# foollh/PicoPose

Measured on AMD Instinct MI355X. Metric: image-crops/sec (224x224, 162 templates), higher is better.
Workload: dtype f32 tensors; networks: f32 operands split into 2 f16 terms (22 bits) on f16 MFMA with f32 accumulate; stage-1 contraction: f16 MFMA operands, f32 accumulate, exact f32 re-evaluation of near-ties; PnP f64

## Files before the change

### include/picopose_hip.h

```cpp
#ifndef PICOPOSE_HIP_H
#define PICOPOSE_HIP_H

#include <stddef.h>
#include <stdint.h>

#ifdef __cplusplus
extern "C" {
#endif

#define PP_OK 0
#define PP_EINVAL (-1)
#define PP_EWORKSPACE (-2)
#define PP_ELAUNCH (-3)

#define PP_MATCH_EXACT 0
#define PP_MATCH_FAST 1

const char* pp_strerror(int code);
int pp_version(void);

int pp_prof_enable(int max_records);
int pp_prof_collect(float* out_ms, int max_out, int* count);
int pp_prof_gemm_enable(int max_records);
int pp_prof_gemm_collect(double* ms, double* flops, int* launches);
int pp_prof_gemm_records(int max_records, int* shape, float* ms, double* flops, int* count);
int pp_prof_gemm_records2(int max_records, int* shape, float* ms, double* flops, double* bytes, int* count);
int pp_gemm_tune_save(const char* path);
int pp_gemm_tune_load(const char* path);
int pp_gemm_tune_entries(void);
int pp_gemm_generic_epilogue(int on);

int pp_stage1_workspace_bytes(int B, int N, int C, size_t* bytes);

int pp_stage1_scores(const float* bank, const float* query, const float* mask,
                     int mask_h, int mask_w, int B, int N, int C, int mode,
                     float eps, void* workspace, size_t workspace_bytes,
                     float* sim_avg, int32_t* stats, void* stream);

#define PP_BANK_F32 0
#define PP_BANK_F16 1
int pp_stage1_scores_ex(const void* bank, int bank_dtype, const float* query, const float* mask,
                        int mask_h, int mask_w, int B, int N, int C, int mode,
                        float eps, void* workspace, size_t workspace_bytes,
                        float* sim_avg, int32_t* stats, void* stream);

int pp_topk(const float* scores, int B, int N, int k, float* out_score,
            int64_t* out_index, void* stream);

int pp_stage1_match(const float* bank, const float* query, const float* mask,
                    int mask_h, int mask_w, int B, int N, int C, int k, int mode,
                    float eps, void* workspace, size_t workspace_bytes,
                    float* sim_avg, float* out_score, int64_t* out_index,
                    int32_t* stats, void* stream);
int pp_stage1_match_ex(const void* bank, int bank_dtype, const float* query, const float* mask,
                       int mask_h, int mask_w, int B, int N, int C, int k, int mode,
                       float eps, void* workspace, size_t workspace_bytes, float* sim_avg,
                       float* out_score, int64_t* out_index, int32_t* stats, void* stream);

int pp_stage1_indexed_workspace_bytes(int B, int N, int C, size_t* bytes);
int pp_stage1_scores_indexed(const void* bank, int bank_dtype, const int64_t* obj_index, int n_obj,
                             const float* query, const float* mask, int mask_h, int mask_w, int B, int N,
                             int C, int mode, float eps, void* workspace, size_t workspace_bytes,
                             float* sim_avg, int32_t* stats, void* stream);
int pp_stage1_match_indexed(const void* bank, int bank_dtype, const int64_t* obj_index, int n_obj,
                            const float* query, const float* mask, int mask_h, int mask_w, int B, int N,
                            int C, int k, int mode, float eps, void* workspace, size_t workspace_bytes,
                            float* sim_avg, float* out_score, int64_t* out_index, int32_t* stats,
                            void* stream);



int pp_similarity_volume(const float* src_feat, const float* tar_feat, const float* src_mask,
                         int mask_h, int mask_w, int B, int C, float* out, void* stream);

int pp_calc_pred_Ms(const float* pred_scale, const float* pred_inplane, const float* pred_translation,
                    const float* tem_pose, const float* tem_K, const float* tem_M, int B,
                    float trans_scale, float* pred_Ms, void* stream);

int pp_pose_recovery_2d(const float* query_M, const float* query_K, const float* pred_Ms,
                        const float* tem_K, const float* tem_M, const float* tem_pose, int B,
                        float* pred_pose, void* stream);

int pp_init_correspondences(const float* pred_Ms, const float* tem_mask, int mask_h, int mask_w, int B,
                            float* init_flow, float* init_certainty, void* stream);

int pp_stage3_correspondences(const float* pred_flow, const float* pred_certainty, int B, int H, int W,
                              float threshold, int64_t* tar_pts, int64_t* src_pts, void* stream);

int pp_gather_valid(const float* features, const int64_t* index_patches, int B, int C, int H, int W,
                    int N, float* out, int32_t* count, void* stream);

#define PP_ACT_NONE 0
#define PP_ACT_RELU 1
#define PP_ACT_GELU 2
#define PP_ACT_LEAKY01 3
#define PP_ACT_TANH 4

#define PP_PREC_F32 0
#define PP_PREC_F16X3 1
#define PP_PREC_F16 2

typedef struct PpGemmDesc {
    const float* A;
    const float* B;
    float* C;
    const float* bias;
    const float* gamma;
    const float* residual;
    const float* residual2;
    int M, N, K;
    int lda, ldb, ldc;
    int b_kn;
    int batch0, batch1;
    long long a_bs0, a_bs1, b_bs0, b_bs1, c_bs0, c_bs1;
    float alpha;
    int act;
    int relu_in;
    int conv_kh, conv_kw, conv_cin, conv_stride, conv_pad, conv_h, conv_w, conv_ho, conv_wo;
    long long conv_bstride;
    int shuffle_r, shuffle_h, shuffle_w;
    int prec;
    const void* B_hl;
    float b_scale;
    const void* A_hl;
    long long a_hl_bytes, b_hl_bytes;
    void* C_hl;
    int ldc_h;
    int c_relu;
    const float* alpha_dev;
    const float* alpha_dev2;
    int ksplit;
    int ks_rows;
    int grp_rows;
    long long grp_b_bytes;
} PpGemmDesc;

int pp_gemm(const PpGemmDesc* desc, void* stream);
int pp_split_f16x3(const float* w, long long n, void* hl, float* scale, void* stream);
int pp_split_weights_ws(const float* w, long long n, int terms, void* out, float* scale2, float* partials, void* stream);
int pp_split_activation(const float* x, long long batch_stride, int B, int P, int row_stride, int C, int relu,
                        void* hl, void* stream);
int pp_split_activation_ld(const float* x, long long batch_stride, int B, int P, int row_stride, int C, int relu,
                           void* hl, int ld_h, void* stream);
int pp_pow2_scale_ws(const float* x, long long n, float* scale2, float* partials, void* stream);
int pp_split_scaled_t(const float* x, long long rows, int ld, int C, const float* scale, void* out, int terms, void* stream);
int pp_split_transpose_t(const float* x, long long rows, int cols, int ld, const float* scale, void* out, int terms, void* stream);
int pp_split_transpose_ld(const float* x, long long rows, int cols, int ld, const float* scale, void* out, long long ld_out, int terms,
                          void* stream);
int pp_im2col_t_operand(const float* x, int B, int H, int W, int C, int ksize, int stride, int pad, void* out, int terms, void* stream);
int pp_sum_slices(const float* part, int S, int M, int N, const float* bias, int act, float* out, void* stream);
int pp_hl_patch_columns(const float* x, int ld_x, int c, long long rows, void* hl, int ld_h, int col0, void* stream);

int pp_split_weights_t(const float* w, long long n, int terms, void* out, float* scale, void* stream);
int pp_split_activation_t(const float* x, long long batch_stride, int B, int P, int row_stride, int C, int relu, void* out,
                          int ld_h, int terms, void* stream);
int pp_hl_patch_columns_t(const float* x, int ld_x, int c, long long rows, void* out, int ld_h, int col0, int terms, void* stream);
int pp_layernorm_t(const float* x, const float* gamma, const float* beta, int rows, int C, float eps, float* y, void* out, int terms,
                   void* stream);
int pp_resize_bilinear_nhwc_t(const float* in, int B, int H, int W, int C, int Ho, int Wo, float mul, void* out, int terms,
                              void* stream);
int pp_resize_bilinear_nhwc_dual(const float* in, int B, int H, int W, int C, int Ho, int Wo, float mul, float* out, void* out_operand,
                                 int terms, void* stream);
int pp_warp_nhwc_t(const float* feat, int feat_batch, const float* flow, int B, int H, int W, int C, int ld_flow, void* out,
                   int ld_h, int terms, void* stream);
int pp_attention_t(const void* qkv_operand, int terms, int B, int T, int heads, int head_dim, float scale, float* out,
                   void* out_operand, void* stream);

int pp_attention(const float* qkv, int B, int T, int heads, int head_dim, float scale, float* out, void* stream);
int pp_attention_split(const float* qkv, int B, int T, int heads, int head_dim, float scale, float* out, void* out_hl,
                       void* stream);
int pp_attention_ex(const float* qkv, int B, int T, int heads, int head_dim, float scale, int prec, float* out, void* out_hl,
                    void* stream);
int pp_attention_hl(const void* qkv_hl, int B, int T, int heads, int head_dim, float scale, float* out, void* out_hl,
                    void* stream);
int pp_attention_train(const float* qkv, int B, int T, int heads, int head_dim, float scale, float* out, float* lse2, void* stream);
int pp_attention_backward(const float* qkv, const float* out, const float* dout, const float* lse2, const float* gpair, int B, int T,
                          int heads, int head_dim, float scale, float* Dws, float* dqkv, void* stream);

int pp_layernorm(const float* x, const float* gamma, const float* beta, int rows, int C, float eps,
                 float* y, void* stream);
int pp_layernorm_split(const float* x, const float* gamma, const float* beta, int rows, int C, float eps, float* y,
                       void* hl, void* stream);
int pp_softmax_rows(float* x, int rows, int n, int ld, void* stream);
int pp_groupnorm_nhwc(const float* x, const float* gamma, const float* beta, int B, int HW, int C,
                      int groups, float eps, int relu, float* y, void* stream);
int pp_transpose_batched(const float* in, long long in_batch_stride, int B, int R, int C, float* out,
                         long long out_batch_stride, int ld_out, int col_off, void* stream);
int pp_assemble_tokens(const float* patches, const float* cls_token, const float* pos, int B, int T, int C,
                       float* tokens, void* stream);
int pp_normalize_rows(const float* x, int rows, int n, float eps, float* y, void* stream);

int pp_resize_bilinear_nhwc(const float* in, int B, int H, int W, int C, int Ho, int Wo, float mul,
                            float* out, void* stream);
int pp_resize_bilinear_nhwc_hl(const float* in, int B, int H, int W, int C, int Ho, int Wo, float mul, void* out_hl,
                               void* stream);
int pp_warp_nhwc(const float* feat, int feat_batch, const float* flow, int B, int H, int W, int C, int ld_flow,
                 float* out, int ld_out, void* stream);
int pp_warp_nhwc_hl(const float* feat, int feat_batch, const float* flow, int B, int H, int W, int C, int ld_flow,
                    void* out_hl, int ld_h, void* stream);
int pp_avgpool2_nhwc(const float* in, int B, int H, int W, int C, float* out, void* stream);
int pp_gather_rows(const float* src, const long long* index, long long n_src_rows, long long row_floats, int n, float* dst,
                   void* stream);
int pp_bank_rows_to_tokens(const float* bank, long long n_bank_rows, int C, int P, const long long* index, int n, float* tokens, int ld,
                           int T, int skip, void* stream);
int pp_patch_operand(const float* bank, long long n_bank_rows, const long long* index, int n, const float* front, int n_front, int H, int W,
                     void* out, int terms, void* stream);
int pp_flow_operand(const float* flow, int ld_flow, long long rows, void* out8, int terms, void* stream);

int pp_crop_resize_normalize(const unsigned char* image, int H, int W, const unsigned char* mask, int y1, int y2, int x1,
                             int x2, int S, int rgb_mask_flag, const double* mean3, const double* std3, float* out_rgb,
                             float* out_mask, void* stream);
int pp_depth_points_nearest(const float* depth_m, int H, int W, int y1, int y2, int x1, int x2, int P, float fx, float fy,
                            float cx, float cy, float* out_pts, void* stream);
int pp_corr_lookup_nhwc(const float* f1, int ld_f1, const float* f2_l0, const float* f2_l1, const float* f2_l2,
                        int f2_batch, const float* flow, int B, int H, int W, int C, int levels, int radius,
                        int ld_flow, float* out, int ld_out, void* stream);
int pp_corr_lookup_nhwc_ex(const float* f1, int ld_f1, const float* f2_l0, const float* f2_l1, const float* f2_l2,
                           int f2_batch, const float* flow, int B, int H, int W, int C, int levels, int radius,
                           int ld_flow, int prec, float* out, int ld_out, void* stream);

int pp_conv_narrow_hl(const void* x_hl, int ld_x, int B, int H, int W, int C, const float* weight, const float* bias, int ksize,
                      int n_out, const float* residual, float* out, void* stream);
int pp_conv_narrow_f32(const float* x, int ld_x, int B, int H, int W, int C, const float* weight, const float* bias, int ksize,
                       int n_out, const float* residual, float* out, void* stream);

int pp_winograd_input_f32(const float* x, int ld_x, long long batch_stride, int B, int H, int W, int C, int relu, float* U, void* stream);
int pp_winograd_weight_f32(const float* w, int Cout, int Cin, int ldw, float* V, void* stream);
int pp_winograd_output_f32(const float* Y, int B, int H, int W, int Cout, const float* bias, int act, const float* residual,
                           const float* residual2, float* out, int ldc, void* stream);

int pp_winograd4_input_hl(const void* x_hl, int ld_x, long long batch_stride, int B, int H, int W, int C, int relu, void* U_hl, long long P_pad,
                          void* stream);
int pp_winograd4_weight_f32(const float* w, int Cout, int Cin, int ldw, float* V, void* stream);
int pp_winograd4_output(const float* Y, int ld_y, int B, int H, int W, int Cout, const float* bias, int act, const float* residual,
                        const float* residual2, float* out, int ldc, void* out_hl, int ld_h, int c_relu, long long P_pad, void* stream);

int pp_winograd4_chain(const float* Y, int ld_y, int B, int H, int W, int C, const float* bias, int act, int c_relu, void* U_hl, long long P_pad,
                       void* stream);

int pp_winograd_chain_f32(const float* Y, int B, int H, int W, int C, const float* bias, int act, int relu_next, float* U, void* stream);

int pp_set_saturation_word(unsigned int* word);

int pp_saturation_take(unsigned int* word, unsigned int* slot, void* stream);


int pp_corr_lookup_nhwc_hl(const void* f1_hl, int ld_f1, const void* f2_hl_l0, const void* f2_hl_l1, const void* f2_hl_l2,
                           int f2_batch, const float* flow, int B, int H, int W, int C, int levels, int radius, int ld_flow,
                           float* out, int ld_out, void* stream);

int pp_pnp_ransac(const float* tar_pts_2d, const float* src_pts_3d, const float* K, const float* tem_pose,
                  const int64_t* tar_pts, const int64_t* src_pts, int P, int H, int W, int N, int iterations,
                  float reproj_threshold, double* rot, double* tvec, double* inlier_ratio, int32_t* success,
                  int32_t* num_points, void* stream);

int pp_pnp_ransac_debug(const float* tar_pts_2d, const float* src_pts_3d, const float* K, const float* tem_pose,
                        const int64_t* tar_pts, const int64_t* src_pts, int P, int H, int W, int N, int iterations,
                        float reproj_threshold, double* rot, double* tvec, double* inlier_ratio, int32_t* success,
                        int32_t* num_points, double* refit_branches, void* stream);

int pp_pnp_ransac_refine(const float* tar_pts_2d, const float* src_pts_3d, const float* K, const float* tem_pose,
                         const int64_t* tar_pts, const int64_t* src_pts, int P, int H, int W, int N, int iterations,
                         float reproj_threshold, int max_iters, double eps, double* rot, double* tvec, double* inlier_ratio,
                         int32_t* success, int32_t* num_points, double* rms_before, double* rms_after, int32_t* lm_iterations,
                         uint8_t* inlier_mask, void* stream);

int pp_pnp_refine_lm(const double* object_points, const double* image_points, const int32_t* count, const double* K,
                     const double* rot_init, const double* tvec_init, int P, int Nmax, int max_iters, double eps, double* rot,
                     double* tvec, double* rms_before, double* rms_after, int32_t* lm_iterations, void* stream);

int pp_rgbd_ransac(const float* tar_pts_2d, const float* src_pts_3d, const float* K, const float* tem_pose,
                   const int64_t* tar_pts, const int64_t* src_pts, int P, int H, int W, int N,
                   const float* depth, int n_images, int dH, int dW, const int32_t* image_index,
                   const float* inlier_dist, int iterations,
                   double* rot, double* tvec, double* inlier_ratio, int32_t* success,
                   int32_t* num_points, int32_t* num_listed, double* rms, uint8_t* inlier_mask, void* stream);

size_t pp_train_keypoints_workspace_bytes(int B);
int pp_train_keypoints(const float* src_mask, const float* tar_mask, int mask_h, int mask_w, const float* src_depth,
                       const float* tar_depth, int depth_h, int depth_w, const float* src_Minv, const float* tar_Minv,
                       const float* src_M, const float* tar_M, const float* src_Kinv, const float* tar_Kinv, const float* src_K,
                       const float* tar_K, const float* T_src2tar, const float* T_tar2src, int B, float* src_pts, float* tar_pts,
                       void* workspace, size_t workspace_bytes, void* stream);
size_t pp_batchnorm_train_workspace_bytes(int rows, int C);
int pp_batchnorm_train(const float* x, const float* gamma, const float* beta, int rows, int C, float eps, float momentum,
                       float* running_mean, float* running_var, int relu, const float* residual, const float* residual2, float* y,
                       void* workspace, size_t workspace_bytes, void* stream);
int pp_gather_normalize_rows(const float* src, long long row_stride, const int64_t* index, int n, int C, float eps, float* out,
                             void* stream);
int pp_xent_diag_rows(const float* logits, int n, int ld, float scale, float* row_loss, void* stream);
int pp_flow_loss_blocks(void);
int pp_flow_loss_sums(const float* flow, const float* certainty, const float* tar_pts, int B, int H, int W, float max_flow,
                      double* partial_sums, void* stream);

size_t pp_colsum_workspace_bytes(long long rows, int cols);
int pp_colsum(const float* x, long long rows, int cols, int ld, float* out, void* workspace, size_t workspace_bytes, void* stream);
int pp_act_forward(const float* z, long long n, int act, float* y, void* stream);
int pp_act_backward(const float* z, const float* dy, long long n, int act, float* dz, void* stream);
int pp_elementwise(int op, const float* a, const float* b, long long n, int cols, float* out, void* stream);
int pp_layernorm_backward(const float* x, const float* gamma, const float* dy, int rows, int C, float eps, float* dx, float* gx, void* stream);
int pp_groupnorm_backward_nhwc(const float* x, const float* gamma, const float* beta, const float* dy, int B, int HW, int C, int groups,
                               float eps, int relu, float* dx, float* gx, float* gy, void* stream);
int pp_softmax_backward_rows(const float* p, const float* dp, long long rows, int n, float* ds, void* stream);
int pp_xent_diag_backward(const float* logits, int n, int ld, float scale, const float* upstream, float* dlogits, void* stream);
int pp_scatter_add_rows(const float* src, const int64_t* index, int n, int C, float* dst, void* stream);
int pp_normalize_rows_backward(const float* x, long long row_stride, const int64_t* index, const float* dq, int rows, int C, float eps,
                               float* dx, void* stream);
int pp_im2col_nhwc(const float* x, int B, int H, int W, int C, int ksize, int stride, int pad, float* col, void* stream);
int pp_col2im_nhwc(const float* col, int B, int H, int W, int C, int ksize, int stride, int pad, float* dx, void* stream);
int pp_split_with_scale_t(const float* w, long long n, int terms, const float* scale, void* out, void* stream);
int pp_pow2_scale(const float* x, long long n, float* scale2, void* stream);
int pp_im2col_t_nhwc(const float* x, int B, int H, int W, int C, int ksize, int stride, int pad, float* colT, void* stream);
int pp_simvol_backward(const float* out, const float* dout, const float* src_mask, int mask_h, int mask_w, int B, float* dS, void* stream);

size_t pp_batchnorm_train_backward_workspace_bytes(long long rows, int C);
int pp_batchnorm_train_backward(const float* x, const float* gamma, const float* beta, const float* dy, long long rows, int C, float eps,
                                int relu, float* dx, float* dgamma, float* dbeta, void* workspace, size_t workspace_bytes, void* stream);
int pp_resize_bilinear_backward_nhwc(const float* dy, int B, int H, int W, int C, int Ho, int Wo, float mul, float* dx, void* stream);
int pp_avgpool2_backward_nhwc(const float* dy, int B, int H, int W, int C, int accumulate, float* dx, void* stream);
int pp_warp_backward_nhwc(const float* feat, const float* flow, const float* dy, int B, int H, int W, int C, int ld_flow, float* dfeat,
                          float* dflow, void* stream);
int pp_corr_lookup_backward_nhwc(const float* f1, const float* const* f2_levels, const float* flow, const float* dout, int B, int H, int W,
                                 int C, int levels, int radius, int ld_flow, int ld_dout, float* df1, float* const* df2_levels, float* dflow,
                                 void* stream);
int pp_warp_backward_nhwc_fixed(const float* feat, const float* flow, const float* dy, int B, int H, int W, int C, int ld_flow,
                                long long* dfeat_acc, float* dflow, void* stream);
int pp_corr_lookup_backward_nhwc_fixed(const float* f1, const float* const* f2_levels, const float* flow, const float* dout, int B, int H,
                                       int W, int C, int levels, int radius, int ld_flow, int ld_dout, float* df1,
                                       long long* const* df2_acc_levels, float* dflow, void* stream);
int pp_fixed_to_float(const long long* acc, long long n, float* out, void* stream);
int pp_flow_loss_backward(const float* flow, const float* certainty, const float* tar_pts, int B, int H, int W, float max_flow,
                          const float* g_flow, const float* g_cert, float* dflow, float* dcertainty, void* stream);


#define PP_ADAM_CHUNK 65536
typedef struct PpAdamTensor {
    float* p;
    float* m;
    float* v;
    void* hl;
    float* scale2;
    long long n;
} PpAdamTensor;
typedef struct PpAdamStep {
    const float* g;
    float neg_step_size, inv_bc2_sqrt, decay, lerp_w, beta2, one_minus_beta2, eps;
    int mode;
} PpAdamStep;
int pp_adam_workspace_bytes(const PpAdamTensor* tensors, int ntensors, size_t* bytes);
int pp_adam_multi_tensor(const PpAdamTensor* tensors, int ntensors, const PpAdamStep* steps, int terms, int rebuild, void* workspace,
                         size_t workspace_bytes, void* stream);

#define PP_AUG_OP_WORDS 8
#define PP_AUG_IMG_WORDS 20
#define PP_AUG_MAX_OPS 13
#define PP_AUG_MAX_PASSES 4
#define PP_AUG_DROP_THRESHOLD 858993459u
int pp_augment_execute(const unsigned char* rgb0, const unsigned char* mask0, long long n_frame0_px, const unsigned char* rgba1,
                       long long n_frame1_px,
                       const int* images, int n_images, const int* ops, int n_ops, const int* tiles, const int* pass_tiles,
                       int n_passes, unsigned char* buf0, unsigned char* buf1, long long n_buf_px, unsigned int* lsum,
                       void* stream);
int pp_augment_resize(const unsigned char* buf0, const unsigned char* buf1, long long n_buf_px, const int* images, int n_images,
                      int S, int rgb_mask_flag, const double* mean3, const double* std3, float* out_rgb, float* out_mask,
                      void* stream);
int pp_depth_u16_scaled(const unsigned short* depth, long long n_per_frame, int n_frames, const float* scale, float* out,
                        void* stream);
int pp_depth_u16_template(const unsigned short* depth, long long n, float* out, void* stream);

int pp_detections_crop(const unsigned char* image, int H, int W, const int* run_ends, int n_runs, const int* run_offset,
                       const int* window, const int* run_offset_host, const int* window_host, int n, int S, int rgb_mask_flag,
                       const double* mean3, const double* std3, float* out_rgb, float* out_mask, void* stream);

int pp_render_workspace_bytes(int H, int W, int n_faces, int chunk_views, size_t* bytes);
int pp_render_views(const float* vertices, int n_vertices, const int* faces, const int* faces_host, int n_faces,
                    const unsigned char* colors, const float* poses, int n_views, float fx, float fy, float cx, float cy, int H,
                    int W, float near, void* workspace, size_t workspace_bytes, unsigned char* rgba, unsigned short* depth_mm,
                    float* depth_m, int* face_id, unsigned int* near_count, void* stream);
#define PP_TEXTURE_MAX 16384
int pp_texture_mips_bytes(int Wt, int Ht, size_t* bytes, int* levels);
int pp_texture_build_mips(const unsigned char* rgb, int Wt, int Ht, void* mips, size_t mips_bytes, void* stream);
int pp_render_views_textured(const float* vertices, int n_vertices, const int* faces, const int* faces_host, int n_faces,
                             const float* face_uv, const void* mips, int Wt, int Ht, const float* poses, int n_views, float fx,
                             float fy, float cx, float cy, int H, int W, float near, void* workspace, size_t workspace_bytes,
                             unsigned char* rgba, unsigned short* depth_mm, float* depth_m, int* face_id, unsigned int* near_count,
                             void* stream);
#define PP_MAX_LIGHTS 16
#define PP_TONE_MAX 65536
#define PP_NORMALS_FLAT 0
#define PP_NORMALS_SMOOTH 1
int pp_vertex_normals(const float* vertices, int n_vertices, const int* faces, int n_faces, const int* vf_offsets, const int* vf_faces,
                      float* normals, void* stream);
int pp_render_views_lit(const float* vertices, int n_vertices, const int* faces, const int* faces_host, int n_faces,
                        const unsigned char* colors, const float* face_uv, const void* mips, int Wt, int Ht, const float* poses,
                        int n_views, float fx, float fy, float cx, float cy, int H, int W, float near, void* workspace,
                        size_t workspace_bytes, unsigned char* rgba, unsigned short* depth_mm, float* depth_m, int* face_id,
                        unsigned int* near_count, const float* lights_host, int n_lights, float ambient, int normal_mode,
                        const float* normals, const unsigned char* base_color_host, const unsigned char* tone_table, int tone_entries,
                        void* stream);
int pp_template_extents(const unsigned char* rgba, int n_views, int H, int W, int* extents, int* counts, void* stream);
int pp_templates_crop(const unsigned char* rgba, const void* depth, int depth_is_f32, int n_views, int H, int W, const int* boxes,
                      const int* boxes_host, float fx, float fy, float cx, float cy, int S, int P, int rgb_mask_flag,
                      const double* mean3, const double* std3, float* out_rgb, float* out_mask, float* out_pts, void* stream);

#define PP_EVAL_MSSD 1
#define PP_EVAL_MSPD 2
#define PP_EVAL_ADD 4
#define PP_EVAL_ADDS 8
#define PP_EVAL_ADDS_TILE 1024
int pp_pose_errors_workspace_bytes(int n_pairs, int max_syms, int max_adds_vertices, int kinds, size_t* bytes);
int pp_pose_errors(const float* vertices, const int* vert_off, const float* adds_vertices, const int* adds_off, const float* sym_R,
                   const float* sym_t, const int* sym_off, const int* vert_off_host, const int* adds_off_host,
                   const int* sym_off_host, int n_objects, const int* pair_obj, const int* pair_obj_host, const float* R_est,
                   const float* t_est, const float* R_gt, const float* t_gt, const float* focal, int n_pairs, int kinds,
                   void* workspace, size_t workspace_bytes, float* mssd, int* mssd_sym, float* mspd, int* mspd_sym, float* add,
                   float* adds, void* stream);

typedef struct PpScene {
    const float* vertices;
    const int* vert_off;
    const int* faces;
    const int* face_off;
    const float* diameters;
    const float* cams;
    const int* view_obj;
    const int* view_img;
    const float* poses;
    const int* windows;
    const long long* view_zoff;
    const int* vert_off_host;
    const int* faces_host;
    const int* face_off_host;
    const float* diameters_host;
    const float* cams_host;
    const int* view_obj_host;
    const int* view_img_host;
    const int* windows_host;
    const long long* view_zoff_host;
    int n_objects, n_images, H, W, n_views;
    float near;
} PpScene;

#define PP_VSD_MAX_TAUS 16
int pp_vsd_workspace_bytes(long long window_samples, long long view_faces, size_t* bytes);
int pp_vsd_errors(const PpScene* scene, const int* pair_est, const int* pair_gt, const int* pair_est_host, const int* pair_gt_host,
                  int n_pairs, const float* depth, float delta, const float* taus_host, int n_taus, void* workspace,
                  size_t workspace_bytes, float* vsd, int* counts, unsigned int* near_count, float* depth_out, void* stream);

#define PP_DEPTH_REFINE_STRIP_ROWS 8
#define PP_DEPTH_REFINE_SUMS 29
#define PP_DEPTH_REFINE_MAX_ITERATIONS 1000
int pp_depth_refine_workspace_bytes(long long window_samples, long long view_faces, long long strips, size_t* bytes);
int pp_depth_refine(const PpScene* scene, const float* boxes, const float* boxes_host, const int* view_soff, const int* view_soff_host,
                    const float* depth, int iterations, float max_distance, int min_points, float min_cos, float rcond, float eps,
                    float max_translation, float max_rotation, void* workspace, size_t workspace_bytes, float* poses_out,
                    int* active, int* status, int* n_iterations, int* rank, int* n_points, float* rms_before, float* rms_after,
                    unsigned int* near_count, float* trajectory, double* sums, void* stream);

int pp_scene_gt_workspace_bytes(long long window_samples, long long view_faces, long long composite_pixels, size_t* bytes);
int pp_scene_gt(const PpScene* scene, const float* canvas_cams, const float* canvas_cams_host, int pad_x, int pad_y, const float* depth,
                float delta, const int* view_label, int use_view_label, void* workspace, size_t workspace_bytes, int* counts, int* boxes,
                unsigned int* near_count, unsigned char* mask_all, unsigned char* mask_visib, float* scene_depth, int* instance_map,
                void* stream);

#define PP_MODEL_INFO_TILE 1024
int pp_model_diameter_workspace_bytes(const int* vert_off_host, int n_objects, size_t* bytes);
int pp_model_diameter(const float* vertices, const int* vert_off, const int* vert_off_host, int n_objects, void* workspace,
                      size_t workspace_bytes, float* d2max, int* pair, void* stream);
int pp_transform_hausdorff_workspace_bytes(int n_candidates, int max_query_vertices, size_t* bytes);
int pp_transform_hausdorff(const float* vertices, const int* vert_off, const float* q_vertices, const int* q_off,
                           const int* vert_off_host, const int* q_off_host, int n_objects, const int* cand_obj,
                           const int* cand_obj_host, const float* cand_T, int n_candidates, void* workspace, size_t workspace_bytes,
                           float* h, void* stream);

#define PP_SYNTH_BG_WORDS 4
#define PP_SYNTH_TILE 1024
int pp_scene_composite_workspace_bytes(int n_layers, int H, int W, size_t* bytes);
int pp_scene_composite(const unsigned char* layers_rgba, const float* layers_depth, const int* layer_off, const int* layer_off_host,
                       int n_layers, int n_images, int H, int W, const int* background, const int* background_host,
                       const unsigned char* bg_images, const float* depth_scale, const float* depth_scale_host, void* workspace,
                       size_t workspace_bytes, unsigned char* rgb, unsigned short* depth, int* instance, int* counts, int* boxes,
                       unsigned char* mask_visib, void* stream);
int pp_depth_quantize_u16(const float* depth_m, long long n, float units_per_metre, unsigned short* out, void* stream);

#define PP_MATCH_TILE 16
#define PP_MATCH_MAX_C 1024
#define PP_MATCH_MAX_TOPK 8
#define PP_MASK_MAX_N 4096
int pp_descriptor_normalize(const float* x, int n, int C, float eps, float* y, void* stream);
int pp_proposal_match(const float* query, int P, const float* bank, const int* offsets, const int* offsets_host, int O, int C,
                      int topk, float* score, int* view, int* label, float* best, void* stream);
int pp_rle_pack_bits(const int* run_ends, int n_runs, const int* run_offset, const int* run_offset_host, int n, int hw, int words,
                     unsigned* bits, int* area, void* stream);
int pp_mask_intersections(const unsigned* bits, int n, int words, int* inter, void* stream);

#ifdef __cplusplus
}
#endif
#endif
```

### picopose_amd/_lib.py

```python
import ctypes
import os
import re

from .build import LIB

_HEADER = os.path.join(os.path.dirname(os.path.abspath(__file__)), "..", "include", "picopose_hip.h")

PP_OK = 0
PP_MATCH_EXACT = 0
PP_MATCH_FAST = 1
PP_BANK_F32 = 0
PP_BANK_F16 = 1

_lib = None


class PpGemmDesc(ctypes.Structure):
    _fields_ = [
        ("A", ctypes.c_void_p), ("B", ctypes.c_void_p), ("C", ctypes.c_void_p), ("bias", ctypes.c_void_p),
        ("gamma", ctypes.c_void_p), ("residual", ctypes.c_void_p), ("residual2", ctypes.c_void_p),
        ("M", ctypes.c_int), ("N", ctypes.c_int), ("K", ctypes.c_int),
        ("lda", ctypes.c_int), ("ldb", ctypes.c_int), ("ldc", ctypes.c_int), ("b_kn", ctypes.c_int),
        ("batch0", ctypes.c_int), ("batch1", ctypes.c_int),
        ("a_bs0", ctypes.c_longlong), ("a_bs1", ctypes.c_longlong), ("b_bs0", ctypes.c_longlong),
        ("b_bs1", ctypes.c_longlong), ("c_bs0", ctypes.c_longlong), ("c_bs1", ctypes.c_longlong),
        ("alpha", ctypes.c_float), ("act", ctypes.c_int), ("relu_in", ctypes.c_int),
        ("conv_kh", ctypes.c_int), ("conv_kw", ctypes.c_int), ("conv_cin", ctypes.c_int),
        ("conv_stride", ctypes.c_int), ("conv_pad", ctypes.c_int), ("conv_h", ctypes.c_int),
        ("conv_w", ctypes.c_int), ("conv_ho", ctypes.c_int), ("conv_wo", ctypes.c_int),
        ("conv_bstride", ctypes.c_longlong),
        ("shuffle_r", ctypes.c_int), ("shuffle_h", ctypes.c_int), ("shuffle_w", ctypes.c_int),
        ("prec", ctypes.c_int), ("B_hl", ctypes.c_void_p), ("b_scale", ctypes.c_float), ("A_hl", ctypes.c_void_p),
        ("a_hl_bytes", ctypes.c_longlong), ("b_hl_bytes", ctypes.c_longlong),
        ("C_hl", ctypes.c_void_p), ("ldc_h", ctypes.c_int), ("c_relu", ctypes.c_int),
        ("alpha_dev", ctypes.c_void_p), ("alpha_dev2", ctypes.c_void_p),
        ("ksplit", ctypes.c_int), ("ks_rows", ctypes.c_int), ("grp_rows", ctypes.c_int), ("grp_b_bytes", ctypes.c_longlong),
    ]


class PpScene(ctypes.Structure):
    _fields_ = ([(name, ctypes.c_void_p) for name in (
        "vertices", "vert_off", "faces", "face_off", "diameters", "cams", "view_obj", "view_img", "poses", "windows", "view_zoff",
        "vert_off_host", "faces_host", "face_off_host", "diameters_host", "cams_host", "view_obj_host", "view_img_host", "windows_host",
        "view_zoff_host")] + [(name, ctypes.c_int) for name in ("n_objects", "n_images", "H", "W", "n_views")] + [("near", ctypes.c_float)])


class PpAdamTensor(ctypes.Structure):
    _fields_ = [("p", ctypes.c_void_p), ("m", ctypes.c_void_p), ("v", ctypes.c_void_p), ("hl", ctypes.c_void_p),
                ("scale2", ctypes.c_void_p), ("n", ctypes.c_longlong)]


class PicoPoseHipError(RuntimeError):
    pass


def declared_symbols():
    text = open(_HEADER).read()
    text = re.sub(r"/\*.*?\*/", "", text, flags=re.S)
    return sorted(set(re.findall(r"\b(pp_[a-z0-9_]+)\s*\(", text)))


def lib():
    global _lib
    if _lib is None:
        if not os.path.exists(LIB):
            raise PicoPoseHipError(
                f"{LIB} not found: build it with `python -m picopose_amd.build` "
                "(hipcc --offload-arch=gfx950). There is no CPU fallback."
            )
        import torch

        L = ctypes.CDLL(LIB)
        c = ctypes
        vp, i32, f32, sz = c.c_void_p, c.c_int, c.c_float, c.c_size_t
        L.pp_strerror.restype = c.c_char_p
        L.pp_strerror.argtypes = [i32]
        L.pp_version.restype = i32
        L.pp_prof_enable.argtypes = [i32]
        L.pp_prof_collect.argtypes = [c.POINTER(f32), i32, c.POINTER(i32)]
        L.pp_prof_gemm_enable.argtypes = [i32]
        L.pp_prof_gemm_collect.argtypes = [c.POINTER(c.c_double), c.POINTER(c.c_double), c.POINTER(i32)]
        L.pp_prof_gemm_records.argtypes = [i32, c.POINTER(i32), c.POINTER(f32), c.POINTER(c.c_double), c.POINTER(i32)]
        L.pp_prof_gemm_records2.argtypes = [i32, c.POINTER(i32), c.POINTER(f32), c.POINTER(c.c_double), c.POINTER(c.c_double), c.POINTER(i32)]
        L.pp_gemm_tune_save.argtypes = [c.c_char_p]
        L.pp_gemm_tune_load.argtypes = [c.c_char_p]
        L.pp_gemm_tune_entries.argtypes = []
        L.pp_gemm_generic_epilogue.argtypes = [i32]
        L.pp_stage1_workspace_bytes.argtypes = [i32, i32, i32, c.POINTER(sz)]
        L.pp_stage1_scores.argtypes = [vp, vp, vp, i32, i32, i32, i32, i32, i32, f32, vp, sz, vp, vp, vp]
        L.pp_stage1_scores_ex.argtypes = [vp, i32, vp, vp, i32, i32, i32, i32, i32, i32, f32, vp, sz, vp, vp, vp]
        L.pp_topk.argtypes = [vp, i32, i32, i32, vp, vp, vp]
        L.pp_stage1_match.argtypes = [vp, vp, vp, i32, i32, i32, i32, i32, i32, i32, f32, vp, sz,
                                      vp, vp, vp, vp, vp]
        L.pp_stage1_match_ex.argtypes = [vp, i32, vp, vp, i32, i32, i32, i32, i32, i32, i32, f32, vp, sz, vp, vp, vp, vp, vp]
        L.pp_stage1_indexed_workspace_bytes.argtypes = [i32, i32, i32, c.POINTER(sz)]
        L.pp_stage1_scores_indexed.argtypes = [vp, i32, vp, i32, vp, vp, i32, i32, i32, i32, i32, i32, f32, vp, sz, vp, vp, vp]
        L.pp_stage1_match_indexed.argtypes = [vp, i32, vp, i32, vp, vp, i32, i32, i32, i32, i32, i32, i32, f32, vp, sz, vp, vp, vp,
                                              vp, vp]
        L.pp_similarity_volume.argtypes = [vp, vp, vp, i32, i32, i32, i32, vp, vp]
        L.pp_calc_pred_Ms.argtypes = [vp, vp, vp, vp, vp, vp, i32, f32, vp, vp]
        L.pp_pose_recovery_2d.argtypes = [vp, vp, vp, vp, vp, vp, i32, vp, vp]
        L.pp_init_correspondences.argtypes = [vp, vp, i32, i32, i32, vp, vp, vp]
        L.pp_stage3_correspondences.argtypes = [vp, vp, i32, i32, i32, f32, vp, vp, vp]
        L.pp_gather_valid.argtypes = [vp, vp, i32, i32, i32, i32, i32, vp, vp, vp]
        L.pp_gemm.argtypes = [c.POINTER(PpGemmDesc), vp]
        L.pp_split_f16x3.argtypes = [vp, c.c_longlong, vp, vp, vp]
        L.pp_split_activation.argtypes = [vp, c.c_longlong, i32, i32, i32, i32, i32, vp, vp]
        L.pp_split_activation_ld.argtypes = [vp, c.c_longlong, i32, i32, i32, i32, i32, vp, i32, vp]
        L.pp_conv_narrow_hl.argtypes = [vp, i32, i32, i32, i32, i32, vp, vp, i32, i32, vp, vp, vp]
        L.pp_conv_narrow_f32.argtypes = [vp, i32, i32, i32, i32, i32, vp, vp, i32, i32, vp, vp, vp]
        L.pp_winograd_input_f32.argtypes = [vp, i32, c.c_longlong, i32, i32, i32, i32, i32, vp, vp]
        L.pp_winograd_weight_f32.argtypes = [vp, i32, i32, i32, vp, vp]
        L.pp_winograd_output_f32.argtypes = [vp, i32, i32, i32, i32, vp, i32, vp, vp, vp, i32, vp]
        L.pp_winograd4_input_hl.argtypes = [vp, i32, c.c_longlong, i32, i32, i32, i32, i32, vp, c.c_longlong, vp]
        L.pp_winograd4_weight_f32.argtypes = [vp, i32, i32, i32, vp, vp]
        L.pp_winograd4_output.argtypes = [vp, i32, i32, i32, i32, i32, vp, i32, vp, vp, vp, i32, vp, i32, i32, c.c_longlong, vp]
        L.pp_winograd4_chain.argtypes = [vp, i32, i32, i32, i32, i32, vp, i32, i32, vp, c.c_longlong, vp]
        L.pp_winograd_chain_f32.argtypes = [vp, i32, i32, i32, i32, vp, i32, i32, vp, vp]
        L.pp_set_saturation_word.argtypes = [vp]
        L.pp_saturation_take.argtypes = [vp, vp, vp]
        L.pp_split_weights_t.argtypes = [vp, c.c_longlong, i32, vp, vp, vp]
        L.pp_split_weights_ws.argtypes = [vp, c.c_longlong, i32, vp, vp, vp, vp]
        L.pp_split_activation_t.argtypes = [vp, c.c_longlong, i32, i32, i32, i32, i32, vp, i32, i32, vp]
        L.pp_hl_patch_columns_t.argtypes = [vp, i32, i32, c.c_longlong, vp, i32, i32, i32, vp]
        L.pp_layernorm_t.argtypes = [vp, vp, vp, i32, i32, f32, vp, vp, i32, vp]
        L.pp_resize_bilinear_nhwc_t.argtypes = [vp, i32, i32, i32, i32, i32, i32, f32, vp, i32, vp]
        L.pp_resize_bilinear_nhwc_dual.argtypes = [vp, i32, i32, i32, i32, i32, i32, f32, vp, vp, i32, vp]
        L.pp_warp_nhwc_t.argtypes = [vp, i32, vp, i32, i32, i32, i32, i32, vp, i32, i32, vp]
        L.pp_attention_t.argtypes = [vp, i32, i32, i32, i32, i32, f32, vp, vp, vp]
        L.pp_sum_slices.argtypes = [vp, i32, i32, i32, vp, i32, vp, vp]
        L.pp_hl_patch_columns.argtypes = [vp, i32, i32, c.c_longlong, vp, i32, i32, vp]
        L.pp_warp_nhwc_hl.argtypes = [vp, i32, vp, i32, i32, i32, i32, i32, vp, i32, vp]
        L.pp_attention.argtypes = [vp, i32, i32, i32, i32, f32, vp, vp]
        L.pp_attention_split.argtypes = [vp, i32, i32, i32, i32, f32, vp, vp, vp]
        L.pp_attention_ex.argtypes = [vp, i32, i32, i32, i32, f32, i32, vp, vp, vp]
        L.pp_attention_hl.argtypes = [vp, i32, i32, i32, i32, f32, vp, vp, vp]
        L.pp_attention_train.argtypes = [vp, i32, i32, i32, i32, f32, vp, vp, vp]
        L.pp_attention_backward.argtypes = [vp, vp, vp, vp, vp, i32, i32, i32, i32, f32, vp, vp, vp]
        L.pp_layernorm.argtypes = [vp, vp, vp, i32, i32, f32, vp, vp]
        L.pp_layernorm_split.argtypes = [vp, vp, vp, i32, i32, f32, vp, vp, vp]
        L.pp_softmax_rows.argtypes = [vp, i32, i32, i32, vp]
        L.pp_groupnorm_nhwc.argtypes = [vp, vp, vp, i32, i32, i32, i32, f32, i32, vp, vp]
        L.pp_transpose_batched.argtypes = [vp, c.c_longlong, i32, i32, i32, vp, c.c_longlong, i32, i32, vp]
        L.pp_assemble_tokens.argtypes = [vp, vp, vp, i32, i32, i32, vp, vp]
        L.pp_normalize_rows.argtypes = [vp, i32, i32, f32, vp, vp]
        L.pp_resize_bilinear_nhwc.argtypes = [vp, i32, i32, i32, i32, i32, i32, f32, vp, vp]
        L.pp_resize_bilinear_nhwc_hl.argtypes = [vp, i32, i32, i32, i32, i32, i32, f32, vp, vp]
        L.pp_warp_nhwc.argtypes = [vp, i32, vp, i32, i32, i32, i32, i32, vp, i32, vp]
        L.pp_avgpool2_nhwc.argtypes = [vp, i32, i32, i32, i32, vp, vp]
        L.pp_gather_rows.argtypes = [vp, vp, c.c_longlong, c.c_longlong, i32, vp, vp]
        L.pp_bank_rows_to_tokens.argtypes = [vp, c.c_longlong, i32, i32, vp, i32, vp, i32, i32, i32, vp]
        L.pp_patch_operand.argtypes = [vp, c.c_longlong, vp, i32, vp, i32, i32, i32, vp, i32, vp]
        L.pp_flow_operand.argtypes = [vp, i32, c.c_longlong, vp, i32, vp]
        L.pp_depth_points_nearest.argtypes = [vp, i32, i32, i32, i32, i32, i32, i32, f32, f32, f32, f32, vp, vp]
        L.pp_crop_resize_normalize.argtypes = [vp, i32, i32, vp, i32, i32, i32, i32, i32, i32, c.POINTER(c.c_double),
                                               c.POINTER(c.c_double), vp, vp, vp]
        L.pp_corr_lookup_nhwc.argtypes = [vp, i32, vp, vp, vp, i32, vp, i32, i32, i32, i32, i32, i32, i32, vp, i32, vp]
        L.pp_corr_lookup_nhwc_ex.argtypes = [vp, i32, vp, vp, vp, i32, vp, i32, i32, i32, i32, i32, i32, i32, i32, vp, i32, vp]
        L.pp_corr_lookup_nhwc_hl.argtypes = [vp, i32, vp, vp, vp, i32, vp, i32, i32, i32, i32, i32, i32, i32, vp, i32, vp]
        L.pp_pnp_ransac.argtypes = [vp, vp, vp, vp, vp, vp, i32, i32, i32, i32, i32, f32, vp, vp, vp, vp, vp, vp]
        L.pp_pnp_ransac_debug.argtypes = [vp, vp, vp, vp, vp, vp, i32, i32, i32, i32, i32, f32, vp, vp, vp, vp, vp, vp, vp]
        L.pp_pnp_ransac_refine.argtypes = [vp, vp, vp, vp, vp, vp, i32, i32, i32, i32, i32, f32, i32, c.c_double] + [vp] * 10
        L.pp_pnp_refine_lm.argtypes = [vp] * 6 + [i32, i32, i32, c.c_double] + [vp] * 6
        L.pp_rgbd_ransac.argtypes = [vp] * 6 + [i32] * 4 + [vp, i32, i32, i32, vp, vp, i32] + [vp] * 9
        L.pp_train_keypoints_workspace_bytes.restype = sz
        L.pp_train_keypoints_workspace_bytes.argtypes = [i32]
        L.pp_train_keypoints.argtypes = [vp, vp, i32, i32, vp, vp, i32, i32] + [vp] * 10 + [i32, vp, vp, vp, sz, vp]
        L.pp_batchnorm_train_workspace_bytes.restype = sz
        L.pp_batchnorm_train_workspace_bytes.argtypes = [i32, i32]
        L.pp_batchnorm_train.argtypes = [vp, vp, vp, i32, i32, f32, f32, vp, vp, i32, vp, vp, vp, vp, sz, vp]
        L.pp_gather_normalize_rows.argtypes = [vp, c.c_longlong, vp, i32, i32, f32, vp, vp]
        L.pp_xent_diag_rows.argtypes = [vp, i32, i32, f32, vp, vp]
        L.pp_flow_loss_blocks.argtypes = []
        L.pp_flow_loss_sums.argtypes = [vp, vp, vp, i32, i32, i32, f32, vp, vp]
        ll = c.c_longlong
        L.pp_colsum_workspace_bytes.restype = sz
        L.pp_colsum_workspace_bytes.argtypes = [ll, i32]
        L.pp_colsum.argtypes = [vp, ll, i32, i32, vp, vp, sz, vp]
        L.pp_act_forward.argtypes = [vp, ll, i32, vp, vp]
        L.pp_act_backward.argtypes = [vp, vp, ll, i32, vp, vp]
        L.pp_elementwise.argtypes = [i32, vp, vp, ll, i32, vp, vp]
        L.pp_layernorm_backward.argtypes = [vp, vp, vp, i32, i32, f32, vp, vp, vp]
        L.pp_groupnorm_backward_nhwc.argtypes = [vp, vp, vp, vp, i32, i32, i32, i32, f32, i32, vp, vp, vp, vp]
        L.pp_softmax_backward_rows.argtypes = [vp, vp, ll, i32, vp, vp]
        L.pp_xent_diag_backward.argtypes = [vp, i32, i32, f32, vp, vp, vp]
        L.pp_normalize_rows_backward.argtypes = [vp, ll, vp, vp, i32, i32, f32, vp, vp]
        L.pp_scatter_add_rows.argtypes = [vp, vp, i32, i32, vp, vp]
        L.pp_im2col_nhwc.argtypes = [vp, i32, i32, i32, i32, i32, i32, i32, vp, vp]
        L.pp_col2im_nhwc.argtypes = [vp, i32, i32, i32, i32, i32, i32, i32, vp, vp]
        L.pp_simvol_backward.argtypes = [vp, vp, vp, i32, i32, i32, vp, vp]
        L.pp_im2col_t_nhwc.argtypes = [vp, i32, i32, i32, i32, i32, i32, i32, vp, vp]
        L.pp_pow2_scale.argtypes = [vp, ll, vp, vp]
        L.pp_pow2_scale_ws.argtypes = [vp, ll, vp, vp, vp]
        L.pp_split_scaled_t.argtypes = [vp, ll, i32, i32, vp, vp, i32, vp]
        L.pp_split_transpose_t.argtypes = [vp, ll, i32, i32, vp, vp, i32, vp]
        L.pp_split_transpose_ld.argtypes = [vp, ll, i32, i32, vp, vp, ll, i32, vp]
        L.pp_im2col_t_operand.argtypes = [vp, i32, i32, i32, i32, i32, i32, i32, vp, i32, vp]
        L.pp_split_with_scale_t.argtypes = [vp, ll, i32, vp, vp, vp]
        L.pp_batchnorm_train_backward_workspace_bytes.restype = sz
        L.pp_batchnorm_train_backward_workspace_bytes.argtypes = [ll, i32]
        L.pp_batchnorm_train_backward.argtypes = [vp, vp, vp, vp, ll, i32, f32, i32, vp, vp, vp, vp, sz, vp]
        L.pp_resize_bilinear_backward_nhwc.argtypes = [vp, i32, i32, i32, i32, i32, i32, f32, vp, vp]
        L.pp_avgpool2_backward_nhwc.argtypes = [vp, i32, i32, i32, i32, i32, vp, vp]
        L.pp_warp_backward_nhwc.argtypes = [vp, vp, vp, i32, i32, i32, i32, i32, vp, vp, vp]
        L.pp_corr_lookup_backward_nhwc.argtypes = [vp, vp, vp, vp, i32, i32, i32, i32, i32, i32, i32, i32, vp, vp, vp, vp]
        L.pp_warp_backward_nhwc_fixed.argtypes = [vp, vp, vp, i32, i32, i32, i32, i32, vp, vp, vp]
        L.pp_corr_lookup_backward_nhwc_fixed.argtypes = [vp, vp, vp, vp, i32, i32, i32, i32, i32, i32, i32, i32, vp, vp, vp, vp]
        L.pp_fixed_to_float.argtypes = [vp, ll, vp, vp]
        L.pp_flow_loss_backward.argtypes = [vp, vp, vp, i32, i32, i32, f32, vp, vp, vp, vp, vp]
        L.pp_adam_workspace_bytes.argtypes = [c.POINTER(PpAdamTensor), i32, c.POINTER(sz)]
        L.pp_adam_multi_tensor.argtypes = [c.POINTER(PpAdamTensor), i32, vp, i32, i32, vp, sz, vp]
        L.pp_augment_execute.argtypes = [vp, vp, ll, vp, ll, vp, i32, vp, i32, vp, c.POINTER(i32), i32, vp, vp, ll, vp, vp]
        L.pp_augment_resize.argtypes = [vp, vp, ll, vp, i32, i32, i32, c.POINTER(c.c_double), c.POINTER(c.c_double), vp, vp, vp]
        L.pp_depth_u16_scaled.argtypes = [vp, ll, i32, vp, vp, vp]
        L.pp_depth_u16_template.argtypes = [vp, ll, vp, vp]
        L.pp_detections_crop.argtypes = [vp, i32, i32, vp, i32, vp, vp, c.POINTER(i32), c.POINTER(i32), i32, i32, i32,
                                         c.POINTER(c.c_double), c.POINTER(c.c_double), vp, vp, vp]
        L.pp_render_workspace_bytes.argtypes = [i32, i32, i32, i32, c.POINTER(sz)]
        L.pp_render_views.argtypes = [vp, i32, vp, vp, i32, vp, vp, i32, f32, f32, f32, f32, i32, i32, f32, vp, sz, vp, vp, vp, vp, vp, vp]
        L.pp_texture_mips_bytes.argtypes = [i32, i32, c.POINTER(sz), c.POINTER(i32)]
        L.pp_texture_build_mips.argtypes = [vp, i32, i32, vp, sz, vp]
        L.pp_render_views_textured.argtypes = [vp, i32, vp, vp, i32, vp, vp, i32, i32, vp, i32, f32, f32, f32, f32, i32, i32, f32, vp, sz,
                                               vp, vp, vp, vp, vp, vp]
        L.pp_vertex_normals.argtypes = [vp, i32, vp, i32, vp, vp, vp, vp]
        L.pp_render_views_lit.argtypes = [vp, i32, vp, vp, i32, vp, vp, vp, i32, i32, vp, i32, f32, f32, f32, f32, i32, i32, f32, vp, sz,
                                          vp, vp, vp, vp, vp, vp, i32, f32, i32, vp, vp, vp, i32, vp]
        L.pp_template_extents.argtypes = [vp, i32, i32, i32, vp, vp, vp]
        L.pp_templates_crop.argtypes = [vp, vp, i32, i32, i32, i32, vp, vp, f32, f32, f32, f32, i32, i32, i32,
                                        c.POINTER(c.c_double), c.POINTER(c.c_double), vp, vp, vp, vp]
        L.pp_pose_errors_workspace_bytes.argtypes = [i32, i32, i32, i32, c.POINTER(sz)]
        L.pp_pose_errors.argtypes = [vp] * 10 + [i32] + [vp] * 7 + [i32, i32, vp, sz] + [vp] * 7
        L.pp_vsd_workspace_bytes.argtypes = [ll, ll, c.POINTER(sz)]
        scene = c.POINTER(PpScene)
        L.pp_vsd_errors.argtypes = [scene, vp, vp, vp, vp, i32, vp, f32, vp, i32, vp, sz, vp, vp, vp, vp, vp]
        L.pp_depth_refine_workspace_bytes.argtypes = [ll, ll, ll, c.POINTER(sz)]
        L.pp_depth_refine.argtypes = [scene, vp, vp, vp, vp, vp, i32, f32, i32, f32, f32, f32, f32, f32, vp, sz,
                                      vp, vp, vp, vp, vp, vp, vp, vp, vp, vp, vp, vp]
        L.pp_scene_gt_workspace_bytes.argtypes = [ll, ll, ll, c.POINTER(sz)]
        L.pp_scene_gt.argtypes = [scene, vp, vp, i32, i32, vp, f32, vp, i32, vp, sz, vp, vp, vp, vp, vp, vp, vp, vp]
        L.pp_model_diameter_workspace_bytes.argtypes = [vp, i32, c.POINTER(sz)]
        L.pp_model_diameter.argtypes = [vp, vp, vp, i32, vp, sz, vp, vp, vp]
        L.pp_transform_hausdorff_workspace_bytes.argtypes = [i32, i32, c.POINTER(sz)]
        L.pp_transform_hausdorff.argtypes = [vp] * 6 + [i32, vp, vp, vp, i32, vp, sz, vp, vp]
        L.pp_scene_composite_workspace_bytes.argtypes = [i32, i32, i32, c.POINTER(sz)]
        L.pp_scene_composite.argtypes = [vp] * 4 + [i32] * 4 + [vp] * 6 + [sz] + [vp] * 7
        L.pp_depth_quantize_u16.argtypes = [vp, ll, f32, vp, vp]
        L.pp_descriptor_normalize.argtypes = [vp, i32, i32, f32, vp, vp]
        L.pp_proposal_match.argtypes = [vp, i32, vp, vp, c.POINTER(i32), i32, i32, i32, vp, vp, vp, vp, vp]
        L.pp_rle_pack_bits.argtypes = [vp, i32, vp, c.POINTER(i32), i32, i32, i32, vp, vp, vp]
        L.pp_mask_intersections.argtypes = [vp, i32, i32, vp, vp]
        _lib = L
    return _lib


def stream_ptr():
    import torch

    return ctypes.c_void_p(torch.cuda.current_stream().cuda_stream)


def dev_f32(*tensors):
    out = []
    for t in tensors:
        if not t.is_cuda:
            raise PicoPoseHipError("picopose_amd runs on the GPU only: inputs must be CUDA(HIP) tensors")
        out.append(t.contiguous().float())
    return out


def check(rc, what):
    if rc != PP_OK:
        raise PicoPoseHipError(f"{what} failed: {lib().pp_strerror(rc).decode()} (code {rc})")
```

### picopose_amd/csrc/pp_sample.hip

```cpp

#include <hip/hip_runtime.h>
#include <stdlib.h>
#include <stdint.h>
#include "../../include/picopose_hip.h"
#include "pp_common.h"
#include "pp_crop_dev.h"

namespace {

typedef float f4 __attribute__((ext_vector_type(4)));

__device__ __forceinline__ float resize_blend(float a, float b, float c, float d, float hx, float lx, float hy, float ly, float mul) {
#pragma clang fp contract(off)
    const float top = fmaf(hx, a, lx * b), bot = fmaf(hx, c, lx * d);
    return (hy * top + ly * bot) * mul;
}

__global__ __launch_bounds__(256) void resize_kernel(const float* __restrict__ in, int H, int W, int C,
                                                     int Ho, int Wo, float mul, float* __restrict__ out,
                                                     _Float16* __restrict__ out_hl, int terms) {
    const int b = blockIdx.z, oy = blockIdx.y, tid = threadIdx.x;
    const float sy = Ho > 1 ? (float)(H - 1) / (float)(Ho - 1) : 0.f;
    const float sx = Wo > 1 ? (float)(W - 1) / (float)(Wo - 1) : 0.f;
    const float fy = sy * (float)oy;
    const int y0 = (int)fy, y1 = y0 + (y0 < H - 1 ? 1 : 0);
    const float ly = fy - (float)y0, hy = 1.f - ly;
    const float* ib = in + (size_t)b * H * W * C;
    if (out_hl) {
        _Float16* oh = out_hl + ((size_t)b * Ho + oy) * Wo * terms * C;
        float* of = out ? out + ((size_t)b * Ho + oy) * Wo * C : nullptr;
        const int C8 = C >> 3;
        for (int i = blockIdx.x * 256 + tid; i < Wo * C8; i += gridDim.x * 256) {
            const int ox = i / C8, c = (i - ox * C8) * 8;
            const float fx = sx * (float)ox;
            const int x0 = (int)fx, x1 = x0 + (x0 < W - 1 ? 1 : 0);
            const float lx = fx - (float)x0, hx = 1.f - lx;
            typedef _Float16 h8 __attribute__((ext_vector_type(8)));
            h8 hh, ll;
#pragma unroll
            for (int q = 0; q < 2; ++q) {
                const int cc = c + 4 * q;
                const f4 a = *(const f4*)(ib + ((size_t)y0 * W + x0) * C + cc), bq = *(const f4*)(ib + ((size_t)y0 * W + x1) * C + cc);
                const f4 cq = *(const f4*)(ib + ((size_t)y1 * W + x0) * C + cc), dq = *(const f4*)(ib + ((size_t)y1 * W + x1) * C + cc);
                f4 vq;
#pragma unroll
                for (int k = 0; k < 4; ++k) {
                    const float v = resize_blend(a[k], bq[k], cq[k], dq[k], hx, lx, hy, ly, mul);
                    _Float16 h, l;
                    pp_split_f16_chk(v, h, l);
                    hh[4 * q + k] = h;
                    ll[4 * q + k] = l;
                    vq[k] = v;
                }
                if (of) *(f4*)(of + (size_t)ox * C + cc) = vq;
            }
            *(h8*)(oh + ((size_t)ox * C + c) * terms) = hh;
            if (terms == 2) *(h8*)(oh + (size_t)ox * 2 * C + 2 * c + 8) = ll;
        }
        return;
    }
    float* ob = out + ((size_t)b * Ho + oy) * Wo * C;
    if ((C & 3) == 0 && (((uintptr_t)in | (uintptr_t)out) & 15) == 0) {
        const int C4 = C >> 2;
        for (int i = blockIdx.x * 256 + tid; i < Wo * C4; i += gridDim.x * 256) {
            const int ox = i / C4, c = (i - ox * C4) * 4;
            const float fx = sx * (float)ox;
            const int x0 = (int)fx, x1 = x0 + (x0 < W - 1 ? 1 : 0);
            const float lx = fx - (float)x0, hx = 1.f - lx;
            const f4 a = *(const f4*)(ib + ((size_t)y0 * W + x0) * C + c), bq = *(const f4*)(ib + ((size_t)y0 * W + x1) * C + c);
            const f4 cq = *(const f4*)(ib + ((size_t)y1 * W + x0) * C + c), dq = *(const f4*)(ib + ((size_t)y1 * W + x1) * C + c);
            f4 v;
#pragma unroll
            for (int k = 0; k < 4; ++k) v[k] = resize_blend(a[k], bq[k], cq[k], dq[k], hx, lx, hy, ly, mul);
            *(f4*)(ob + (size_t)ox * C + c) = v;
        }
        return;
    }
    for (int i = blockIdx.x * 256 + tid; i < Wo * C; i += gridDim.x * 256) {
        const int ox = i / C, c = i - ox * C;
        const float fx = sx * (float)ox;
        const int x0 = (int)fx, x1 = x0 + (x0 < W - 1 ? 1 : 0);
        const float lx = fx - (float)x0, hx = 1.f - lx;
        ob[i] = resize_blend(ib[((size_t)y0 * W + x0) * C + c], ib[((size_t)y0 * W + x1) * C + c], ib[((size_t)y1 * W + x0) * C + c],
                             ib[((size_t)y1 * W + x1) * C + c], hx, lx, hy, ly, mul);
    }
}

__device__ __forceinline__ float roundtrip(float x, int size) {
    const float n = x * 2.f / (float)(size - 1 > 1 ? size - 1 : 1) - 1.f;
    return ((n + 1.f) / 2.f) * (float)(size - 1);
}

template <bool HL>
__global__ __launch_bounds__(256) void warp_kernel(const float* __restrict__ feat, int feat_batch,
                                                   const float* __restrict__ flow, int H, int W, int C, int ld_flow,
                                                   float* __restrict__ out, int ld_out, int terms) {
    const int b = blockIdx.y, p = blockIdx.x * 4 + (threadIdx.x >> 6), lane = threadIdx.x & 63;
    if (p >= H * W) return;
    const int y = p / W, x = p - y * W;
    const float* fl = flow + ((size_t)b * H * W + p) * ld_flow;
    const float ix = fminf(fmaxf(roundtrip((float)x + fl[0], W), -2.f), (float)W + 1.f);
    const float iy = fminf(fmaxf(roundtrip((float)y + fl[1], H), -2.f), (float)H + 1.f);
    const float x0f = floorf(ix), y0f = floorf(iy);
    const int x0 = (int)x0f, y0 = (int)y0f;
    const float wx1 = ix - x0f, wx0 = (x0f + 1.f) - ix, wy1 = iy - y0f, wy0 = (y0f + 1.f) - iy;
    const float* fb = feat + (size_t)(b % feat_batch) * H * W * C;
    float* o = HL ? nullptr : out + ((size_t)b * H * W + p) * ld_out;
    _Float16* oh = HL ? (_Float16*)out + ((size_t)b * H * W + p) * terms * ld_out : nullptr;
    const bool vx0 = x0 >= 0 && x0 < W, vx1 = x0 + 1 >= 0 && x0 + 1 < W;
    const bool vy0 = y0 >= 0 && y0 < H, vy1 = y0 + 1 >= 0 && y0 + 1 < H;
    typedef unsigned u4w __attribute__((ext_vector_type(4)));
    const unsigned m00 = 0u - (unsigned)(vy0 & vx0), m01 = 0u - (unsigned)(vy0 & vx1), m10 = 0u - (unsigned)(vy1 & vx0),
                   m11 = 0u - (unsigned)(vy1 & vx1);
    const int xa = min(max(x0, 0), W - 1), xb = min(max(x0 + 1, 0), W - 1), ya = min(max(y0, 0), H - 1), yb = min(max(y0 + 1, 0), H - 1);
    auto tap = [&](int yy, int xx, int c, unsigned m) __attribute__((always_inline)) -> f4 {
        const u4w raw = *(const u4w*)(fb + ((size_t)yy * W + xx) * C + c) & m;
        return __builtin_bit_cast(f4, raw);
    };
    for (int c = lane * 4; c < C; c += 256) {
        f4 acc = {0.f, 0.f, 0.f, 0.f};
        acc += tap(ya, xa, c, m00) * (wx0 * wy0);
        acc += tap(ya, xb, c, m01) * (wx1 * wy0);
        acc += tap(yb, xa, c, m10) * (wx0 * wy1);
        acc += tap(yb, xb, c, m11) * (wx1 * wy1);
        if (HL) {
            typedef _Float16 h4w __attribute__((ext_vector_type(4)));
            _Float16 h0, h1, h2, h3, l0, l1, l2, l3;
            pp_split_f16_chk(acc.x, h0, l0);
            pp_split_f16_chk(acc.y, h1, l1);
            pp_split_f16_chk(acc.z, h2, l2);
            pp_split_f16_chk(acc.w, h3, l3);
            if (terms == 2) {
                _Float16* q = oh + pp_hl_col(c, 0);
                *(h4w*)q = h4w{h0, h1, h2, h3};
                *(h4w*)(q + 8) = h4w{l0, l1, l2, l3};
            } else {
                *(h4w*)(oh + c) = h4w{h0, h1, h2, h3};
            }
        } else {
            *(f4*)(o + c) = acc;
        }
    }
}

__global__ __launch_bounds__(256) void avgpool2_kernel(const float* __restrict__ in, int H, int W, int C,
                                                       float* __restrict__ out) {
    const int Ho = H / 2, Wo = W / 2, b = blockIdx.y;
    const size_t n = (size_t)Ho * Wo * C;
    const float* ib = in + (size_t)b * H * W * C;
    float* ob = out + (size_t)b * n;
    for (size_t i = (size_t)blockIdx.x * 256 + threadIdx.x; i < n; i += (size_t)gridDim.x * 256) {
        const int c = (int)(i % C);
        const size_t q = i / C;
        const int ox = (int)(q % Wo), oy = (int)(q / Wo);
        const float* p = ib + ((size_t)(2 * oy) * W + 2 * ox) * C + c;
        ob[i] = ((p[0] + p[C]) + (p[(size_t)W * C] + p[(size_t)W * C + C])) * 0.25f;
    }
}

constexpr int MAXR = 2, TW = 2 * MAXR + 2, MAXL = 3;
__global__ __launch_bounds__(256) void corr_lookup_kernel(const float* __restrict__ f1, int ld_f1,
                                                          int f2_batch, const float* __restrict__ f2l0,
                                                          const float* __restrict__ f2l1,
                                                          const float* __restrict__ f2l2,
                                                          const float* __restrict__ flow, int H, int W, int C,
                                                          int L, int r, int ld_flow, float inv_sqrt_c,
                                                          float* __restrict__ out, int ld_out) {
    extern __shared__ __attribute__((aligned(16))) float sm[];
    const int wv = threadIdx.x >> 6, lane = threadIdx.x & 63;
    float* a = sm + (size_t)wv * (C + MAXL * TW * TW);
    float* tab = a + C;
    const int b = blockIdx.y, p = blockIdx.x * 4 + wv;
    const bool live = p < H * W;
    const int y = live ? p / W : 0, x = live ? p - y * W : 0;
    const int tw = 2 * r + 2, win = 2 * r + 1;
    if (live) {
        const float* src = f1 + ((size_t)b * H * W + p) * ld_f1;
        for (int c = lane * 4; c < C; c += 256) *(f4*)(a + c) = *(const f4*)(src + c);
    }
    __builtin_amdgcn_fence(__ATOMIC_RELEASE, "wavefront");
    __builtin_amdgcn_s_waitcnt(0xC07F);
    __builtin_amdgcn_wave_barrier();
    float cx[MAXL], cy[MAXL];
    int bx[MAXL], by[MAXL];
    if (live) {
        const float* fl = flow + ((size_t)b * H * W + p) * ld_flow;
        const float gx = (float)x + fl[0], gy = (float)y + fl[1];
        for (int l = 0; l < L; ++l) {
            const int Hl = H >> l, Wl = W >> l;
            const float sc = (float)(1 << l);
            cx[l] = fminf(fmaxf(roundtrip(gx / sc, Wl), -(float)(r + 2)), (float)(Wl + r + 1));
            cy[l] = fminf(fmaxf(roundtrip(gy / sc, Hl), -(float)(r + 2)), (float)(Hl + r + 1));
            bx[l] = (int)floorf(cx[l]) - r;
            by[l] = (int)floorf(cy[l]) - r;
        }
        const int npos = L * tw * tw;
        for (int i = lane; i < npos; i += 64) {
            const int l = i / (tw * tw), rem = i - l * tw * tw, dy = rem / tw, dx = rem - dy * tw;
            const int Hl = H >> l, Wl = W >> l;
            const int qx = bx[l] + dx, qy = by[l] + dy;
            float dot = 0.f;
            const bool inside = qx >= 0 && qx < Wl && qy >= 0 && qy < Hl;
            const int qxc = min(max(qx, 0), Wl - 1), qyc = min(max(qy, 0), Hl - 1);
            const float* f2 = l == 0 ? f2l0 : (l == 1 ? f2l1 : f2l2);
            const float* q = f2 + (((size_t)(b % f2_batch) * Hl + qyc) * Wl + qxc) * C;
            for (int c = 0; c < C; c += 4) {
                const f4 u = *(const f4*)(a + c), v = *(const f4*)(q + c);
                dot = fmaf(u.x, v.x, dot);
                dot = fmaf(u.y, v.y, dot);
                dot = fmaf(u.z, v.z, dot);
                dot = fmaf(u.w, v.w, dot);
            }
            tab[i] = inside ? dot * inv_sqrt_c : 0.f;
        }
    }
    __builtin_amdgcn_fence(__ATOMIC_RELEASE, "wavefront");
    __builtin_amdgcn_s_waitcnt(0xC07F);
    __builtin_amdgcn_wave_barrier();
    if (live) {
        float* o = out + ((size_t)b * H * W + p) * ld_out;
        const int nout = L * win * win;
        for (int i = lane; i < nout; i += 64) {
            const int l = i / (win * win), rem = i - l * win * win, ai = rem / win, bi = rem - ai * win;
            const float wx1 = cx[l] - floorf(cx[l]), wy1 = cy[l] - floorf(cy[l]);
            const float wx0 = 1.f - wx1, wy0 = 1.f - wy1;
            const float* t = tab + l * tw * tw + bi * tw + ai;
            o[i] = t[0] * (wx0 * wy0) + t[1] * (wx1 * wy0) + t[tw] * (wx0 * wy1) + t[tw + 1] * (wx1 * wy1);
        }
        for (int i = nout + lane; i < ld_out; i += 64) o[i] = 0.f;
    }
}

constexpr int CT = 8, CM = CT * CT;
constexpr int CRW = 16, CN = CRW * CRW;
constexpr int CK = 32, CKP = CK + 4;
typedef _Float16 h8_t __attribute__((ext_vector_type(8)));
typedef _Float16 h4_t __attribute__((ext_vector_type(4)));
constexpr int CSP = CN + 4;
typedef float f32x16_t __attribute__((ext_vector_type(16)));

template <bool HLIN, bool EXACT = false, bool ONE = false>
__global__ __launch_bounds__(256, 2) void corr_lookup_mfma_kernel(const void* __restrict__ f1v, int ld_f1, int f2_batch,
                                                                  const void* __restrict__ f2l0, const void* __restrict__ f2l1,
                                                                  const void* __restrict__ f2l2, const float* __restrict__ flow,
                                                                  int B, int H, int W, int C, int L, int r, int ld_flow,
                                                                  float inv_sqrt_c, float* __restrict__ out, int ld_out) {
    extern __shared__ __attribute__((aligned(16))) float sm[];
    float* As = sm;
    float* Bs = sm + CM * CKP;
    float* S = sm;
    __shared__ float s_cx[CM], s_cy[CM];
    __shared__ int s_bx[CM], s_by[CM], s_state[CM], s_ox, s_oy, s_todo;
    const int tid = threadIdx.x, lane = tid & 63, wv = tid >> 6, l31 = lane & 31, lh = lane >> 5;
    const int tiles_x = W / CT, tiles = tiles_x * (H / CT), total = tiles * B;
    int g = blockIdx.x;
    if (total % 8 == 0) g = (g % 8) * (total / 8) + g / 8;
    const int b = g / tiles, tile = g - b * tiles;
    const int y0 = (tile / tiles_x) * CT, x0 = (tile % tiles_x) * CT;
    const int tw = 2 * r + 2, win = 2 * r + 1, fit = CRW - tw;
    const int my = tid >> 3, mx = tid & 7;
    float gx = 0.f, gy = 0.f;
    if (tid < CM) {
        const float* fl = flow + ((size_t)b * H * W + (size_t)(y0 + my) * W + x0 + mx) * ld_flow;
        gx = (float)(x0 + mx) + fl[0];
        gy = (float)(y0 + my) + fl[1];
    }
    for (int npad = ld_out - L * win * win, idx = tid; idx < CM * npad; idx += 256) {
        const int m = idx / npad, o = idx - m * npad;
        out[((size_t)b * H * W + (size_t)(y0 + (m >> 3)) * W + x0 + (m & 7)) * ld_out + L * win * win + o] = 0.f;
    }
    for (int l = 0; l < L; ++l) {
        const int Hl = H >> l, Wl = W >> l;
        const void* f2v = l == 0 ? f2l0 : (l == 1 ? f2l1 : f2l2);
        const float* f2 = (const float*)f2v + (size_t)(b % f2_batch) * Hl * Wl * C;
        const _Float16* f2h = (const _Float16*)f2v + (size_t)(b % f2_batch) * Hl * Wl * C * 2;
        const float* f1 = (const float*)f1v;
        const _Float16* f1h = (const _Float16*)f1v;
        if (tid == 0) s_todo = 0;
        __syncthreads();
        if (tid < CM) {
            const float sc = (float)(1 << l);
            const float cx = fminf(fmaxf(roundtrip(gx / sc, Wl), -1.0e6f), 1.0e6f);
            const float cy = fminf(fmaxf(roundtrip(gy / sc, Hl), -1.0e6f), 1.0e6f);
            const int bx = (int)floorf(cx) - r, by = (int)floorf(cy) - r;
            s_cx[tid] = cx; s_cy[tid] = cy; s_bx[tid] = bx; s_by[tid] = by;
            const bool outside = bx >= Wl || by >= Hl || bx + tw <= 0 || by + tw <= 0;
            s_state[tid] = outside ? 2 : 0;
            if (!outside) atomicAdd(&s_todo, 1);
        }
        __syncthreads();
        for (int idx = tid; idx < CM * win * win; idx += 256) {
            const int m = idx / (win * win), o = idx - m * (win * win);
            if (s_state[m] == 2)
                out[((size_t)b * H * W + (size_t)(y0 + (m >> 3)) * W + x0 + (m & 7)) * ld_out + l * win * win + o] = 0.f;
        }
        while (s_todo > 0) {
            if (tid == 0) { s_ox = 0x7fffffff; s_oy = 0x7fffffff; }
            __syncthreads();
            if (tid < CM && s_state[tid] == 0) atomicMin(&s_ox, s_bx[tid]);
            __syncthreads();
            if (tid < CM && s_state[tid] == 0 && s_bx[tid] - s_ox <= fit) atomicMin(&s_oy, s_by[tid]);
            __syncthreads();
            const int ox = s_ox, oy = s_oy;
            f32x16_t acc[2][2];
#pragma unroll
            for (int i = 0; i < 2; ++i)
#pragma unroll
                for (int j = 0; j < 2; ++j)
#pragma unroll
                    for (int e = 0; e < 16; ++e) acc[i][j][e] = 0.f;
            f4 ra0[2], rb0[8], ra1[2], rb1[8];
            const int part = tid & 7, row0 = tid >> 3;
            auto load_chunk = [&](int kc, f4 (&ra)[2], f4 (&rb)[8]) __attribute__((always_inline)) {
#pragma unroll
                for (int i = 0; i < 2; ++i) {
                    const int m = row0 + 32 * i;
                    const size_t px = (size_t)b * H * W + (size_t)(y0 + (m >> 3)) * W + x0 + (m & 7);
                    ra[i] = HLIN ? *(const f4*)(f1h + (px * ld_f1 + kc * CK) * 2 + 8 * part) : *(const f4*)(f1 + px * ld_f1 + kc * CK + 4 * part);
                }
#pragma unroll
                for (int i = 0; i < 8; ++i) {
                    const int n = row0 + 32 * i, qy = oy + (n >> 4), qx = ox + (n & 15);
                    const bool in = qx >= 0 && qx < Wl && qy >= 0 && qy < Hl;
                    const size_t px = (size_t)qy * Wl + qx;
                    rb[i] = !in ? f4{0.f, 0.f, 0.f, 0.f}
                                : (HLIN ? *(const f4*)(f2h + (px * C + kc * CK) * 2 + 8 * part) : *(const f4*)(f2 + px * C + kc * CK + 4 * part));
                }
            };
            auto put = [&](float* rowp, f4 v) __attribute__((always_inline)) {
                if (EXACT) {
                    *(f4*)(rowp + 4 * part) = v;
                    return;
                }
                if (HLIN) {
                    *(f4*)((_Float16*)rowp + 8 * part) = v;
                    return;
                }
                _Float16* g8 = (_Float16*)rowp + 16 * (part >> 1) + 4 * (part & 1);
                if (ONE) {
                    const h4_t hi = {pp_to_f16(v.x), pp_to_f16(v.y), pp_to_f16(v.z), pp_to_f16(v.w)};
                    *(h4_t*)g8 = hi;
                    return;
                }
                _Float16 h0, h1, h2, h3, l0, l1, l2, l3;
                pp_split_f16(v.x, h0, l0);
                pp_split_f16(v.y, h1, l1);
                pp_split_f16(v.z, h2, l2);
                pp_split_f16(v.w, h3, l3);
                const h4_t hi = {h0, h1, h2, h3}, lo = {l0, l1, l2, l3};
                *(h4_t*)g8 = hi;
                *(h4_t*)(g8 + 8) = lo;
            };
#ifdef PP_STUDY_CORR_NK1
            const int nk = 1;
#else
            const int nk = C / CK;
#endif
            auto chunk = [&](int kc, f4 (&ra)[2], f4 (&rb)[8]) __attribute__((always_inline)) {
                __syncthreads();
#pragma unroll
                for (int i = 0; i < 2; ++i) put(As + (row0 + 32 * i) * CKP, ra[i]);
#pragma unroll
                for (int i = 0; i < 8; ++i) put(Bs + (row0 + 32 * i) * CKP, rb[i]);
                __syncthreads();
                if (kc + 2 < nk) load_chunk(kc + 2, ra, rb);
                if constexpr (EXACT) {
#pragma unroll
                    for (int q = 0; q < 4; ++q) {
                        f4 af[2], bf[2];
#pragma unroll
                        for (int i = 0; i < 2; ++i) {
                            af[i] = *(const f4*)(As + (i * 32 + l31) * CKP + 16 * lh + 4 * q);
                            bf[i] = *(const f4*)(Bs + (wv * 64 + i * 32 + l31) * CKP + 16 * lh + 4 * q);
                        }
#pragma unroll
                        for (int e = 0; e < 4; ++e)
#pragma unroll
                            for (int i = 0; i < 2; ++i)
#pragma unroll
                                for (int j = 0; j < 2; ++j)
                                    acc[i][j] = __builtin_amdgcn_mfma_f32_32x32x2f32(af[i][e], bf[j][e], acc[i][j], 0, 0, 0);
                    }
                    return;
                }
#pragma unroll
                for (int q = 0; q < 2; ++q) {
                    h8_t ah[2], al[2], bh[2], bl[2];
#pragma unroll
                    for (int i = 0; i < 2; ++i) {
                        const _Float16* ar = (const _Float16*)(As + (i * 32 + l31) * CKP) + 16 * (2 * q + lh);
                        const _Float16* br = (const _Float16*)(Bs + (wv * 64 + i * 32 + l31) * CKP) + 16 * (2 * q + lh);
                        ah[i] = *(const h8_t*)ar;
                        bh[i] = *(const h8_t*)br;
                        if (!ONE) {
                            al[i] = *(const h8_t*)(ar + 8);
                            bl[i] = *(const h8_t*)(br + 8);
                        }
                    }
#pragma unroll
                    for (int i = 0; i < 2; ++i)
#pragma unroll
                        for (int j = 0; j < 2; ++j) {
                            acc[i][j] = __builtin_amdgcn_mfma_f32_32x32x16_f16(ah[i], bh[j], acc[i][j], 0, 0, 0);
                            if (!ONE) {
                                acc[i][j] = __builtin_amdgcn_mfma_f32_32x32x16_f16(ah[i], bl[j], acc[i][j], 0, 0, 0);
                                acc[i][j] = __builtin_amdgcn_mfma_f32_32x32x16_f16(al[i], bh[j], acc[i][j], 0, 0, 0);
                            }
                        }
                }
            };
            load_chunk(0, ra0, rb0);
            if (nk > 1) load_chunk(1, ra1, rb1);
            for (int kc = 0; kc < nk; kc += 2) {
                chunk(kc, ra0, rb0);
                if (kc + 1 < nk) chunk(kc + 1, ra1, rb1);
            }
            __syncthreads();
#pragma unroll
            for (int i = 0; i < 2; ++i)
#pragma unroll
                for (int j = 0; j < 2; ++j)
#pragma unroll
                    for (int e = 0; e < 16; ++e)
                        S[(i * 32 + (e >> 2) * 8 + lh * 4 + (e & 3)) * CSP + wv * 64 + j * 32 + l31] =
                            acc[i][j][e] * (EXACT ? inv_sqrt_c : inv_sqrt_c / (PP_A_SCALE * PP_A_SCALE));
            __syncthreads();
            for (int idx = tid; idx < CM * win * win; idx += 256) {
                const int m = idx / (win * win), o = idx - m * (win * win), ai = o / win, bi = o - ai * win;
                const int dx = s_bx[m] - ox, dy = s_by[m] - oy;
                if (s_state[m] == 0 && dx >= 0 && dx <= fit && dy >= 0 && dy <= fit) {
                    const float cx = s_cx[m], cy = s_cy[m];
                    const float wx1 = cx - floorf(cx), wy1 = cy - floorf(cy), wx0 = 1.f - wx1, wy0 = 1.f - wy1;
                    const float* t = S + m * CSP + (dy + bi) * CRW + dx + ai;
                    out[((size_t)b * H * W + (size_t)(y0 + (m >> 3)) * W + x0 + (m & 7)) * ld_out + l * win * win + o] =
                        t[0] * (wx0 * wy0) + t[1] * (wx1 * wy0) + t[CRW] * (wx0 * wy1) + t[CRW + 1] * (wx1 * wy1);
                }
            }
            __syncthreads();
            if (tid < CM && s_state[tid] == 0) {
                const int dx = s_bx[tid] - ox, dy = s_by[tid] - oy;
                if (dx >= 0 && dx <= fit && dy >= 0 && dy <= fit) {
                    s_state[tid] = 1;
                    atomicSub(&s_todo, 1);
                }
            }
            __syncthreads();
        }
        __syncthreads();
    }
}

__global__ __launch_bounds__(256) void gather_rows_kernel(const float* __restrict__ src, const long long* __restrict__ index,
                                                          long long row, long long nsrc, float* __restrict__ dst) {
    const long long r = index[blockIdx.y];
    if (r < 0 || r >= nsrc) return;
    const f4* s4 = (const f4*)(src + r * row);
    f4* d4 = (f4*)(dst + (long long)blockIdx.y * row);
    const long long n4 = row >> 2;
    for (long long i = (long long)blockIdx.x * 256 + threadIdx.x; i < n4; i += (long long)gridDim.x * 256) d4[i] = s4[i];
}

__global__ __launch_bounds__(256) void bank_rows_to_tokens_kernel(const float* __restrict__ bank, const long long* __restrict__ index,
                                                                  long long nsrc, int C, int P, float* __restrict__ tokens, int ld, int T,
                                                                  int skip) {
    __shared__ float t[32][33];
    const long long r = index[blockIdx.z];
    if (r < 0 || r >= nsrc) return;
    const int c0 = blockIdx.x * 32, p0 = blockIdx.y * 32;
    const int tx = threadIdx.x & 31, ty = threadIdx.x >> 5;
    const float* src = bank + (size_t)r * C * P;
    float* dst = tokens + (size_t)blockIdx.z * T * ld;
#pragma unroll
    for (int i = 0; i < 4; ++i) {
        const int c = c0 + ty + 8 * i, p = p0 + tx;
        if (c < C && p < P) t[ty + 8 * i][tx] = src[(size_t)c * P + p];
    }
    __syncthreads();
#pragma unroll
    for (int i = 0; i < 4; ++i) {
        const int p = p0 + ty + 8 * i, c = c0 + tx;
        if (p < P && c < C) dst[(size_t)(skip + p) * ld + c] = t[tx][ty + 8 * i];
    }
    if (blockIdx.y == 0 && c0 + tx < C)
        for (int s = ty; s < skip; s += 8) dst[(size_t)s * ld + c0 + tx] = 0.f;
}

__global__ __launch_bounds__(64) void saturation_take_kernel(unsigned* __restrict__ word, unsigned* __restrict__ slot) {
    if (threadIdx.x == 0) *slot = atomicExch(word, 0u);
}

__global__ __launch_bounds__(256) void crop_resize_kernel(const unsigned char* __restrict__ img, int W,
                                                          const unsigned char* __restrict__ mask, int y1, int y2, int x1,
                                                          int x2, int S, int mask_rgb, double m0, double m1, double m2,
                                                          double s0, double s1, double s2, float* __restrict__ out_rgb,
                                                          float* __restrict__ out_mask) {
    const int i = blockIdx.x * 256 + threadIdx.x;
    if (i >= S * S) return;
    const int oy = i / S, ox = i - oy * S, h = y2 - y1, w = x2 - x1;
    int ya, yb, xa, xb;
    double fy, fx;
    pp_crop_taps(oy, h, S, ya, yb, fy);
    pp_crop_taps(ox, w, S, xa, xb, fx);
    const double mean[3] = {m0, m1, m2}, stdv[3] = {s0, s1, s2};
    auto px = [&](int yy, int xx, int c) -> double {
        const size_t p = (size_t)(y1 + yy) * W + (x1 + xx);
        double v = (double)img[p * 3 + (2 - c)] / 255.0;
        if (mask_rgb && mask && mask[p] == 0) v = 0.0;
        return v;
    };
#pragma unroll
    for (int c = 0; c < 3; ++c) out_rgb[(size_t)c * S * S + i] = pp_crop_blend(px, c, ya, yb, xa, xb, fx, fy, mean[c], stdv[c]);
    if (out_mask) {
        const int yi = pp_crop_nearest(oy, h, S), xi = pp_crop_nearest(ox, w, S);
        out_mask[i] = mask ? (float)mask[(size_t)(y1 + yi) * W + (x1 + xi)] : 1.f;
    }
}

__global__ __launch_bounds__(256) void depth_points_kernel(const float* __restrict__ depth, int W, int y1, int y2, int x1,
                                                           int x2, int P, float fx, float fy, float cx, float cy,
                                                           float* __restrict__ out) {
    const int i = blockIdx.x * 256 + threadIdx.x;
    if (i >= P * P) return;
    const int oy = i / P, ox = i - oy * P, h = y2 - y1, w = x2 - x1;
    const int y = y1 + pp_crop_nearest(oy, h, P), x = x1 + pp_crop_nearest(ox, w, P);
    pp_depth_point(depth[(size_t)y * W + x], x, y, fx, fy, cx, cy, out + 3 * i);
}


constexpr int NRW_PITCH = 144;

template <int KS, int NOUT, bool F32IN = false>
__global__ __launch_bounds__(256) void conv_narrow_kernel(const _Float16* __restrict__ x, int ldx, int H, int W, int C,
                                                          const float* __restrict__ w, const float* __restrict__ bias,
                                                          const float* __restrict__ residual, float* __restrict__ out) {
    constexpr int R = KS / 2;
    extern __shared__ __attribute__((aligned(16))) unsigned char nsm[];
    const int TH = 256 / W, bands = H / TH;
    const int b = blockIdx.x / bands, y0 = (blockIdx.x % bands) * TH;
    const int tid = threadIdx.x, ty = tid / W, tx = tid % W;
    const int PW = W + 2 * R, PH = TH + 2 * R;
    float acc[NOUT];
#pragma unroll
    for (int n = 0; n < NOUT; ++n) acc[n] = 0.f;
    const int K = KS * KS * C;
    constexpr int MAXP = F32IN ? 13 : 7, PPX = F32IN ? 8 : 4;
    const int npiece = PH * PW * PPX;
    float4 pre[F32IN ? MAXP : 2 * MAXP];
    auto fetch = [&](int c0) __attribute__((always_inline)) {
#pragma unroll
        for (int j = 0; j < MAXP; ++j) {
            const int i = min(tid + 256 * j, npiece - 1);
            const int piece = i % PPX, px = i / PPX, sy = px / PW, sx = px - sy * PW;
            const int iy = y0 + sy - R, ix = sx - R;
            const unsigned m = 0u - (unsigned)((tid + 256 * j < npiece) & (iy >= 0) & (iy < H) & (ix >= 0) & (ix < W));
            const int iyc = min(max(iy, 0), H - 1), ixc = min(max(ix, 0), W - 1);
            typedef unsigned u4n __attribute__((ext_vector_type(4)));
            if constexpr (F32IN) {
                const u4n raw = *(const u4n*)((const float*)x + (((size_t)b * H + iyc) * W + ixc) * (size_t)ldx + c0 + 4 * piece) & m;
                pre[j] = __builtin_bit_cast(float4, raw);
            } else {
                const u4n* src = (const u4n*)(x + (((size_t)b * H + iyc) * W + ixc) * (size_t)(2 * ldx) + 2 * c0 + 16 * piece);
                pre[2 * j] = __builtin_bit_cast(float4, src[0] & m);
                pre[2 * j + 1] = __builtin_bit_cast(float4, src[1] & m);
            }
        }
    };
    fetch(0);
    for (int c0 = 0; c0 < C; c0 += 32) {
        __syncthreads();
#pragma unroll
        for (int j = 0; j < MAXP; ++j) {
            const int i = tid + 256 * j;
            if (i >= npiece) continue;
            if constexpr (F32IN) {
                *(float4*)(nsm + (size_t)(i >> 3) * NRW_PITCH + 16 * (i & 7)) = pre[j];
            } else {
                typedef _Float16 h8v __attribute__((ext_vector_type(8)));
                const h8v hi = __builtin_bit_cast(h8v, pre[2 * j]), lo = __builtin_bit_cast(h8v, pre[2 * j + 1]);
                float4 a, c;
                a.x = (float)hi[0] + (float)lo[0]; a.y = (float)hi[1] + (float)lo[1]; a.z = (float)hi[2] + (float)lo[2]; a.w = (float)hi[3] + (float)lo[3];
                c.x = (float)hi[4] + (float)lo[4]; c.y = (float)hi[5] + (float)lo[5]; c.z = (float)hi[6] + (float)lo[6]; c.w = (float)hi[7] + (float)lo[7];
                unsigned char* d = nsm + (size_t)(i >> 2) * NRW_PITCH + 32 * (i & 3);
                *(float4*)d = a;
                *(float4*)(d + 16) = c;
            }
        }
        __syncthreads();
        if (c0 + 32 < C) fetch(c0 + 32);
#pragma unroll
        for (int dy = 0; dy < KS; ++dy)
#pragma unroll
            for (int dx = 0; dx < KS; ++dx) {
                const unsigned char* p = nsm + (size_t)((ty + dy) * PW + tx + dx) * NRW_PITCH;
                const float* wt = w + (dy * KS + dx) * C + c0;
#pragma unroll
                for (int g = 0; g < 8; ++g) {
                    const f4 xv = *(const f4*)(p + 16 * g);
#pragma unroll
                    for (int e = 0; e < 4; ++e)
#pragma unroll
                        for (int n = 0; n < NOUT; ++n) acc[n] = fmaf(xv[e], wt[n * K + 4 * g + e], acc[n]);
                }
            }
    }
    const size_t o = (((size_t)b * H + y0 + ty) * W + tx) * NOUT;
#pragma unroll
    for (int n = 0; n < NOUT; ++n) {
        float v = (F32IN ? acc[n] : acc[n] * (1.0f / PP_A_SCALE)) + (bias ? bias[n] : 0.f);
        if (residual) v += residual[o + n];
        out[o + n] = v;
    }
}

__global__ __launch_bounds__(256) void flow_operand_kernel(const float* __restrict__ flow, int ld_flow, long long rows, _Float16* __restrict__ op8,
                                                           int terms) {
    const long long p = (long long)blockIdx.x * 256 + threadIdx.x;
    if (p >= rows) return;
    const float* f = flow + p * ld_flow;
    _Float16 h0, l0, h1, l1;
    pp_split_f16_chk(f[0], h0, l0);
    pp_split_f16_chk(f[1], h1, l1);
    const _Float16 z = (_Float16)0.f;
    const h8_t hi = {h0, h1, z, z, z, z, z, z}, lo = {l0, l1, z, z, z, z, z, z};
    h8_t* o = (h8_t*)(op8 + p * 8 * terms);
    o[0] = hi;
    if (terms == 2) o[1] = lo;
}

constexpr int PO_TILE = 1024;
__global__ __launch_bounds__(256) void patch_operand_kernel(const float* __restrict__ bank, const long long* __restrict__ index, long long n_rows,
                                                            const float* __restrict__ front, int n_front, int HW, _Float16* __restrict__ out,
                                                            int terms) {
    __shared__ __attribute__((aligned(16))) float t[3][PO_TILE];
    const int j = blockIdx.y, tid = threadIdx.x;
    const float* src;
    if (j < n_front) {
        src = front + (size_t)j * 3 * HW;
    } else {
        const long long r = index[j - n_front];
        if (r < 0 || r >= n_rows) return;
        src = bank + (size_t)r * 3 * HW;
    }
    const int p0 = blockIdx.x * PO_TILE, np = min(PO_TILE, HW - p0);
    if ((HW & 3) == 0) {
        for (int i = tid; i < 3 * (np >> 2); i += 256) {
            const int c = i / (np >> 2), q = i - c * (np >> 2);
            *(f4*)&t[c][4 * q] = *(const f4*)(src + (size_t)c * HW + p0 + 4 * q);
        }
    } else {
        for (int i = tid; i < 3 * np; i += 256) {
            const int c = i / np, q = i - c * np;
            t[c][q] = src[(size_t)c * HW + p0 + q];
        }
    }
    __syncthreads();
    h8_t* o = (h8_t*)(out + ((size_t)j * HW + p0) * 8 * terms);
    const _Float16 z = (_Float16)0.f;
    for (int i = tid; i < np * terms; i += 256) {
        const int q = terms == 2 ? i >> 1 : i;
        _Float16 h0, l0, h1, l1, h2, l2;
        if (terms == 1 || (i & 1) == 0) {
            pp_split_f16_chk(t[0][q], h0, l0);
            pp_split_f16_chk(t[1][q], h1, l1);
            pp_split_f16_chk(t[2][q], h2, l2);
            o[i] = h8_t{h0, h1, h2, z, z, z, z, z};
        } else {
            pp_split_f16(t[0][q], h0, l0);
            pp_split_f16(t[1][q], h1, l1);
            pp_split_f16(t[2][q], h2, l2);
            o[i] = h8_t{l0, l1, l2, z, z, z, z, z};
        }
    }
}

}

PP_SAT_SETTER(pp_sat_set_sample)

extern "C" {

int pp_resize_bilinear_nhwc(const float* in, int B, int H, int W, int C, int Ho, int Wo, float mul, float* out,
                            void* stream) {
    if (!in || !out || B <= 0 || H <= 0 || W <= 0 || C <= 0 || Ho <= 0 || Wo <= 0) return PP_EINVAL;
    const bool vec = (C & 3) == 0 && (((uintptr_t)in | (uintptr_t)out) & 15) == 0;
    const int work = vec ? Wo * (C / 4) : Wo * C;
    const int gx = (work + 1023) / 1024;
    hipLaunchKernelGGL(resize_kernel, dim3(gx < 64 ? gx : 64, Ho, B), dim3(256), 0, (hipStream_t)stream, in, H, W,
                       C, Ho, Wo, mul, out, (_Float16*)nullptr, 2);
    return pp_last_launch();
}

int pp_resize_bilinear_nhwc_t(const float* in, int B, int H, int W, int C, int Ho, int Wo, float mul, void* out_hl,
                              int terms, void* stream) {
    if (!in || !out_hl || B <= 0 || H <= 0 || W <= 0 || C <= 0 || C % 8 != 0 || Ho <= 0 || Wo <= 0 ||
        (((uintptr_t)in | (uintptr_t)out_hl) & 15) != 0 || (terms != 1 && terms != 2))
        return PP_EINVAL;
    const int gx = (Wo * (C / 8) + 1023) / 1024;
    hipLaunchKernelGGL(resize_kernel, dim3(gx < 64 ? gx : 64, Ho, B), dim3(256), 0, (hipStream_t)stream, in, H, W,
                       C, Ho, Wo, mul, (float*)nullptr, (_Float16*)out_hl, terms);
    return pp_last_launch();
}

int pp_resize_bilinear_nhwc_dual(const float* in, int B, int H, int W, int C, int Ho, int Wo, float mul, float* out, void* out_hl,
                                 int terms, void* stream) {
    if (!in || !out || !out_hl || B <= 0 || H <= 0 || W <= 0 || C <= 0 || C % 8 != 0 || Ho <= 0 || Wo <= 0 ||
        (((uintptr_t)in | (uintptr_t)out | (uintptr_t)out_hl) & 15) != 0 || (terms != 1 && terms != 2))
        return PP_EINVAL;
    const int gx = (Wo * (C / 8) + 1023) / 1024;
    hipLaunchKernelGGL(resize_kernel, dim3(gx < 64 ? gx : 64, Ho, B), dim3(256), 0, (hipStream_t)stream, in, H, W,
                       C, Ho, Wo, mul, out, (_Float16*)out_hl, terms);
    return pp_last_launch();
}

int pp_resize_bilinear_nhwc_hl(const float* in, int B, int H, int W, int C, int Ho, int Wo, float mul, void* out_hl,
                               void* stream) {
    return pp_resize_bilinear_nhwc_t(in, B, H, W, C, Ho, Wo, mul, out_hl, 2, stream);
}

int pp_warp_nhwc(const float* feat, int feat_batch, const float* flow, int B, int H, int W, int C, int ld_flow,
                 float* out, int ld_out, void* stream) {
    if (!feat || !flow || !out || B <= 0 || H <= 0 || W <= 0 || C <= 0 || C % 4 != 0 || ld_flow < 2 || feat_batch <= 0 ||
        ld_out < C || ld_out % 4 != 0 || ((uintptr_t)out % 16) != 0)
        return PP_EINVAL;
    hipLaunchKernelGGL(warp_kernel<false>, dim3((H * W + 3) / 4, B), dim3(256), 0, (hipStream_t)stream, feat, feat_batch, flow,
                       H, W, C, ld_flow, out, ld_out, 2);
    return pp_last_launch();
}

int pp_warp_nhwc_t(const float* feat, int feat_batch, const float* flow, int B, int H, int W, int C, int ld_flow,
                   void* out_hl, int ld_h, int terms, void* stream) {
    if (!feat || !flow || !out_hl || B <= 0 || H <= 0 || W <= 0 || C <= 0 || C % 8 != 0 || ld_flow < 2 || feat_batch <= 0 ||
        ld_h < C || ld_h % 8 != 0 || ((uintptr_t)out_hl % 16) != 0 || (terms != 1 && terms != 2))
        return PP_EINVAL;
    hipLaunchKernelGGL(warp_kernel<true>, dim3((H * W + 3) / 4, B), dim3(256), 0, (hipStream_t)stream, feat, feat_batch, flow,
                       H, W, C, ld_flow, (float*)out_hl, ld_h, terms);
    return pp_last_launch();
}

int pp_warp_nhwc_hl(const float* feat, int feat_batch, const float* flow, int B, int H, int W, int C, int ld_flow,
                    void* out_hl, int ld_h, void* stream) {
    return pp_warp_nhwc_t(feat, feat_batch, flow, B, H, W, C, ld_flow, out_hl, ld_h, 2, stream);
}

int pp_avgpool2_nhwc(const float* in, int B, int H, int W, int C, float* out, void* stream) {
    if (!in || !out || B <= 0 || H < 2 || W < 2 || C <= 0 || H % 2 != 0 || W % 2 != 0) return PP_EINVAL;
    const size_t n = (size_t)(H / 2) * (W / 2) * C;
    const int gx = (int)((n + 255) / 256 < 1024 ? (n + 255) / 256 : 1024);
    hipLaunchKernelGGL(avgpool2_kernel, dim3(gx, B), dim3(256), 0, (hipStream_t)stream, in, H, W, C, out);
    return pp_last_launch();
}

static int corr_tiled_launch(bool hl, const void* f1, int ld_f1, const void* f2_l0, const void* f2_l1, const void* f2_l2, int f2_batch,
                             const float* flow, int B, int H, int W, int C, int levels, int radius, int ld_flow, float* out, int ld_out,
                             void* stream, bool exact = false, bool one = false) {
    const size_t lds = (size_t)(CM * CSP > (CM + CN) * CKP ? CM * CSP : (CM + CN) * CKP) * sizeof(float);
    static signed char attr[PP_MAX_DEVICES];
    signed char& ok = attr[pp_cur_device()];
    if (ok == 0)
        ok = hipFuncSetAttribute((const void*)corr_lookup_mfma_kernel<false>, hipFuncAttributeMaxDynamicSharedMemorySize, (int)lds) == hipSuccess &&
                     hipFuncSetAttribute((const void*)corr_lookup_mfma_kernel<true>, hipFuncAttributeMaxDynamicSharedMemorySize, (int)lds) == hipSuccess &&
                     hipFuncSetAttribute((const void*)corr_lookup_mfma_kernel<false, true>, hipFuncAttributeMaxDynamicSharedMemorySize, (int)lds) == hipSuccess &&
                     hipFuncSetAttribute((const void*)corr_lookup_mfma_kernel<false, false, true>, hipFuncAttributeMaxDynamicSharedMemorySize, (int)lds) == hipSuccess
                 ? 1 : -1;
    if (ok < 0) return PP_ELAUNCH;
    const dim3 grid((unsigned)((H / CT) * (W / CT) * B));
    if (exact)
        hipLaunchKernelGGL((corr_lookup_mfma_kernel<false, true>), grid, dim3(256), lds, (hipStream_t)stream, f1, ld_f1, f2_batch, f2_l0, f2_l1, f2_l2,
                           flow, B, H, W, C, levels, radius, ld_flow, 1.0f / sqrtf((float)C), out, ld_out);
    else if (one)
        hipLaunchKernelGGL((corr_lookup_mfma_kernel<false, false, true>), grid, dim3(256), lds, (hipStream_t)stream, f1, ld_f1, f2_batch, f2_l0, f2_l1,
                           f2_l2, flow, B, H, W, C, levels, radius, ld_flow, 1.0f / sqrtf((float)C), out, ld_out);
    else if (hl)
        hipLaunchKernelGGL(corr_lookup_mfma_kernel<true>, grid, dim3(256), lds, (hipStream_t)stream, f1, ld_f1, f2_batch, f2_l0, f2_l1, f2_l2,
                           flow, B, H, W, C, levels, radius, ld_flow, 1.0f / sqrtf((float)C), out, ld_out);
    else
        hipLaunchKernelGGL(corr_lookup_mfma_kernel<false>, grid, dim3(256), lds, (hipStream_t)stream, f1, ld_f1, f2_batch, f2_l0, f2_l1, f2_l2,
                           flow, B, H, W, C, levels, radius, ld_flow, 1.0f / sqrtf((float)C), out, ld_out);
    return pp_last_launch();
}

int pp_conv_narrow_f32(const float* x, int ld_x, int B, int H, int W, int C, const float* weight, const float* bias, int ksize,
                       int n_out, const float* residual, float* out, void* stream) {
    if (!x || !weight || !out || B <= 0 || H <= 0 || C <= 0 || C % 32 != 0 || ld_x < C || ld_x % 4 != 0) return PP_EINVAL;
    if ((W != 16 && W != 32 && W != 64) || H % (256 / W) != 0 || (ksize != 1 && ksize != 3) || (n_out != 1 && n_out != 2)) return PP_EINVAL;
    if (((uintptr_t)x % 16) != 0) return PP_EINVAL;
    const int TH = 256 / W, R = ksize / 2;
    const size_t lds = (size_t)(TH + 2 * R) * (W + 2 * R) * NRW_PITCH;
    const dim3 grid((unsigned)(B * (H / TH)));
    hipStream_t st = (hipStream_t)stream;
#define NRW_LAUNCH(KS_, N_)                                                                                                                  \
    hipLaunchKernelGGL((conv_narrow_kernel<KS_, N_, true>), grid, dim3(256), lds, st, (const _Float16*)x, ld_x, H, W, C, weight, bias, residual, out)
    if (ksize == 3 && n_out == 2) NRW_LAUNCH(3, 2);
    else if (ksize == 3) NRW_LAUNCH(3, 1);
    else if (n_out == 2) NRW_LAUNCH(1, 2);
    else NRW_LAUNCH(1, 1);
#undef NRW_LAUNCH
    return pp_last_launch();
}

int pp_corr_lookup_nhwc_ex(const float* f1, int ld_f1, const float* f2_l0, const float* f2_l1, const float* f2_l2,
                           int f2_batch, const float* flow, int B, int H, int W, int C, int levels, int radius,
                           int ld_flow, int prec, float* out, int ld_out, void* stream) {
    if (prec != PP_PREC_F32 && prec != PP_PREC_F16X3 && prec != PP_PREC_F16) return PP_EINVAL;
    if (!f1 || !f2_l0 || !flow || !out || B <= 0 || H <= 0 || W <= 0 || C <= 0 || C % 4 != 0) return PP_EINVAL;
    if (ld_f1 < C || ld_f1 % 4 != 0 || ((uintptr_t)f1 % 16) != 0 || f2_batch <= 0) return PP_EINVAL;
    if (levels < 1 || levels > MAXL || radius < 1 || radius > MAXR) return PP_EINVAL;
    if ((levels > 1 && !f2_l1) || (levels > 2 && !f2_l2)) return PP_EINVAL;
    if ((H >> (levels - 1)) < 1 || (W >> (levels - 1)) < 1 || ld_flow < 2) return PP_EINVAL;
    const int win = 2 * radius + 1;
    if (ld_out < levels * win * win) return PP_EINVAL;
    const char* te = getenv("PP_CORR_TILED");
    const bool tiled = !(te && te[0] == '0');
    const bool aligned = (((uintptr_t)f2_l0 | (levels > 1 ? (uintptr_t)f2_l1 : 0) | (levels > 2 ? (uintptr_t)f2_l2 : 0)) % 16) == 0;
    if (tiled && H % CT == 0 && W % CT == 0 && C % CK == 0 && aligned)
        return corr_tiled_launch(false, f1, ld_f1, f2_l0, f2_l1, f2_l2, f2_batch, flow, B, H, W, C, levels, radius, ld_flow, out, ld_out, stream,
                                 prec == PP_PREC_F32, prec == PP_PREC_F16);
    const size_t smem = (size_t)4 * (C + MAXL * TW * TW) * sizeof(float);
    hipLaunchKernelGGL(corr_lookup_kernel, dim3((H * W + 3) / 4, B), dim3(256), smem, (hipStream_t)stream, f1, ld_f1,
                       f2_batch, f2_l0, f2_l1, f2_l2, flow, H, W, C, levels, radius, ld_flow, 1.0f / sqrtf((float)C), out,
                       ld_out);
    return pp_last_launch();
}

int pp_corr_lookup_nhwc_hl(const void* f1_hl, int ld_f1, const void* f2_hl_l0, const void* f2_hl_l1, const void* f2_hl_l2,
                           int f2_batch, const float* flow, int B, int H, int W, int C, int levels, int radius, int ld_flow,
                           float* out, int ld_out, void* stream) {
    if (!f1_hl || !f2_hl_l0 || !flow || !out || B <= 0 || H <= 0 || W <= 0 || C <= 0 || f2_batch <= 0) return PP_EINVAL;
    if (H % CT != 0 || W % CT != 0 || C % CK != 0 || ld_f1 < C || ld_f1 % 8 != 0) return PP_EINVAL;
    if (((uintptr_t)f1_hl | (uintptr_t)f2_hl_l0 | (uintptr_t)f2_hl_l1 | (uintptr_t)f2_hl_l2) % 16 != 0) return PP_EINVAL;
    if (levels < 1 || levels > MAXL || radius < 1 || radius > MAXR) return PP_EINVAL;
    if ((levels > 1 && !f2_hl_l1) || (levels > 2 && !f2_hl_l2)) return PP_EINVAL;
    if ((H >> (levels - 1)) < 1 || (W >> (levels - 1)) < 1 || ld_flow < 2) return PP_EINVAL;
    const int win = 2 * radius + 1;
    if (ld_out < levels * win * win) return PP_EINVAL;
    return corr_tiled_launch(true, f1_hl, ld_f1, f2_hl_l0, f2_hl_l1, f2_hl_l2, f2_batch, flow, B, H, W, C, levels, radius, ld_flow, out, ld_out,
                             stream);
}

int pp_corr_lookup_nhwc(const float* f1, int ld_f1, const float* f2_l0, const float* f2_l1, const float* f2_l2,
                        int f2_batch, const float* flow, int B, int H, int W, int C, int levels, int radius,
                        int ld_flow, float* out, int ld_out, void* stream) {
    return pp_corr_lookup_nhwc_ex(f1, ld_f1, f2_l0, f2_l1, f2_l2, f2_batch, flow, B, H, W, C, levels, radius, ld_flow,
                                  PP_PREC_F16X3, out, ld_out, stream);
}

int pp_gather_rows(const float* src, const long long* index, long long n_src_rows, long long row_floats, int n, float* dst,
                   void* stream) {
    if (!src || !index || !dst || n <= 0 || n_src_rows <= 0 || row_floats <= 0 || row_floats % 4 != 0 ||
        ((uintptr_t)src % 16) != 0 || ((uintptr_t)dst % 16) != 0)
        return PP_EINVAL;
    const long long n4 = row_floats / 4;
    const int gx = (int)((n4 + 255) / 256 < 64 ? (n4 + 255) / 256 : 64);
    hipLaunchKernelGGL(gather_rows_kernel, dim3(gx, n), dim3(256), 0, (hipStream_t)stream, src, index, row_floats, n_src_rows,
                       dst);
    return pp_last_launch();
}

int pp_bank_rows_to_tokens(const float* bank, long long n_bank_rows, int C, int P, const long long* index, int n, float* tokens, int ld,
                           int T, int skip, void* stream) {
    if (!bank || !index || !tokens || n_bank_rows <= 0 || C <= 0 || P <= 0 || n <= 0 || ld < C || skip < 0 || T <= 0 ||
        (long long)skip + P > T)
        return PP_EINVAL;
    if (n > 65535 || (P + 31) / 32 > 65535) return PP_EINVAL;
    hipLaunchKernelGGL(bank_rows_to_tokens_kernel, dim3((C + 31) / 32, (P + 31) / 32, n), dim3(256), 0, (hipStream_t)stream, bank, index,
                       n_bank_rows, C, P, tokens, ld, T, skip);
    return pp_last_launch();
}

int pp_patch_operand(const float* bank, long long n_bank_rows, const long long* index, int n, const float* front, int n_front, int H, int W,
                     void* out, int terms, void* stream) {
    if (!out || n < 0 || n_front < 0 || n + n_front <= 0 || H <= 0 || W <= 0 || (terms != 1 && terms != 2)) return PP_EINVAL;
    if ((n > 0 && (!bank || !index || n_bank_rows <= 0)) || (n_front > 0 && !front)) return PP_EINVAL;
    if (((uintptr_t)out | (n > 0 ? (uintptr_t)bank : 0) | (n_front > 0 ? (uintptr_t)front : 0)) % 16 != 0) return PP_EINVAL;
    const long long hw = (long long)H * W, tiles = (hw + PO_TILE - 1) / PO_TILE;
    if (n + n_front > 65535 || hw > 0x7fffffff || tiles > 0x7fffffff) return PP_EINVAL;
    hipLaunchKernelGGL(patch_operand_kernel, dim3((unsigned)tiles, n + n_front), dim3(256), 0, (hipStream_t)stream, bank, index, n_bank_rows,
                       front, n_front, (int)hw, (_Float16*)out, terms);
    return pp_last_launch();
}

int pp_flow_operand(const float* flow, int ld_flow, long long rows, void* out8, int terms, void* stream) {
    if (!flow || !out8 || rows <= 0 || ld_flow < 2 || ((uintptr_t)out8 % 16) != 0 || (terms != 1 && terms != 2)) return PP_EINVAL;
    if ((rows + 255) / 256 > 0x7fffffff) return PP_EINVAL;
    hipLaunchKernelGGL(flow_operand_kernel, dim3((unsigned)((rows + 255) / 256)), dim3(256), 0, (hipStream_t)stream, flow, ld_flow, rows,
                       (_Float16*)out8, terms);
    return pp_last_launch();
}

int pp_saturation_take(unsigned int* word, unsigned int* slot, void* stream) {
    if (!word || !slot) return PP_EINVAL;
    hipLaunchKernelGGL(saturation_take_kernel, dim3(1), dim3(64), 0, (hipStream_t)stream, word, slot);
    return pp_last_launch();
}

int pp_crop_resize_normalize(const unsigned char* image, int H, int W, const unsigned char* mask, int y1, int y2, int x1,
                             int x2, int S, int rgb_mask_flag, const double* mean3, const double* std3, float* out_rgb,
                             float* out_mask, void* stream) {
    if (!image || !out_rgb || !mean3 || !std3 || H <= 0 || W <= 0 || S <= 0 || y1 < 0 || x1 < 0 || y2 > H || x2 > W ||
        y2 <= y1 || x2 <= x1)
        return PP_EINVAL;
    hipLaunchKernelGGL(crop_resize_kernel, dim3((S * S + 255) / 256), dim3(256), 0, (hipStream_t)stream, image, W, mask, y1, y2,
                       x1, x2, S, rgb_mask_flag, mean3[0], mean3[1], mean3[2], std3[0], std3[1], std3[2], out_rgb, out_mask);
    return pp_last_launch();
}

int pp_depth_points_nearest(const float* depth_m, int H, int W, int y1, int y2, int x1, int x2, int P, float fx, float fy,
                            float cx, float cy, float* out_pts, void* stream) {
    if (!depth_m || !out_pts || H <= 0 || W <= 0 || P <= 0 || y1 < 0 || x1 < 0 || y2 > H || x2 > W || y2 <= y1 || x2 <= x1 ||
        fx == 0.f || fy == 0.f)
        return PP_EINVAL;
    hipLaunchKernelGGL(depth_points_kernel, dim3((P * P + 255) / 256), dim3(256), 0, (hipStream_t)stream, depth_m, W, y1, y2, x1,
                       x2, P, fx, fy, cx, cy, out_pts);
    return pp_last_launch();
}

int pp_conv_narrow_hl(const void* x_hl, int ld_x, int B, int H, int W, int C, const float* weight, const float* bias, int ksize,
                      int n_out, const float* residual, float* out, void* stream) {
    if (!x_hl || !weight || !out || B <= 0 || H <= 0 || C <= 0 || C % 32 != 0 || ld_x < C || ld_x % 8 != 0) return PP_EINVAL;
    if ((W != 16 && W != 32 && W != 64) || H % (256 / W) != 0 || (ksize != 1 && ksize != 3) || (n_out != 1 && n_out != 2)) return PP_EINVAL;
    if (((uintptr_t)x_hl % 16) != 0) return PP_EINVAL;
    const int TH = 256 / W, R = ksize / 2;
    const size_t lds = (size_t)(TH + 2 * R) * (W + 2 * R) * NRW_PITCH;
    const dim3 grid((unsigned)(B * (H / TH)));
    hipStream_t st = (hipStream_t)stream;
#define NRW_LAUNCH(KS_, N_)                                                                                                        \
    hipLaunchKernelGGL((conv_narrow_kernel<KS_, N_>), grid, dim3(256), lds, st, (const _Float16*)x_hl, ld_x, H, W, C, weight, bias, \
                       residual, out)
    if (ksize == 3 && n_out == 2) NRW_LAUNCH(3, 2);
    else if (ksize == 3) NRW_LAUNCH(3, 1);
    else if (n_out == 2) NRW_LAUNCH(1, 2);
    else NRW_LAUNCH(1, 1);
#undef NRW_LAUNCH
    return pp_last_launch();
}

}
```

### picopose_amd/model/stage3.py

```python
import os

import torch
import torch.nn as nn

from .. import ops
from .common import Holder, Packed, bn_p, conv_p, convT_p, fold_bn, seq


COMPUTE_DEAD_LAYER1 = os.environ.get("PP_DPT_DEAD_LAYER1", "0") == "1"
OUT_CONV_FIRST = os.environ.get("PP_DPT_OUT_CONV_FIRST", "1") != "0"


def _rcu(c):
    m = Holder()
    m.conv1, m.conv2 = conv_p(c, c, 3), conv_p(c, c, 3)
    m.bn1, m.bn2 = bn_p(c), bn_p(c)
    return m


def _fusion(c):
    m = Holder()
    m.out_conv = conv_p(c, c, 1)
    m.resConfUnit1, m.resConfUnit2 = _rcu(c), _rcu(c)
    return m


class DPTHead(Packed):
    def __init__(self, nclass, in_channels, features=256, use_bn=False, out_channels=(256, 512, 1024, 1024),
                 use_clstoken=False):
        super().__init__()
        oc = list(out_channels)
        self.projects = nn.ModuleList([conv_p(in_channels, c, 1) for c in oc])
        self.resize_layers = seq((0, convT_p(oc[0], oc[0], 4)), (1, convT_p(oc[1], oc[1], 2)), (3, conv_p(oc[3], oc[3], 3)))
        s = Holder()
        for i in range(4):
            setattr(s, f"layer{i + 1}_rn", conv_p(oc[i], features, 3, bias=False))
        for i in range(4):
            setattr(s, f"refinenet{i + 1}", _fusion(features))
        s.output_conv1 = conv_p(features, features // 2, 3)
        s.output_conv2 = seq((0, conv_p(features // 2, 32, 3)), (2, conv_p(32, 1, 1)))
        self.scratch = s

    def _pack(self):
        pk = {}
        for i, p in enumerate(self.projects):
            pk[f"proj{i}"] = ops.pack_conv_weight(p.weight.float())
        r = self.resize_layers
        pk["up0"], pk["up0_b"] = ops.pack_convT_weight(getattr(r, "0").weight.float(), getattr(r, "0").bias.float())
        pk["up1"], pk["up1_b"] = ops.pack_convT_weight(getattr(r, "1").weight.float(), getattr(r, "1").bias.float())
        pk["down3"] = ops.pack_conv_weight(getattr(r, "3").weight.float())
        for i in range(4):
            pk[f"rn{i + 1}"] = ops.pack_conv_weight(getattr(self.scratch, f"layer{i + 1}_rn").weight.float())
        for i in (2, 3, 4):
            f = getattr(self.scratch, f"refinenet{i}")
            pk[f"f{i}_out"] = ops.pack_conv_weight(f.out_conv.weight.float())
            for j in (1, 2):
                u = getattr(f, f"resConfUnit{j}")
                for c in (1, 2):
                    w, b = fold_bn(getattr(u, f"conv{c}").weight.float(), getattr(u, f"conv{c}").bias.float(),
                                   getattr(u, f"bn{c}"))
                    pk[f"f{i}_u{j}_c{c}"], pk[f"f{i}_u{j}_b{c}"] = ops.pack_conv_weight(w), b.contiguous()
        return pk

    def _pack_train(self):
        pk = {}
        for i in (2, 3, 4):
            f = getattr(self.scratch, f"refinenet{i}")
            for j in (1, 2):
                u = getattr(f, f"resConfUnit{j}")
                for c in (1, 2):
                    pk[f"f{i}_u{j}_c{c}"] = ops.pack_conv_weight(getattr(u, f"conv{c}").weight.float())
        return pk

    def _rcu_train(self, i, j, x, extra=None):
        u, pkt = getattr(getattr(self.scratch, f"refinenet{i}"), f"resConfUnit{j}"), self.packed_train()
        h = ops.conv2d(x, pkt[f"f{i}_u{j}_c1"], u.conv1.bias, 3, pad=1, relu_in=True)
        h = ops.batchnorm_train(h, u.bn1, relu=True)
        h = ops.conv2d(h, pkt[f"f{i}_u{j}_c2"], u.conv2.bias, 3, pad=1)
        return ops.batchnorm_train(h, u.bn2, residual=x, residual2=extra)

    def _rcu(self, pk, key, x, extra=None, more=False, operand_only=False):
        xin = getattr(x, "_hl_relu", None)
        h = ops.conv2d(x if xin is None else xin, pk[key + "_c1"], pk[key + "_b1"], 3, pad=1, relu_in=xin is None,
                       out_split=True, split_relu=True, wino_next="relu")
        return ops.conv2d(h, pk[key + "_c2"], pk[key + "_b2"], 3, pad=1, relu_in=not isinstance(h, (ops.Split, ops.WinoInput)), residual=x,
                          residual2=extra, also_split="relu" if more else None, out_split=operand_only)

    def _fuse(self, pk, i, size, x0, x1=None, train=False, operand_only=False):
        if train:
            out = x0 if x1 is None else self._rcu_train(i, 1, x1, extra=x0)
            out = self._rcu_train(i, 2, out)
        else:
            out = x0 if x1 is None else self._rcu(pk, f"f{i}_u1", x1, extra=x0, more=True)
            if OUT_CONV_FIRST:
                out = self._rcu(pk, f"f{i}_u2", out, operand_only=True)
                out = ops.conv2d(out, pk[f"f{i}_out"], getattr(self.scratch, f"refinenet{i}").out_conv.bias, 1)
                return ops.resize_bilinear(out, size[0], size[1], **(dict(out_split=True) if operand_only else dict(also_split=True)))
            out = self._rcu(pk, f"f{i}_u2", out)
        out = ops.resize_bilinear(out, size[0], size[1], out_split=True)
        return ops.conv2d(out, pk[f"f{i}_out"], getattr(self.scratch, f"refinenet{i}").out_conv.bias, 1, also_split="plain")

    def forward_nhwc(self, feats, train=False, finest_operand_only=False):
        pk, r = self.packed(for_training=train), self.resize_layers
        live = range(4) if COMPUTE_DEAD_LAYER1 else range(1, 4)
        x = {i: ops.conv2d(feats[i], pk[f"proj{i}"], self.projects[i].bias, 1, out_split=True) for i in live}
        _, H0, W0, _ = feats[0].shape
        size1 = (4 * H0, 4 * W0)
        l2 = ops.conv_transpose2d(x[1], pk["up1"], pk["up1_b"], 2, out_split=True)
        l3 = x[2]
        l4 = ops.conv2d(x[3], pk["down3"], getattr(r, "3").bias, 3, stride=2, pad=1, out_split=True)
        rn = {i: ops.conv2d(l, pk[f"rn{i + 1}"], None, 3, pad=1, also_split="relu", wino=i in (1, 2)) for i, l in ((1, l2), (2, l3), (3, l4))}
        if COMPUTE_DEAD_LAYER1:
            l1 = ops.conv_transpose2d(x[0], pk["up0"], pk["up0_b"], 4, out_split=True)
            rn[0] = ops.conv2d(l1, pk["rn1"], None, 3, pad=1, also_split="relu")
            assert tuple(rn[0].shape[1:3]) == size1
        p4 = self._fuse(pk, 4, rn[2].shape[1:3], rn[3], train=train)
        p3 = self._fuse(pk, 3, rn[1].shape[1:3], p4, rn[2], train)
        p2 = self._fuse(pk, 2, size1, p3, rn[1], train, operand_only=finest_operand_only and not train and ops.decoder_lean())
        if train:
            self.bn_moved()
        return [p4, p3, p2]

    def forward(self, out_features):
        with torch.no_grad():
            return [ops.to_nchw(p) for p in self.forward_nhwc([ops.to_nhwc(f) for f in out_features])]


def _cm(cin, cout, k):
    m = Holder()
    m.conv = conv_p(cin, cout, k)
    return m


def _motion_encoder(levels, radius):
    m = Holder()
    m.corr_net = seq((0, _cm(levels * (2 * radius + 1) ** 2, 256, 1)), (1, _cm(256, 192, 3)))
    m.flow_net = seq((0, _cm(2, 128, 7)), (1, _cm(128, 64, 3)))
    m.out_net = seq((0, _cm(256, 126, 3)))
    return m


FUSE_XHEADS = os.environ.get("PP_FUSE_XHEADS", "0") == "1"


def _xhead(cin, kind):
    m = Holder()
    m.layers = seq((0, _cm(cin, 512, 3)), (1, _cm(512, 256, 3)))
    m.predict_layer = conv_p(256, 2, 3) if kind == "flow" else conv_p(256, 1, 1)
    return m


class FlowDecoder(Packed):
    def __init__(self, num_levels, radius):
        super().__init__()
        self.num_levels, self.radius = num_levels, radius
        self.r = int(radius / 2)
        self.proj = nn.ModuleList([seq((0, conv_p(256, 256, 1)), (1, bn_p(256))) for _ in range(num_levels)])
        self.encoder = nn.ModuleList([_motion_encoder(l + 1, self.r) for l in range(num_levels)])
        self.flow_pred = nn.ModuleList([_xhead(640, "flow") for _ in range(num_levels)])
        self.mask_pred = nn.ModuleList([_xhead(640, "mask") for _ in range(num_levels)])

    def _pack(self):
        pk = {}
        for l in range(self.num_levels):
            w, b = fold_bn(getattr(self.proj[l], "0").weight.float(), getattr(self.proj[l], "0").bias.float(),
                           getattr(self.proj[l], "1"))
            pk[f"proj{l}"], pk[f"proj{l}_b"] = ops.pack_conv_weight(w), b.contiguous()
            e = self.encoder[l]
            for name, net in (("corr", e.corr_net), ("flow", e.flow_net), ("out", e.out_net)):
                for idx, sub in net.named_children():
                    w = sub.conv.weight.float()
                    pad = -(-w.shape[1] // 8) * 8 if w.shape[1] % 8 else None
                    pk[f"e{l}_{name}{idx}"] = ops.pack_conv_weight(w, cin_pad=pad)
            w126 = pk[f"e{l}_out0"]
            pk[f"e{l}_out0_128"] = torch.cat([w126, w126.new_zeros(2, w126.shape[1])]).contiguous()
            b126 = getattr(e.out_net, "0").conv.bias.float()
            pk[f"e{l}_out0_b128"] = torch.cat([b126, b126.new_zeros(2)]).contiguous()
            for name, head in (("fp", self.flow_pred[l]), ("mp", self.mask_pred[l])):
                for idx, sub in head.layers.named_children():
                    pk[f"{name}{l}_{idx}"] = ops.pack_conv_weight(sub.conv.weight.float())
                pk[f"{name}{l}_p"] = ops.pack_conv_weight(head.predict_layer.weight.float())
            pk[f"x{l}_0"] = torch.cat([pk[f"fp{l}_0"], pk[f"mp{l}_0"]]).contiguous()
            pk[f"x{l}_0_b"] = torch.cat([getattr(self.flow_pred[l].layers, "0").conv.bias.float(),
                                         getattr(self.mask_pred[l].layers, "0").conv.bias.float()]).contiguous()
        return pk

    def _pack_train(self):
        return {f"proj{l}": ops.pack_conv_weight(getattr(self.proj[l], "0").weight.float()) for l in range(self.num_levels)}

    def forward_nhwc(self, feat_render_list, feat_real_list, flow, cert, train=False):
        pkt = self.packed_train() if train else None
        pk = self.packed(for_training=train)
        flows, certs = [], []
        lean = ops.decoder_lean() and not train
        for l in range(self.num_levels):
            fr_in, fq_in = feat_render_list[l], feat_real_list[l]
            B, H, W = fr_in.image if isinstance(fr_in, ops.Split) else fr_in.shape[:3]
            opcat = ops.presplit()
            dev = fr_in.device
            if opcat:
                Xs = ops.Split.empty(B * H * W, 640, dev)
                Xs.image = (B, H, W)
                X = None
            else:
                X = torch.empty(B, H, W, 640, dtype=torch.float32, device=dev)
            e = self.encoder[l]
            fr_src = getattr(fr_in, "_hl", fr_in)
            if train:
                pj = self.proj[l]
                fr = ops.batchnorm_train(ops.conv2d(fr_src, pkt[f"proj{l}"], getattr(pj, "0").bias, 1), getattr(pj, "1"))
                fq = ops.batchnorm_train(ops.conv2d(getattr(fq_in, "_hl", fq_in), pkt[f"proj{l}"], getattr(pj, "0").bias, 1), getattr(pj, "1"))
                if opcat:
                    ops.split_activation(fr, B, H * W, 256, H * W * 256, 256, into=(Xs, 0))
                else:
                    X[..., 0:256] = fr
            else:
                fq = ops.conv2d(getattr(fq_in, "_hl", fq_in), pk[f"proj{l}"], pk[f"proj{l}_b"], 1, also_split="plain" if opcat else None)
            hl_maps = dict(f1_hl=(Xs, 0), f2_hl=getattr(fq, "_hl", None)) if opcat and not train and ops.terms() == 2 else {}
            if not train and opcat:
                fr_dead = lean and bool(hl_maps) and ops.corr_takes_operands(hl_maps["f1_hl"], hl_maps["f2_hl"], H, W, 256)
                fr = ops.conv2d(fr_src, pk[f"proj{l}"], pk[f"proj{l}_b"], 1, hl_into=(Xs, 0),
                                out=None if fr_dead else torch.empty(B, H, W, 256, dtype=torch.float32, device=dev))
            elif not train:
                fr = ops.conv2d(fr_src, pk[f"proj{l}"], pk[f"proj{l}_b"], 1, out=X[..., 0:256])
            ncorr = (l + 1) * (2 * self.r + 1) ** 2
            corr = ops.corr_lookup(fr, fq, flow, l + 1, self.r, c_pad=-(-ncorr // 8) * 8, **hl_maps)
            hl_cat = opcat
            if hl_cat:
                cf = ops.Split.empty(B * H * W, 256, dev)
                cf.image = (B, H, W)
            else:
                cf = torch.empty(B, H, W, 256, dtype=torch.float32, device=dev)
            c1 = ops.conv2d(corr, pk[f"e{l}_corr0"], getattr(e.corr_net, "0").conv.bias, 1, act="relu", out_split=True)
            ops.conv2d(c1, pk[f"e{l}_corr1"], getattr(e.corr_net, "1").conv.bias, 3, pad=1, act="relu",
                       **(dict(hl_into=(cf, 0)) if hl_cat else dict(out=cf[..., 0:192])))
            if lean and opcat:
                flow8 = ops.flow_operand(flow)
            else:
                flow8 = torch.zeros(B, H, W, 8, dtype=torch.float32, device=dev)
                flow8[..., 0:2] = flow
            f1 =ops.conv2d(flow8, pk[f"e{l}_flow0"], getattr(e.flow_net, "0").conv.bias, 7, pad=3, act="relu", out_split=True)
            ops.conv2d(f1, pk[f"e{l}_flow1"], getattr(e.flow_net, "1").conv.bias, 3, pad=1, act="relu",
                       **(dict(hl_into=(cf, 192)) if hl_cat else dict(out=cf[..., 192:256])))
            if opcat:
                ops.conv2d(cf, pk[f"e{l}_out0_128"], pk[f"e{l}_out0_b128"], 3, pad=1, act="relu", hl_into=(Xs, 512))
                ops.hl_patch_columns(flow[..., 0:2] if lean else (flow[..., 0:2].contiguous() if flow.shape[-1] != 2 else flow), Xs, 638)
                ops.warp(fq, flow, hl_into=(Xs, 256))
            else:
                ops.conv2d(cf, pk[f"e{l}_out0"], getattr(e.out_net, "0").conv.bias, 3, pad=1, act="relu", out=X[..., 512:638])
                X[..., 638:640] = flow
                ops.warp(fq, flow, out=X[..., 256:512])
                Xs = ops.split_image(X)
            fp, mp = self.flow_pred[l], self.mask_pred[l]
            if FUSE_XHEADS and isinstance(Xs, ops.Split) and B * H * W * 1024 * 2 * Xs.terms < 0xFFFFFF00:
                hx = ops.conv2d(Xs, pk[f"x{l}_0"], pk[f"x{l}_0_b"], 3, pad=1, act="relu", out_split=True)
                h = ops.conv2d(hx, pk[f"fp{l}_1"], getattr(fp.layers, "1").conv.bias, 3, pad=1, act="relu", out_split=True, in_cols=(0, 512))
                flow = ops.conv2d(h, pk[f"fp{l}_p"], fp.predict_layer.bias, 3, pad=1, residual=flow)
                h = ops.conv2d(hx, pk[f"mp{l}_1"], getattr(mp.layers, "1").conv.bias, 3, pad=1, act="relu", out_split=True, in_cols=(512, 512))
                cert = ops.conv2d(h, pk[f"mp{l}_p"], mp.predict_layer.bias, 1, residual=cert)
            else:
                Xs = ops.winograd_shared(Xs, cout=512)
                if isinstance(Xs, ops.WinoInput4):
                    hf, hm = ops.conv2d_wino_pair(Xs, (pk[f"fp{l}_0"], getattr(fp.layers, "0").conv.bias), (pk[f"mp{l}_0"], getattr(mp.layers, "0").conv.bias),
                                                  act="relu", out_split=True, wino_next=True)
                else:
                    hf = ops.conv2d(Xs, pk[f"fp{l}_0"], getattr(fp.layers, "0").conv.bias, 3, pad=1, act="relu", out_split=True, wino=True, wino_next=True)
                    hm = ops.conv2d(Xs, pk[f"mp{l}_0"], getattr(mp.layers, "0").conv.bias, 3, pad=1, act="relu", out_split=True, wino=True, wino_next=True)
                h = ops.conv2d(hf, pk[f"fp{l}_1"], getattr(fp.layers, "1").conv.bias, 3, pad=1, act="relu", out_split=True, wino=True)
                flow = ops.conv2d(h, pk[f"fp{l}_p"], fp.predict_layer.bias, 3, pad=1, residual=flow)
                h = ops.conv2d(hm, pk[f"mp{l}_1"], getattr(mp.layers, "1").conv.bias, 3, pad=1, act="relu", out_split=True, wino=True)
                cert = ops.conv2d(h, pk[f"mp{l}_p"], mp.predict_layer.bias, 1, residual=cert)
            flows.append(flow)
            certs.append(cert)
            if l != self.num_levels - 1:
                flow = ops.resize_bilinear(flow, 2 * H, 2 * W, mul=2.0)
                cert = ops.resize_bilinear(cert, 2 * H, 2 * W)
        if train:
            self.bn_moved()
        return flows, certs

    def forward(self, feat_render_list, feat_real_list, init_flow, init_certainty, iters=1):
        assert iters == 1
        with torch.no_grad():
            fl, ce = self.forward_nhwc([ops.to_nhwc(f) for f in feat_render_list], [ops.to_nhwc(f) for f in feat_real_list],
                                       ops.to_nhwc(init_flow), ops.to_nhwc(init_certainty))
            return [ops.to_nchw(f) for f in fl], [ops.to_nchw(c) for c in ce]


class OffsetRegressor(nn.Module):
    def __init__(self, cfg):
        super().__init__()
        self.dpt_head = DPTHead(cfg.nclass, cfg.in_channels, features=256, use_bn=True,
                                out_channels=[256, 512, 1024, 1024], use_clstoken=False)
        self.flow_decoder = FlowDecoder(cfg.num_levels, cfg.radius)

    def forward_nhwc(self, feats_tem, feats_real, init_flow, init_cert, train=False):
        tem = self.dpt_head.forward_nhwc(feats_tem, train)
        real = self.dpt_head.forward_nhwc(feats_real, train)
        return self.flow_decoder.forward_nhwc(tem, real, init_flow, init_cert, train)

    def forward(self, features_tem, features_real, init_flow, init_certainty):
        return self.flow_decoder(self.dpt_head(features_tem), self.dpt_head(features_real), init_flow, init_certainty)
```

### picopose_amd/ops.py

```python
import contextlib
import ctypes
import os
import threading

import torch

from . import _lib
from ._lib import PpGemmDesc

ACT = {None: 0, "none": 0, "relu": 1, "gelu": 2, "leaky01": 3, "tanh": 4}

PRECISION = "f16x3"
_PREC = {"f32": 0, "f16x3": 1, "f16": 2}
_split_cache = {}
_scope = threading.local()


def precision():
    return getattr(_scope, "mode", None) or PRECISION


def check_precision(mode):
    if mode is not None and mode not in _PREC:
        raise ValueError(f"unknown arithmetic mode {mode!r}: expected None or one of {sorted(_PREC)}")
# ... 734 lines not shown
    key = (wp.data_ptr(), tuple(wp.shape), "wino4")
    hit = _wino_cache.get(key)
    if hit is None or hit[2] != wp._version:
        Cout = wp.shape[0]
        V = hit[0] if hit is not None else torch.empty(36 * Cout, cin, dtype=torch.float32, device=wp.device)
        hl = hit[3] if hit is not None else torch.empty(36 * Cout, 2 * cin, dtype=torch.float16, device=wp.device)
        _lib.check(_lib.lib().pp_winograd4_weight_f32(_p(wp), Cout, cin, wp.shape[1], _p(V), _lib.stream_ptr()), "pp_winograd4_weight_f32")
        scale = torch.empty(1, dtype=torch.float32, device=wp.device)
        _lib.check(_lib.lib().pp_split_weights_t(_p(V), V.numel(), 2, _p(hl), _p(scale), _lib.stream_ptr()), "pp_split_weights_t")
        if len(_wino_cache) > 1024:
            _wino_cache.clear()
        hit = _wino_cache[key] = (V, wp, wp._version, hl, float(scale.item()))
    return hit[0], hit[3], hit[4]


def _winograd4_input(src_ptr, ld_x, B, H, W, cin, dev):
    P = B * (H // 4) * (W // 4)
    Pp = _wino4_rows(P)
    U = Split((torch.empty if Pp == P else torch.zeros)(36 * Pp, 2 * cin, dtype=torch.float16, device=dev), 2)
    _lib.check(_lib.lib().pp_winograd4_input_hl(src_ptr, ld_x, H * W * ld_x, B, H, W, cin, 0, _p(U.hl), Pp, _lib.stream_ptr()), "pp_winograd4_input_hl")
    _chk(U.hl, "pp_winograd4_input_hl")
    return U


WINO4_CHAIN = os.environ.get("PP_WINOGRAD4_CHAIN", "1") != "0"
WINO4_CHAIN_WIDTHS = (32, 64)


def _wino4_products(U, V, vhl, vscale, Pp, cin, N):
    Y = torch.empty(36, Pp, N, dtype=torch.float32, device=U.device)
    per = max(1, min(WINO4_GROUPS_PER_LAUNCH, 0xF0000000 // (4 * Pp * max(cin, N))))
    for x0 in range(0, 36, per):
        n = min(per, 36 - x0)
        _run(_desc(A_hl=U.hl.data_ptr() + x0 * Pp * cin * 4, B=_p(V), B_hl=vhl.data_ptr() + x0 * N * cin * 4, b_scale=vscale, C=_p(Y[x0]),
                   M=Pp, N=N, K=cin, lda=cin, ldb=cin, ldc=N, prec=_PREC["f16x3"], batch0=n, a_bs0=Pp * cin, b_bs0=N * cin,
                   c_bs0=Pp * N, alpha=PP_A_SCALE / WINO4_U_SCALE, _keep=(U, vhl, V)))
    return Y


def _wino4_finish(Y, col0, ldy, bias, B, H, W, Cout, act, residual, residual2, out, out_split, split_relu, also_split, chain_next):
    P = B * (H // 4) * (W // 4)
    Pp, dev, L = _wino4_rows(P), Y.device, _lib.lib()
    yp = Y.data_ptr() + 4 * col0
    ret, hl_t, ldc = None, None, 0
    if (chain_next and WINO4_CHAIN and out_split and out is None and residual is None and residual2 is None and W in WINO4_CHAIN_WIDTHS and Cout % 32 == 0
            and _winograd4_ok(B, H, W, Cout, Cout)):
        U1 = Split((torch.empty if Pp == P else torch.zeros)(36 * Pp, 2 * Cout, dtype=torch.float16, device=dev), 2)
        _lib.check(L.pp_winograd4_chain(yp, ldy, B, H, W, Cout, _p(bias), ACT[act], int(split_relu), _p(U1.hl), Pp, _lib.stream_ptr()), "pp_winograd4_chain")
        _chk(U1.hl, "pp_winograd4_chain")
        return WinoInput4(U1, (B, H, W, Cout), None)
    if out_split and out is None and residual is None and residual2 is None:
        hl_t = Split.empty(B * H * W, Cout, dev)
        hl_t.image = (B, H, W)
        ret, c_relu = hl_t, int(split_relu)
    else:
        if out is None:
            out = torch.empty(B, H, W, Cout, dtype=torch.float32, device=dev)
        ldc = out.stride(2)
        assert out.stride(3) == 1 and out.stride(1) == W * ldc and out.stride(0) == H * W * ldc
        for r_ in (residual, residual2):
            if r_ is not None:
                assert r_.stride() == out.stride()
        ret, c_relu = out, 0
        if also_split is not None and out.is_contiguous():
            hl_t = Split.empty(B * H * W, Cout, dev)
            hl_t.image = (B, H, W)
            c_relu = int(also_split == "relu")
            setattr(out, "_hl_relu" if also_split == "relu" else "_hl", hl_t)
    _lib.check(L.pp_winograd4_output(yp, ldy, B, H, W, Cout, _p(bias), ACT[act], _p(residual), _p(residual2), _p(out), ldc,
                                     _p(hl_t.hl) if hl_t is not None else None, Cout, c_relu, Pp, _lib.stream_ptr()), "pp_winograd4_output")
    if hl_t is not None:
        _chk(hl_t.hl, "pp_winograd4_output")
    return ret


def _conv3x3_winograd4(x, wp, bias, B, H, W, cin, Cout, act, residual, residual2, out, out_split, split_relu, also_split, chain_next=False):
    P = B * (H // 4) * (W // 4)
    V, vhl, vscale = winograd4_weight(wp, cin)
    if isinstance(x, WinoInput4):
        assert x.geom == (B, H, W, cin)
        U = x.U
    elif isinstance(x, tuple):
        U = _winograd4_input(x[0].col_ptr(x[1]), x[0].shape[1], B, H, W, cin, x[0].device)
    else:
        U = _winograd4_input(x.hl.data_ptr(), x.shape[1], B, H, W, cin, x.device)
    Pp = _wino4_rows(P)
    assert U.hl.shape[0] == 36 * Pp
    Y = _wino4_products(U, V, vhl, vscale, Pp, cin, Cout)
    return _wino4_finish(Y, 0, Cout, bias, B, H, W, Cout, act, residual, residual2, out, out_split, split_relu, also_split, chain_next)


WINO4_PAIR = os.environ.get("PP_WINOGRAD4_PAIR", "1") != "0"


def winograd4_weight_pair(wp_a, wp_b, cin):
    key = (wp_a.data_ptr(), wp_b.data_ptr(), tuple(wp_a.shape), tuple(wp_b.shape), "wino4pair")
    hit = _wino_cache.get(key)
    if hit is None or hit[2] != (wp_a._version, wp_b._version):
        Va, Vb = winograd4_weight(wp_a, cin)[0], winograd4_weight(wp_b, cin)[0]
        Ca, Cb = wp_a.shape[0], wp_b.shape[0]
        V = torch.cat([Va.view(36, Ca, cin), Vb.view(36, Cb, cin)], dim=1).reshape(36 * (Ca + Cb), cin).contiguous()
        hl = torch.empty(V.shape[0], 2 * cin, dtype=torch.float16, device=V.device)
        scale = torch.empty(1, dtype=torch.float32, device=V.device)
        _lib.check(_lib.lib().pp_split_weights_t(_p(V), V.numel(), 2, _p(hl), _p(scale), _lib.stream_ptr()), "pp_split_weights_t")
        hit = _wino_cache[key] = (V, (wp_a, wp_b), (wp_a._version, wp_b._version), hl, float(scale.item()))
    return hit[0], hit[3], hit[4]


def conv2d_wino_pair(x, layer_a, layer_b, act=None, out_split=False, split_relu=False, wino_next=False):
    (wa, ba), (wb, bb) = layer_a, layer_b
    kw = dict(act=act, out_split=out_split, split_relu=split_relu, wino=True, wino_next=wino_next)
    src = x.src if isinstance(x, WinoInput4) else x
    if not (WINO4_PAIR and isinstance(x, (WinoInput4, Split)) and out_split):
        return conv2d(x, wa, ba, 3, pad=1, **kw), conv2d(x, wb, bb, 3, pad=1, **kw)
    if isinstance(x, WinoInput4):
        B, H, W, cin = x.geom
    else:
        (B, H, W), cin = src.image, src.shape[1]
    Ca, Cb = wa.shape[0], wb.shape[0]
    if not (_winograd4_ok(B, H, W, cin, Ca) and _winograd4_ok(B, H, W, cin, Cb) and wa.shape[1] == 9 * cin == wb.shape[1] and Ca % 8 == 0):
        return conv2d(x, wa, ba, 3, pad=1, **kw), conv2d(x, wb, bb, 3, pad=1, **kw)
    P = B * (H // 4) * (W // 4)
    Pp = _wino4_rows(P)
    U = x.U if isinstance(x, WinoInput4) else _winograd4_input(src.hl.data_ptr(), cin, B, H, W, cin, src.device)
    V, vhl, vscale = winograd4_weight_pair(wa, wb, cin)
    Y = _wino4_products(U, V, vhl, vscale, Pp, cin, Ca + Cb)
    fin = lambda col0, C, bias: _wino4_finish(Y, col0, Ca + Cb, bias, B, H, W, C, act, None, None, None, out_split, split_relu, None, wino_next)
    return fin(0, Ca, ba), fin(Ca, Cb, bb)


def conv_transpose2d(x, wp, bias_tiled, r, out_split=False):
    xs = x if isinstance(x, Split) else None
    if xs is not None:
        (B, H, W), Cin = xs.image, xs.shape[1]
    else:
        B, H, W, Cin = x.shape
        assert x.is_contiguous()
    Cout = wp.shape[0] // (r * r)
    wargs = _weight_args(wp, Cin)
    dev = xs.device if xs is not None else x.device
    if xs is not None or ("B_hl" in wargs and _can_presplit(x, Cin, Cin) and x.numel() < 2 ** 31):
        assert "B_hl" in wargs
        hl = xs.hl if xs is not None else split_activation(x, 1, B * H * W, Cin, 0, Cin)
        if out_split and _split_ok(Cout):
            sp = Split.empty(B * H * r * W * r, Cout, dev)
            sp.image = (B, H * r, W * r)
            _run(_desc(A_hl=_p(hl), B=_p(wp), C=None, bias=_p(bias_tiled), M=B * H * W, N=r * r * Cout, K=Cin,
                       lda=Cin, ldb=Cin, ldc=Cout, shuffle_r=r, shuffle_h=H, shuffle_w=W, C_hl=_p(sp.hl), ldc_h=Cout, **wargs),
                 written=sp)
            return sp
        out = torch.empty(B, H * r, W * r, Cout, dtype=torch.float32, device=dev)
        _run(_desc(A_hl=_p(hl), B=_p(wp), C=_p(out), bias=_p(bias_tiled), M=B * H * W, N=r * r * Cout, K=Cin,
                   lda=Cin, ldb=Cin, ldc=Cout, shuffle_r=r, shuffle_h=H, shuffle_w=W, **wargs))
        return out
    out = torch.empty(B, H * r, W * r, Cout, dtype=torch.float32, device=x.device)
    _run(_desc(A=_p(x), B=_p(wp), C=_p(out), bias=_p(bias_tiled), M=B * H * W, N=r * r * Cout, K=Cin, lda=Cin, ldb=Cin,
               ldc=Cout, shuffle_r=r, shuffle_h=H, shuffle_w=W, **_fly_args(wargs, wp)))
    return out


def attention(qkv, B, T, heads, hd, out_split=False):
    sp = out = None
    dev = qkv.device
    if out_split and _split_ok(heads * hd):
        sp = Split.empty(B * T, heads * hd, dev)
    else:
        out = torch.empty(B * T, heads * hd, dtype=torch.float32, device=dev)
    if isinstance(qkv, Split):
        _lib.check(_lib.lib().pp_attention_t(_p(qkv.hl), qkv.terms, B, T, heads, hd, float(hd) ** -0.5, _p(out),
                                             _p(sp.hl) if sp else None, _lib.stream_ptr()), "pp_attention_t")
    else:
        assert qkv.is_contiguous()
        if sp is not None and sp.terms == 1:
            sp, out = None, torch.empty(B * T, heads * hd, dtype=torch.float32, device=dev)
        _lib.check(_lib.lib().pp_attention_ex(_p(qkv), B, T, heads, hd, float(hd) ** -0.5, _fly_prec(), _p(out),
                                              _p(sp.hl) if sp else None, _lib.stream_ptr()), "pp_attention_ex")
    if sp is not None:
        _chk(sp.hl, "pp_attention")
    return sp if sp is not None else out


def layernorm(x, weight, bias, eps, out_split=False):
    rows, C = x.shape
    assert x.is_contiguous()
    if out_split and _split_ok(C):
        sp = Split.empty(rows, C, x.device)
        _lib.check(_lib.lib().pp_layernorm_t(_p(x), _p(weight), _p(bias), rows, C, float(eps), None, _p(sp.hl), sp.terms,
                                             _lib.stream_ptr()), "pp_layernorm_t")
        _chk(sp.hl, "pp_layernorm_t")
        return sp
    y = torch.empty_like(x)
    _lib.check(_lib.lib().pp_layernorm(_p(x), _p(weight), _p(bias), rows, C, float(eps), _p(y), _lib.stream_ptr()),
               "pp_layernorm")
    return y


def softmax_rows_(x):
    assert x.is_contiguous()
    n = x.shape[-1]
    _lib.check(_lib.lib().pp_softmax_rows(_p(x), x.numel() // n, n, n, _lib.stream_ptr()), "pp_softmax_rows")
    return x


def groupnorm(x, weight, bias, groups, eps=1e-5, relu=False):
    B, H, W, C = x.shape
    assert x.is_contiguous()
    y = torch.empty_like(x)
    _lib.check(_lib.lib().pp_groupnorm_nhwc(_p(x), _p(weight), _p(bias), B, H * W, C, groups, float(eps), int(relu),
                                            _p(y), _lib.stream_ptr()), "pp_groupnorm_nhwc")
    return y


def batchnorm_train(x, bn, relu=False, residual=None, residual2=None, eps=1e-5, momentum=0.1):
    assert x.is_contiguous() and x.dtype == torch.float32
    C = x.shape[-1]
    rows = x.numel() // C
    L = _lib.lib()
    nbytes = L.pp_batchnorm_train_workspace_bytes(rows, C)
    ws = torch.empty(nbytes, dtype=torch.uint8, device=x.device)
    y = torch.empty_like(x)
    for r in (residual, residual2):
        assert r is None or (r.is_contiguous() and r.shape == x.shape)
    _lib.check(L.pp_batchnorm_train(_p(x), _p(bn.weight), _p(bn.bias), rows, C, float(eps), float(momentum), _p(bn.running_mean),
                                    _p(bn.running_var), int(relu), _p(residual) if residual is not None else None,
                                    _p(residual2) if residual2 is not None else None, _p(y), _p(ws), nbytes, _lib.stream_ptr()),
               "pp_batchnorm_train")
    bn.num_batches_tracked += 1
    return y


def to_nhwc(x, c_pad=None):
    B, C, H, W = x.shape
    x = x.contiguous().float()
    Cp = c_pad if c_pad and c_pad > C else C
    out = (torch.zeros if Cp > C else torch.empty)(B, H, W, Cp, dtype=torch.float32, device=x.device)
    _lib.check(_lib.lib().pp_transpose_batched(_p(x), 0, B, C, H * W, _p(out), 0, Cp, 0, _lib.stream_ptr()),
               "pp_transpose_batched")
    return out


def to_nchw(x):
    B, H, W, C = x.shape
    assert x.is_contiguous()
    out = torch.empty(B, C, H, W, dtype=torch.float32, device=x.device)
    _lib.check(_lib.lib().pp_transpose_batched(_p(x), 0, B, H * W, C, _p(out), 0, H * W, 0, _lib.stream_ptr()),
               "pp_transpose_batched")
    return out


def resize_bilinear(x, Ho, Wo, mul=1.0, out_split=False, also_split=False):
    B, H, W, C = x.shape
    assert x.is_contiguous()
    if also_split and _split_ok(C) and x.data_ptr() % 16 == 0:
        out = torch.empty(B, Ho, Wo, C, dtype=torch.float32, device=x.device)
        sp = Split.empty(B * Ho * Wo, C, x.device)
        sp.image = (B, Ho, Wo)
        _lib.check(_lib.lib().pp_resize_bilinear_nhwc_dual(_p(x), B, H, W, C, Ho, Wo, float(mul), _p(out), _p(sp.hl), sp.terms,
                                                            _lib.stream_ptr()), "pp_resize_bilinear_nhwc_dual")
        _chk(sp.hl, "pp_resize_bilinear_nhwc_dual")
        out._hl = sp
        return out
    if out_split and _split_ok(C) and x.data_ptr() % 16 == 0:
        sp = Split.empty(B * Ho * Wo, C, x.device)
        sp.image = (B, Ho, Wo)
        _lib.check(_lib.lib().pp_resize_bilinear_nhwc_t(_p(x), B, H, W, C, Ho, Wo, float(mul), _p(sp.hl), sp.terms, _lib.stream_ptr()),
                   "pp_resize_bilinear_nhwc_t")
        _chk(sp.hl, "pp_resize_bilinear_nhwc_t")
        return sp
    out = torch.empty(B, Ho, Wo, C, dtype=torch.float32, device=x.device)
    _lib.check(_lib.lib().pp_resize_bilinear_nhwc(_p(x), B, H, W, C, Ho, Wo, float(mul), _p(out), _lib.stream_ptr()),
               "pp_resize_bilinear_nhwc")
    return out


def warp(feat, flow, out=None, hl_into=None):
    B, H, W = flow.shape[:3]
    Bf, Hf, Wf, C = feat.shape
    assert (Hf, Wf) == (H, W) and B % Bf == 0
    assert feat.is_contiguous() and flow.stride(3) == 1 and flow.stride(2) * W == flow.stride(1)
    if hl_into is not None:
        tgt, col0 = hl_into
        ctot = tgt.shape[1]
        assert tgt.shape[0] == B * H * W and col0 % 8 == 0 and col0 + C <= ctot and C % 8 == 0
        _lib.check(_lib.lib().pp_warp_nhwc_t(_p(feat), Bf, _p(flow), B, H, W, C, flow.stride(2), tgt.col_ptr(col0),
                                             ctot, tgt.terms, _lib.stream_ptr()), "pp_warp_nhwc_t")
        if CHECK_SATURATION:
            _chk(tgt.cols(col0, C), "pp_warp_nhwc_t")
        return None
    if out is None:
        out = torch.empty(B, H, W, C, dtype=torch.float32, device=feat.device)
    _lib.check(_lib.lib().pp_warp_nhwc(_p(feat), Bf, _p(flow), B, H, W, C, flow.stride(2), _p(out), out.stride(2),
                                       _lib.stream_ptr()), "pp_warp_nhwc")
    return out


def avgpool2(x):
    B, H, W, C = x.shape
    assert x.is_contiguous()
    out = torch.empty(B, H // 2, W // 2, C, dtype=torch.float32, device=x.device)
    _lib.check(_lib.lib().pp_avgpool2_nhwc(_p(x), B, H, W, C, _p(out), _lib.stream_ptr()), "pp_avgpool2_nhwc")
    return out


def decoder_lean():
    return os.environ.get("PP_DECODER_LEAN", "1") != "0"


def corr_takes_operands(f1_hl, f2_hl, H, W, C):
    return (f1_hl is not None and f2_hl is not None and precision() == "f16x3" and f2_hl.terms == 2 and H % 8 == 0 and W % 8 == 0 and C % 32 == 0
            and os.environ.get("PP_CORR_TILED", "1") != "0" and os.environ.get("PP_CORR_HL", "1") != "0")


def corr_lookup(f1, f2, flow, levels, radius, c_pad=None, f1_hl=None, f2_hl=None):
    (H, W, C), B = f2.shape[1:], flow.shape[0]
    assert f2.is_contiguous() and flow.stride(3) == 1 and B % f2.shape[0] == 0 and tuple(flow.shape[1:3]) == (H, W)
    operands = corr_takes_operands(f1_hl, f2_hl, H, W, C)
    if f1 is None:
        assert operands, "corr_lookup without the fp32 map f1 needs the operand form of both maps (corr_takes_operands)"
    else:
        assert tuple(f1.shape) == (B, H, W, C) and f1.stride(3) == 1 and f1.stride(1) == W * f1.stride(2) and f1.stride(0) == H * f1.stride(1)
    pyr = [f2]
    for _ in range(levels - 1):
        pyr.append(avgpool2(pyr[-1]))
    n = levels * (2 * radius + 1) ** 2
    np_ = c_pad if c_pad and c_pad > n else n
    out = (torch.zeros if np_ > n and not decoder_lean() else torch.empty)(B, H, W, np_, dtype=torch.float32, device=f2.device)
    if operands:
        tgt, col0 = f1_hl
        assert tgt.shape[0] == B * H * W and col0 % 8 == 0 and col0 + C <= tgt.shape[1] and f2_hl.shape == (f2.shape[0] * H * W, C)
        hls = [f2_hl.hl] + [split_activation(p, p.shape[0], p.shape[1] * p.shape[2], C, p.shape[1] * p.shape[2] * C, C) for p in pyr[1:]]
        _lib.check(_lib.lib().pp_corr_lookup_nhwc_hl(tgt.hl.data_ptr() + 4 * col0, tgt.shape[1], _p(hls[0]), _p(hls[1]) if levels > 1 else None,
                                                     _p(hls[2]) if levels > 2 else None, f2.shape[0], _p(flow), B, H, W, C, levels, radius,
                                                     flow.stride(2), _p(out), np_, _lib.stream_ptr()), "pp_corr_lookup_nhwc_hl")
        return out
    _lib.check(_lib.lib().pp_corr_lookup_nhwc_ex(_p(f1), f1.stride(2), _p(pyr[0]), _p(pyr[1]) if levels > 1 else None,
                                                 _p(pyr[2]) if levels > 2 else None, f2.shape[0], _p(flow), B, H, W, C,
                                                 levels, radius, flow.stride(2), 2 if precision() == "f16" else _fly_prec(), _p(out), np_,
                                                 _lib.stream_ptr()), "pp_corr_lookup_nhwc_ex")
    return out


def tokens_to_nchw(tokens, skip, H, W):
    B, T, C = tokens.shape
    assert tokens.is_contiguous()
    out = torch.empty(B, C, H, W, dtype=torch.float32, device=tokens.device)
    src = tokens[:, skip:]
    _lib.check(_lib.lib().pp_transpose_batched(_p(src), T * C, B, H * W, C, _p(out), 0, H * W, 0, _lib.stream_ptr()),
               "pp_transpose_batched")
    return out


def assemble_tokens(patches, cls_token, pos):
    B, T, C = patches.shape
    assert patches.is_contiguous() and pos.is_contiguous() and cls_token.is_contiguous()
    out = torch.empty(B, T + 1, C, dtype=torch.float32, device=patches.device)
    _lib.check(_lib.lib().pp_assemble_tokens(_p(patches), _p(cls_token), _p(pos), B, T, C, _p(out), _lib.stream_ptr()),
               "pp_assemble_tokens")
    return out


def normalize_rows(x, eps=1e-12):
    rows, n = x.shape
    assert x.is_contiguous()
    y = torch.empty_like(x)
    _lib.check(_lib.lib().pp_normalize_rows(_p(x), rows, n, float(eps), _p(y), _lib.stream_ptr()), "pp_normalize_rows")
    return y


def gather_rows(src, index):
    R = src.shape[0]
    row = src[0].numel()
    if row % 4 != 0 or not src.is_contiguous() or src.dtype != torch.float32 or src.data_ptr() % 16 != 0:
        return src[index]
    index = index.contiguous()
    dst = torch.empty((index.numel(),) + tuple(src.shape[1:]), dtype=torch.float32, device=src.device)
    _lib.check(_lib.lib().pp_gather_rows(_p(src), _p(index), R, row, index.numel(), _p(dst), _lib.stream_ptr()),
               "pp_gather_rows")
    return dst


def bank_rows_to_tokens(bank, index, T, skip=1, out=None):
    R, C = bank.shape[:2]
    P = bank[0, 0].numel()
    n = index.numel()
    assert bank.is_contiguous() and bank.dtype == torch.float32 and index.dtype == torch.int64 and index.device == bank.device
    if out is None:
        out = torch.empty(n * T, C, dtype=torch.float32, device=bank.device)
    assert out.dim() == 2 and out.dtype == torch.float32 and out.shape[0] == n * T and out.shape[1] >= C and out.stride(1) == 1 and out.device == bank.device
    _lib.check(_lib.lib().pp_bank_rows_to_tokens(_p(bank), R, C, P, _p(index.contiguous()), n, _p(out), out.stride(0), T, skip,
                                                 _lib.stream_ptr()), "pp_bank_rows_to_tokens")
    return out
```

Measured before the change: 584.6.

## Fuse f16 split into avgpool pyramid and corr lookup output, add ring-buffered corr kernel

Adds an avgpool2 kernel that writes the two-term f16 split form directly, which removes the separate split_activation pass for each pyramid level and skips the f32 copy for the last level. The correlation lookup kernel can now write its output already split into hi/lo f16 operands, so the following conv no longer needs its own split kernel. It also adds a new correlation kernel that streams operands into LDS through a staged buffer-load ring with MFMA. Together these reduce launches and memory traffic in the stage-3 decoder, at the cost of more code paths and more complex output layout handling.

```diff
diff --git a/include/picopose_hip.h b/include/picopose_hip.h
--- a/include/picopose_hip.h
+++ b/include/picopose_hip.h
@@ -248,6 +248,10 @@
 int pp_corr_lookup_nhwc_hl(const void* f1_hl, int ld_f1, const void* f2_hl_l0, const void* f2_hl_l1, const void* f2_hl_l2,
                            int f2_batch, const float* flow, int B, int H, int W, int C, int levels, int radius, int ld_flow,
                            float* out, int ld_out, void* stream);
+int pp_corr_lookup_nhwc_hl_op(const void* f1_hl, int ld_f1, const void* f2_hl_l0, const void* f2_hl_l1, const void* f2_hl_l2,
+                              int f2_batch, const float* flow, int B, int H, int W, int C, int levels, int radius, int ld_flow,
+                              float* out, int ld_out, void* out_hl, int ld_out_h, void* stream);
+int pp_avgpool2_hl(const float* in, int B, int H, int W, int C, float* out, void* out_hl, void* stream);
 
 int pp_pnp_ransac(const float* tar_pts_2d, const float* src_pts_3d, const float* K, const float* tem_pose,
                   const int64_t* tar_pts, const int64_t* src_pts, int P, int H, int W, int N, int iterations,
diff --git a/picopose_amd/_lib.py b/picopose_amd/_lib.py
--- a/picopose_amd/_lib.py
+++ b/picopose_amd/_lib.py
@@ -158,6 +158,8 @@
         L.pp_corr_lookup_nhwc.argtypes = [vp, i32, vp, vp, vp, i32, vp, i32, i32, i32, i32, i32, i32, i32, vp, i32, vp]
         L.pp_corr_lookup_nhwc_ex.argtypes = [vp, i32, vp, vp, vp, i32, vp, i32, i32, i32, i32, i32, i32, i32, i32, vp, i32, vp]
         L.pp_corr_lookup_nhwc_hl.argtypes = [vp, i32, vp, vp, vp, i32, vp, i32, i32, i32, i32, i32, i32, i32, vp, i32, vp]
+        L.pp_corr_lookup_nhwc_hl_op.argtypes = [vp, i32, vp, vp, vp, i32, vp, i32, i32, i32, i32, i32, i32, i32, vp, i32, vp, i32, vp]
+        L.pp_avgpool2_hl.argtypes = [vp, i32, i32, i32, i32, vp, vp, vp]
         L.pp_pnp_ransac.argtypes = [vp, vp, vp, vp, vp, vp, i32, i32, i32, i32, i32, f32, vp, vp, vp, vp, vp, vp]
         L.pp_pnp_ransac_debug.argtypes = [vp, vp, vp, vp, vp, vp, i32, i32, i32, i32, i32, f32, vp, vp, vp, vp, vp, vp, vp]
         L.pp_pnp_ransac_refine.argtypes = [vp, vp, vp, vp, vp, vp, i32, i32, i32, i32, i32, f32, i32, c.c_double] + [vp] * 10
diff --git a/picopose_amd/csrc/pp_sample.hip b/picopose_amd/csrc/pp_sample.hip
--- a/picopose_amd/csrc/pp_sample.hip
+++ b/picopose_amd/csrc/pp_sample.hip
@@ -158,6 +158,34 @@
     }
 }
 
+__global__ __launch_bounds__(256) void avgpool2_hl_kernel(const float* __restrict__ in, int H, int W, int C, float* __restrict__ out,
+                                                          _Float16* __restrict__ out_hl) {
+    const int Ho = H / 2, Wo = W / 2, b = blockIdx.y, C4 = C >> 2;
+    const size_t n4 = (size_t)Ho * Wo * C4;
+    const float* ib = in + (size_t)b * H * W * C;
+    for (size_t i = (size_t)blockIdx.x * 256 + threadIdx.x; i < n4; i += (size_t)gridDim.x * 256) {
+        const int c = (int)(i % C4) * 4;
+        const size_t q = i / C4;
+        const int ox = (int)(q % Wo), oy = (int)(q / Wo);
+        const float* p = ib + ((size_t)(2 * oy) * W + 2 * ox) * C + c;
+        const f4 p0 = *(const f4*)p, p1 = *(const f4*)(p + C), p2 = *(const f4*)(p + (size_t)W * C), p3 = *(const f4*)(p + (size_t)W * C + C);
+        f4 v;
+#pragma unroll
+        for (int k = 0; k < 4; ++k) v[k] = ((p0[k] + p1[k]) + (p2[k] + p3[k])) * 0.25f;
+        const size_t row = (size_t)b * Ho * Wo + q;
+        if (out) *(f4*)(out + row * C + c) = v;
+        _Float16 h0, h1, h2, h3, l0, l1, l2, l3;
+        pp_split_f16_chk(v[0], h0, l0);
+        pp_split_f16_chk(v[1], h1, l1);
+        pp_split_f16_chk(v[2], h2, l2);
+        pp_split_f16_chk(v[3], h3, l3);
+        _Float16* o = out_hl + row * 2 * (size_t)C + pp_hl_col(c, 0);
+        typedef _Float16 h4w __attribute__((ext_vector_type(4)));
+        *(h4w*)o = h4w{h0, h1, h2, h3};
+        *(h4w*)(o + 8) = h4w{l0, l1, l2, l3};
+    }
+}
+
 constexpr int MAXR = 2, TW = 2 * MAXR + 2, MAXL = 3;
 __global__ __launch_bounds__(256) void corr_lookup_kernel(const float* __restrict__ f1, int ld_f1,
                                                           int f2_batch, const float* __restrict__ f2l0,
@@ -239,12 +267,25 @@
 constexpr int CSP = CN + 4;
 typedef float f32x16_t __attribute__((ext_vector_type(16)));
 
+__device__ __forceinline__ void corr_put(float* __restrict__ out, _Float16* __restrict__ out_hl, size_t row, int ld_out, int ch, float v) {
+    if (out_hl) {
+        _Float16 h, l;
+        pp_split_f16_chk(v, h, l);
+        _Float16* q = out_hl + row * 2 * (size_t)ld_out + pp_hl_col(ch, 0);
+        q[0] = h;
+        q[8] = l;
+    } else {
+        out[row * ld_out + ch] = v;
+    }
+}
+
 template <bool HLIN, bool EXACT = false, bool ONE = false>
 __global__ __launch_bounds__(256, 2) void corr_lookup_mfma_kernel(const void* __restrict__ f1v, int ld_f1, int f2_batch,
                                                                   const void* __restrict__ f2l0, const void* __restrict__ f2l1,
                                                                   const void* __restrict__ f2l2, const float* __restrict__ flow,
                                                                   int B, int H, int W, int C, int L, int r, int ld_flow,
-                                                                  float inv_sqrt_c, float* __restrict__ out, int ld_out) {
+                                                                  float inv_sqrt_c, float* __restrict__ out, int ld_out,
+                                                                  _Float16* __restrict__ out_hl) {
     extern __shared__ __attribute__((aligned(16))) float sm[];
     float* As = sm;
     float* Bs = sm + CM * CKP;
@@ -267,7 +308,7 @@
     }
     for (int npad = ld_out - L * win * win, idx = tid; idx < CM * npad; idx += 256) {
         const int m = idx / npad, o = idx - m * npad;
-        out[((size_t)b * H * W + (size_t)(y0 + (m >> 3)) * W + x0 + (m & 7)) * ld_out + L * win * win + o] = 0.f;
+        corr_put(out, out_hl, (size_t)b * H * W + (size_t)(y0 + (m >> 3)) * W + x0 + (m & 7), ld_out, L * win * win + o, 0.f);
     }
     for (int l = 0; l < L; ++l) {
         const int Hl = H >> l, Wl = W >> l;
@@ -292,7 +333,7 @@
         for (int idx = tid; idx < CM * win * win; idx += 256) {
             const int m = idx / (win * win), o = idx - m * (win * win);
             if (s_state[m] == 2)
-                out[((size_t)b * H * W + (size_t)(y0 + (m >> 3)) * W + x0 + (m & 7)) * ld_out + l * win * win + o] = 0.f;
+                corr_put(out, out_hl, (size_t)b * H * W + (size_t)(y0 + (m >> 3)) * W + x0 + (m & 7), ld_out, l * win * win + o, 0.f);
         }
         while (s_todo > 0) {
             if (tid == 0) { s_ox = 0x7fffffff; s_oy = 0x7fffffff; }
@@ -432,8 +473,8 @@
                     const float cx = s_cx[m], cy = s_cy[m];
                     const float wx1 = cx - floorf(cx), wy1 = cy - floorf(cy), wx0 = 1.f - wx1, wy0 = 1.f - wy1;
                     const float* t = S + m * CSP + (dy + bi) * CRW + dx + ai;
-                    out[((size_t)b * H * W + (size_t)(y0 + (m >> 3)) * W + x0 + (m & 7)) * ld_out + l * win * win + o] =
-                        t[0] * (wx0 * wy0) + t[1] * (wx1 * wy0) + t[CRW] * (wx0 * wy1) + t[CRW + 1] * (wx1 * wy1);
+                    corr_put(out, out_hl, (size_t)b * H * W + (size_t)(y0 + (m >> 3)) * W + x0 + (m & 7), ld_out, l * win * win + o,
+                             t[0] * (wx0 * wy0) + t[1] * (wx1 * wy0) + t[CRW] * (wx0 * wy1) + t[CRW + 1] * (wx1 * wy1));
                 }
             }
             __syncthreads();
@@ -448,6 +489,208 @@
         }
         __syncthreads();
     }
+}
+
+constexpr int RK = 16, RROW = 2 * RK;
+constexpr int RP = 512 / RROW, LPR = 64 / RP;
+constexpr int RST = 2;
+constexpr int RG0_W = 16, RG0_N = 256, RG1_W = 11, RG1_N = 128, RG2_W = 11, RG2_N = 128;
+constexpr int corr_ring_nb(int rw) { return (rw * rw + 31) / 32; }
+constexpr size_t corr_ring_bytes(int rw, int nrp) {
+    const size_t ring = (size_t)RST * (CM + nrp) * RROW * 2, s = (size_t)(CM / 2) * (corr_ring_nb(rw) * 32 + 4) * 4;
+    return ring > s ? ring : s;
+}
+constexpr size_t CORR_RING_LDS = corr_ring_bytes(RG0_W, RG0_N);
+static_assert(corr_ring_bytes(RG1_W, RG1_N) <= CORR_RING_LDS && corr_ring_bytes(RG2_W, RG2_N) <= CORR_RING_LDS, "level 0 sizes the LDS");
+static_assert(corr_ring_nb(RG0_W) * 32 <= RG0_N && corr_ring_nb(RG1_W) * 32 <= RG1_N && corr_ring_nb(RG2_W) * 32 <= RG2_N, "S columns are staged rows");
+static_assert(RG0_N % (4 * RP) == 0 && RG1_N % (4 * RP) == 0 && RG2_N % (4 * RP) == 0 && CM % (4 * RP) == 0, "whole DMA pieces per wave");
+
+#if defined(__HIP_DEVICE_COMPILE__)
+typedef __attribute__((address_space(3))) void* corr_lds_ptr_t;
+
+template <int RW, int NRP>
+__device__ __forceinline__ void corr_ring_level(float* sm, float* s_cx, float* s_cy, int* s_bx, int* s_by, int* s_state, int* s_org, int l,
+                                                const _Float16* f1b, int ld_f1, int f1_bytes, const _Float16* f2b, int Hl, int Wl, int C,
+                                                float gx, float gy, int r, float inv_sqrt_c, size_t row0, int y0, int x0, int W,
+                                                float* __restrict__ out, _Float16* __restrict__ out_hl, int ld_out) {
+    constexpr int NB = corr_ring_nb(RW), NT = (2 * NB + 3) / 4;
+    constexpr int PA = CM / RP / 4, PB = NRP / RP / 4, NP = PA + PB;
+    constexpr int STG = (CM + NRP) * RROW;
+    constexpr int SP = NB * 32 + 4;
+    _Float16* ring = (_Float16*)sm;
+    float* S = sm;
+    const int tid = threadIdx.x, lane = tid & 63, wv = __builtin_amdgcn_readfirstlane(tid >> 6), l31 = lane & 31, lh = lane >> 5;
+    const int tw = 2 * r + 2, win = 2 * r + 1, fit = RW - tw;
+    if (tid == 0) s_org[2] = 0;
+    __syncthreads();
+    if (tid < CM) {
+        const float sc = (float)(1 << l);
+        const float cx = fminf(fmaxf(roundtrip(gx / sc, Wl), -1.0e6f), 1.0e6f);
+        const float cy = fminf(fmaxf(roundtrip(gy / sc, Hl), -1.0e6f), 1.0e6f);
+        const int bx = (int)floorf(cx) - r, by = (int)floorf(cy) - r;
+        s_cx[tid] = cx; s_cy[tid] = cy; s_bx[tid] = bx; s_by[tid] = by;
+        const bool outside = bx >= Wl || by >= Hl || bx + tw <= 0 || by + tw <= 0;
+        s_state[tid] = outside ? 2 : 0;
+        if (!outside) atomicAdd(&s_org[2], 1);
+    }
+    __syncthreads();
+    for (int idx = tid; idx < CM * win * win; idx += 256) {
+        const int m = idx / (win * win), o = idx - m * (win * win);
+        if (s_state[m] == 2) corr_put(out, out_hl, row0 + (size_t)(y0 + (m >> 3)) * W + x0 + (m & 7), ld_out, l * win * win + o, 0.f);
+    }
+    const int lr = lane / LPR, sc = (lane % LPR) ^ ((lr >> 2) & 3);
+    const __amdgpu_buffer_rsrc_t Ar = __builtin_amdgcn_make_buffer_rsrc((void*)f1b, 0, f1_bytes, 0x00020000);
+    const __amdgpu_buffer_rsrc_t Br = __builtin_amdgcn_make_buffer_rsrc((void*)f2b, 0, Hl * Wl * C * 4, 0x00020000);
+    unsigned abyte[PA];
+#pragma unroll
+    for (int j = 0; j < PA; ++j) {
+        const int ma = (j * 4 + wv) * RP + lr;
+        abyte[j] = (unsigned)(((y0 + (ma >> 3)) * W + x0 + (ma & 7)) * ld_f1) * 4u + (unsigned)sc * 16u;
+    }
+    const int ns = C / RK;
+    const int ph = ((2 * lh) ^ ((l31 >> 2) & 3)) * 8, pl = ph ^ 8;
+    while (s_org[2] > 0) {
+        if (tid == 0) { s_org[0] = 0x7fffffff; s_org[1] = 0x7fffffff; }
+        __syncthreads();
+        if (tid < CM && s_state[tid] == 0) atomicMin(&s_org[0], s_bx[tid]);
+        __syncthreads();
+        if (tid < CM && s_state[tid] == 0 && s_bx[tid] - s_org[0] <= fit) atomicMin(&s_org[1], s_by[tid]);
+        __syncthreads();
+        const int ox = s_org[0], oy = s_org[1];
+        unsigned bbyte[PB];
+#pragma unroll
+        for (int j = 0; j < PB; ++j) {
+            const int n = (j * 4 + wv) * RP + lr, ry = n / RW, qy = oy + ry, qx = ox + n - ry * RW;
+            const bool in = n < RW * RW && qx >= 0 && qx < Wl && qy >= 0 && qy < Hl;
+            bbyte[j] = in ? (unsigned)((qy * Wl + qx) * C) * 4u + (unsigned)sc * 16u : 0xFFFFFFFFu;
+        }
+#define CORR_RING_ISSUE(STEP, STAGE)                                                                                                \
+        {                                                                                                                               \
+            const unsigned dead_ = (STEP) < ns ? 0u : 0xFFFFFFFFu;                                                                      \
+            const int so_ = (STEP) * (RK * 4);                                                                                          \
+            _Float16* st_ = ring + (STAGE) * STG;                                                                                       \
+            _Pragma("unroll") for (int j = 0; j < PA; ++j)                                                                              \
+                __builtin_amdgcn_raw_ptr_buffer_load_lds(Ar, (corr_lds_ptr_t)(st_ + (j * 4 + wv) * RP * RROW), 16, abyte[j] | dead_,    \
+                                                         so_, 0, 0);                                                                    \
+            _Pragma("unroll") for (int j = 0; j < PB; ++j)                                                                              \
+                __builtin_amdgcn_raw_ptr_buffer_load_lds(Br, (corr_lds_ptr_t)(st_ + (CM + (j * 4 + wv) * RP) * RROW), 16,               \
+                                                         bbyte[j] | dead_, so_, 0, 0);                                                  \
+        }
+        f32x16_t acc[NT];
+#pragma unroll
+        for (int i = 0; i < NT; ++i)
+#pragma unroll
+            for (int e = 0; e < 16; ++e) acc[i][e] = 0.f;
+        asm volatile("s_waitcnt vmcnt(0)" ::: "memory");
+#pragma unroll
+        for (int s = 0; s < RST - 1; ++s) CORR_RING_ISSUE(s, s)
+        int cur = 0;
+        for (int s = 0; s < ns; ++s) {
+            asm volatile("s_waitcnt vmcnt(%0)" ::"n"((RST - 2) * NP) : "memory");
+            __builtin_amdgcn_s_barrier();
+            const int nxt = cur == 0 ? RST - 1 : cur - 1;
+            CORR_RING_ISSUE(s + RST - 1, nxt)
+            const _Float16* sa = ring + cur * STG;
+            const _Float16* sb = sa + CM * RROW;
+#pragma unroll
+            for (int i = 0; i < NT; ++i) {
+                const int t = wv + 4 * i;
+                if ((2 * NB) % 4 == 0 || t < 2 * NB) {
+                    const int m = t / NB, n = t - m * NB;
+                    const _Float16* ar = sa + (m * 32 + l31) * RROW;
+                    const _Float16* br = sb + (n * 32 + l31) * RROW;
+                    const h8_t ah = *(const h8_t*)(ar + ph), al = *(const h8_t*)(ar + pl);
+                    const h8_t bh = *(const h8_t*)(br + ph), bl = *(const h8_t*)(br + pl);
+                    acc[i] = __builtin_amdgcn_mfma_f32_32x32x16_f16(ah, bh, acc[i], 0, 0, 0);
+                    acc[i] = __builtin_amdgcn_mfma_f32_32x32x16_f16(ah, bl, acc[i], 0, 0, 0);
+                    acc[i] = __builtin_amdgcn_mfma_f32_32x32x16_f16(al, bh, acc[i], 0, 0, 0);
+                }
+            }
+            cur = cur == RST - 1 ? 0 : cur + 1;
+        }
+#undef CORR_RING_ISSUE
+        asm volatile("s_waitcnt vmcnt(0)" ::: "memory");
+        __syncthreads();
+        for (int half = 0; half < 2; ++half) {
+            if (half) __syncthreads();
+#pragma unroll
+            for (int i = 0; i < NT; ++i) {
+                const int t = wv + 4 * i;
+                if (((2 * NB) % 4 == 0 || t < 2 * NB) && t / NB == half) {
+                    const int n = t - half * NB;
+#pragma unroll
+                    for (int e = 0; e < 16; ++e)
+                        S[((e >> 2) * 8 + lh * 4 + (e & 3)) * SP + n * 32 + l31] =
+                            acc[i][e] * (inv_sqrt_c / (PP_A_SCALE * PP_A_SCALE));
+                }
+            }
+            __syncthreads();
+            for (int idx = tid; idx < CM / 2 * win * win; idx += 256) {
+                const int ms = idx / (win * win), o = idx - ms * (win * win), ai = o / win, bi = o - ai * win, m = ms + 32 * half;
+                const int dx = s_bx[m] - ox, dy = s_by[m] - oy;
+                if (s_state[m] == 0 && dx >= 0 && dx <= fit && dy >= 0 && dy <= fit) {
+                    const float cx = s_cx[m], cy = s_cy[m];
+                    const float wx1 = cx - floorf(cx), wy1 = cy - floorf(cy), wx0 = 1.f - wx1, wy0 = 1.f - wy1;
+                    const float* t = S + ms * SP + (dy + bi) * RW + dx + ai;
+                    corr_put(out, out_hl, row0 + (size_t)(y0 + (m >> 3)) * W + x0 + (m & 7), ld_out, l * win * win + o,
+                             t[0] * (wx0 * wy0) + t[1] * (wx1 * wy0) + t[RW] * (wx0 * wy1) + t[RW + 1] * (wx1 * wy1));
+                }
+            }
+        }
+        __syncthreads();
+        if (tid < CM && s_state[tid] == 0) {
+            const int dx = s_bx[tid] - ox, dy = s_by[tid] - oy;
+            if (dx >= 0 && dx <= fit && dy >= 0 && dy <= fit) {
+                s_state[tid] = 1;
+                atomicSub(&s_org[2], 1);
+            }
+        }
+        __syncthreads();
+    }
+    __syncthreads();
+}
+#endif
+
+__global__ __launch_bounds__(256, 3) void corr_lookup_ring_kernel(const _Float16* __restrict__ f1h, int ld_f1, int f2_batch,
+                                                                  const _Float16* __restrict__ f2l0, const _Float16* __restrict__ f2l1,
+                                                                  const _Float16* __restrict__ f2l2, const float* __restrict__ flow, int B,
+                                                                  int H, int W, int C, int L, int r, int ld_flow, float inv_sqrt_c,
+                                                                  float* __restrict__ out, int ld_out, _Float16* __restrict__ out_hl) {
+#if defined(__HIP_DEVICE_COMPILE__)
+    extern __shared__ __attribute__((aligned(16))) float sm[];
+    __shared__ float s_cx[CM], s_cy[CM];
+    __shared__ int s_bx[CM], s_by[CM], s_state[CM], s_org[3];
+    const int tid = threadIdx.x;
+    const int tiles_x = W / CT, tiles = tiles_x * (H / CT), total = tiles * B;
+    int g = blockIdx.x;
+    if (total % 8 == 0) g = (g % 8) * (total / 8) + g / 8;
+    const int b = g / tiles, tile = g - b * tiles;
+    const int y0 = (tile / tiles_x) * CT, x0 = (tile % tiles_x) * CT;
+    const int win = 2 * r + 1;
+    const int my = tid >> 3, mx = tid & 7;
+    const size_t row0 = (size_t)b * H * W;
+    float gx = 0.f, gy = 0.f;
+    if (tid < CM) {
+        const float* fl = flow + (row0 + (size_t)(y0 + my) * W + x0 + mx) * ld_flow;
+        gx = (float)(x0 + mx) + fl[0];
+        gy = (float)(y0 + my) + fl[1];
+    }
+    for (int npad = ld_out - L * win * win, idx = tid; idx < CM * npad; idx += 256) {
+        const int m = idx / npad, o = idx - m * npad;
+        corr_put(out, out_hl, row0 + (size_t)(y0 + (m >> 3)) * W + x0 + (m & 7), ld_out, L * win * win + o, 0.f);
+    }
+    const _Float16* f1b = f1h + row0 * ld_f1 * 2;
+    const int f1_bytes = ((H * W - 1) * ld_f1 + C) * 4;
+    const size_t q = (size_t)(b % f2_batch);
+    corr_ring_level<RG0_W, RG0_N>(sm, s_cx, s_cy, s_bx, s_by, s_state, s_org, 0, f1b, ld_f1, f1_bytes, f2l0 + q * H * W * C * 2, H, W, C, gx, gy,
+                                  r, inv_sqrt_c, row0, y0, x0, W, out, out_hl, ld_out);
+    if (L > 1)
+        corr_ring_level<RG1_W, RG1_N>(sm, s_cx, s_cy, s_bx, s_by, s_state, s_org, 1, f1b, ld_f1, f1_bytes, f2l1 + q * (H >> 1) * (W >> 1) * C * 2,
+                                      H >> 1, W >> 1, C, gx, gy, r, inv_sqrt_c, row0, y0, x0, W, out, out_hl, ld_out);
+    if (L > 2)
+        corr_ring_level<RG2_W, RG2_N>(sm, s_cx, s_cy, s_bx, s_by, s_state, s_org, 2, f1b, ld_f1, f1_bytes, f2l2 + q * (H >> 2) * (W >> 2) * C * 2,
+                                      H >> 2, W >> 2, C, gx, gy, r, inv_sqrt_c, row0, y0, x0, W, out, out_hl, ld_out);
+#endif
 }
 
 __global__ __launch_bounds__(256) void gather_rows_kernel(const float* __restrict__ src, const long long* __restrict__ index,
@@ -750,9 +993,18 @@
     return pp_last_launch();
 }
 
+int pp_avgpool2_hl(const float* in, int B, int H, int W, int C, float* out, void* out_hl, void* stream) {
+    if (!in || !out_hl || B <= 0 || H < 2 || W < 2 || C <= 0 || H % 2 != 0 || W % 2 != 0 || C % 8 != 0) return PP_EINVAL;
+    if (((uintptr_t)in | (uintptr_t)out | (uintptr_t)out_hl) % 16 != 0) return PP_EINVAL;
+    const size_t n = (size_t)(H / 2) * (W / 2) * (C / 4);
+    const int gx = (int)((n + 255) / 256 < 1024 ? (n + 255) / 256 : 1024);
+    hipLaunchKernelGGL(avgpool2_hl_kernel, dim3(gx, B), dim3(256), 0, (hipStream_t)stream, in, H, W, C, out, (_Float16*)out_hl);
+    return pp_last_launch();
+}
+
 static int corr_tiled_launch(bool hl, const void* f1, int ld_f1, const void* f2_l0, const void* f2_l1, const void* f2_l2, int f2_batch,
                              const float* flow, int B, int H, int W, int C, int levels, int radius, int ld_flow, float* out, int ld_out,
-                             void* stream, bool exact = false, bool one = false) {
+                             void* stream, bool exact = false, bool one = false, void* out_hl = nullptr) {
     const size_t lds = (size_t)(CM * CSP > (CM + CN) * CKP ? CM * CSP : (CM + CN) * CKP) * sizeof(float);
     static signed char attr[PP_MAX_DEVICES];
     signed char& ok = attr[pp_cur_device()];
@@ -760,22 +1012,30 @@
         ok = hipFuncSetAttribute((const void*)corr_lookup_mfma_kernel<false>, hipFuncAttributeMaxDynamicSharedMemorySize, (int)lds) == hipSuccess &&
                      hipFuncSetAttribute((const void*)corr_lookup_mfma_kernel<true>, hipFuncAttributeMaxDynamicSharedMemorySize, (int)lds) == hipSuccess &&
                      hipFuncSetAttribute((const void*)corr_lookup_mfma_kernel<false, true>, hipFuncAttributeMaxDynamicSharedMemorySize, (int)lds) == hipSuccess &&
-                     hipFuncSetAttribute((const void*)corr_lookup_mfma_kernel<false, false, true>, hipFuncAttributeMaxDynamicSharedMemorySize, (int)lds) == hipSuccess
+                     hipFuncSetAttribute((const void*)corr_lookup_mfma_kernel<false, false, true>, hipFuncAttributeMaxDynamicSharedMemorySize, (int)lds) == hipSuccess &&
+                     hipFuncSetAttribute((const void*)corr_lookup_ring_kernel, hipFuncAttributeMaxDynamicSharedMemorySize, (int)CORR_RING_LDS) == hipSuccess
                  ? 1 : -1;
     if (ok < 0) return PP_ELAUNCH;
     const dim3 grid((unsigned)((H / CT) * (W / CT) * B));
-    if (exact)
+    _Float16* oh = (_Float16*)out_hl;
+    const char* re = getenv("PP_CORR_RING");
+    const bool ring = hl && !(re && re[0] == '0') && (long long)H * W * ld_f1 * 4 < 0x7FFFFFFFLL && (long long)H * W * C * 4 < 0x7FFFFFFFLL;
+    if (ring)
+        hipLaunchKernelGGL(corr_lookup_ring_kernel, grid, dim3(256), CORR_RING_LDS, (hipStream_t)stream, (const _Float16*)f1, ld_f1, f2_batch,
+                           (const _Float16*)f2_l0, (const _Float16*)f2_l1, (const _Float16*)f2_l2, flow, B, H, W, C, levels, radius, ld_flow,
+                           1.0f / sqrtf((float)C), out, ld_out, oh);
+    else if (exact)
         hipLaunchKernelGGL((corr_lookup_mfma_kernel<false, true>), grid, dim3(256), lds, (hipStream_t)stream, f1, ld_f1, f2_batch, f2_l0, f2_l1, f2_l2,
-                           flow, B, H, W, C, levels, radius, ld_flow, 1.0f / sqrtf((float)C), out, ld_out);
+                           flow, B, H, W, C, levels, radius, ld_flow, 1.0f / sqrtf((float)C), out, ld_out, oh);
     else if (one)
         hipLaunchKernelGGL((corr_lookup_mfma_kernel<false, false, true>), grid, dim3(256), lds, (hipStream_t)stream, f1, ld_f1, f2_batch, f2_l0, f2_l1,
-                           f2_l2, flow, B, H, W, C, levels, radius, ld_flow, 1.0f / sqrtf((float)C), out, ld_out);
+                           f2_l2, flow, B, H, W, C, levels, radius, ld_flow, 1.0f / sqrtf((float)C), out, ld_out, oh);
     else if (hl)
         hipLaunchKernelGGL(corr_lookup_mfma_kernel<true>, grid, dim3(256), lds, (hipStream_t)stream, f1, ld_f1, f2_batch, f2_l0, f2_l1, f2_l2,
-                           flow, B, H, W, C, levels, radius, ld_flow, 1.0f / sqrtf((float)C), out, ld_out);
+                           flow, B, H, W, C, levels, radius, ld_flow, 1.0f / sqrtf((float)C), out, ld_out, oh);
     else
         hipLaunchKernelGGL(corr_lookup_mfma_kernel<false>, grid, dim3(256), lds, (hipStream_t)stream, f1, ld_f1, f2_batch, f2_l0, f2_l1, f2_l2,
-                           flow, B, H, W, C, levels, radius, ld_flow, 1.0f / sqrtf((float)C), out, ld_out);
+                           flow, B, H, W, C, levels, radius, ld_flow, 1.0f / sqrtf((float)C), out, ld_out, oh);
     return pp_last_launch();
 }
 
@@ -822,19 +1082,28 @@
     return pp_last_launch();
 }
 
-int pp_corr_lookup_nhwc_hl(const void* f1_hl, int ld_f1, const void* f2_hl_l0, const void* f2_hl_l1, const void* f2_hl_l2,
-                           int f2_batch, const float* flow, int B, int H, int W, int C, int levels, int radius, int ld_flow,
-                           float* out, int ld_out, void* stream) {
-    if (!f1_hl || !f2_hl_l0 || !flow || !out || B <= 0 || H <= 0 || W <= 0 || C <= 0 || f2_batch <= 0) return PP_EINVAL;
+int pp_corr_lookup_nhwc_hl_op(const void* f1_hl, int ld_f1, const void* f2_hl_l0, const void* f2_hl_l1, const void* f2_hl_l2,
+                              int f2_batch, const float* flow, int B, int H, int W, int C, int levels, int radius, int ld_flow,
+                              float* out, int ld_out, void* out_hl, int ld_out_h, void* stream) {
+    if (!f1_hl || !f2_hl_l0 || !flow || (out != nullptr) == (out_hl != nullptr) || B <= 0 || H <= 0 || W <= 0 || C <= 0 || f2_batch <= 0)
+        return PP_EINVAL;
     if (H % CT != 0 || W % CT != 0 || C % CK != 0 || ld_f1 < C || ld_f1 % 8 != 0) return PP_EINVAL;
     if (((uintptr_t)f1_hl | (uintptr_t)f2_hl_l0 | (uintptr_t)f2_hl_l1 | (uintptr_t)f2_hl_l2) % 16 != 0) return PP_EINVAL;
     if (levels < 1 || levels > MAXL || radius < 1 || radius > MAXR) return PP_EINVAL;
     if ((levels > 1 && !f2_hl_l1) || (levels > 2 && !f2_hl_l2)) return PP_EINVAL;
     if ((H >> (levels - 1)) < 1 || (W >> (levels - 1)) < 1 || ld_flow < 2) return PP_EINVAL;
-    const int win = 2 * radius + 1;
-    if (ld_out < levels * win * win) return PP_EINVAL;
-    return corr_tiled_launch(true, f1_hl, ld_f1, f2_hl_l0, f2_hl_l1, f2_hl_l2, f2_batch, flow, B, H, W, C, levels, radius, ld_flow, out, ld_out,
-                             stream);
+    const int win = 2 * radius + 1, ld = out_hl ? ld_out_h : ld_out;
+    if (ld < levels * win * win) return PP_EINVAL;
+    if (out_hl && (ld_out_h % 8 != 0 || ((uintptr_t)out_hl % 16) != 0)) return PP_EINVAL;
+    return corr_tiled_launch(true, f1_hl, ld_f1, f2_hl_l0, f2_hl_l1, f2_hl_l2, f2_batch, flow, B, H, W, C, levels, radius, ld_flow, out, ld,
+                             stream, false, false, out_hl);
+}
+
+int pp_corr_lookup_nhwc_hl(const void* f1_hl, int ld_f1, const void* f2_hl_l0, const void* f2_hl_l1, const void* f2_hl_l2,
+                           int f2_batch, const float* flow, int B, int H, int W, int C, int levels, int radius, int ld_flow,
+                           float* out, int ld_out, void* stream) {
+    return pp_corr_lookup_nhwc_hl_op(f1_hl, ld_f1, f2_hl_l0, f2_hl_l1, f2_hl_l2, f2_batch, flow, B, H, W, C, levels, radius, ld_flow, out, ld_out,
+                                     nullptr, 0, stream);
 }
 
 int pp_corr_lookup_nhwc(const float* f1, int ld_f1, const float* f2_l0, const float* f2_l1, const float* f2_l2,
diff --git a/picopose_amd/model/stage3.py b/picopose_amd/model/stage3.py
--- a/picopose_amd/model/stage3.py
+++ b/picopose_amd/model/stage3.py
@@ -224,7 +224,8 @@
             elif not train:
                 fr = ops.conv2d(fr_src, pk[f"proj{l}"], pk[f"proj{l}_b"], 1, out=X[..., 0:256])
             ncorr = (l + 1) * (2 * self.r + 1) ** 2
-            corr = ops.corr_lookup(fr, fq, flow, l + 1, self.r, c_pad=-(-ncorr // 8) * 8, **hl_maps)
+            corr_op = lean and bool(hl_maps) and ops.corr_takes_operands(hl_maps["f1_hl"], hl_maps["f2_hl"], H, W, 256)
+            corr = ops.corr_lookup(fr, fq, flow, l + 1, self.r, c_pad=-(-ncorr // 8) * 8, out_split=corr_op, **hl_maps)
             hl_cat = opcat
             if hl_cat:
                 cf = ops.Split.empty(B * H * W, 256, dev)
diff --git a/picopose_amd/ops.py b/picopose_amd/ops.py
--- a/picopose_amd/ops.py
+++ b/picopose_amd/ops.py
@@ -1060,6 +1060,21 @@
     return out
 
 
+def avgpool2_hl(x, keep_f32=True):
+    B, H, W, C = x.shape
+    assert x.is_contiguous() and C % 8 == 0 and terms() == 2
+    out = torch.empty(B, H // 2, W // 2, C, dtype=torch.float32, device=x.device) if keep_f32 else None
+    sp = Split.empty(B * (H // 2) * (W // 2), C, x.device)
+    sp.image = (B, H // 2, W // 2)
+    _lib.check(_lib.lib().pp_avgpool2_hl(_p(x), B, H, W, C, _p(out) if keep_f32 else None, _p(sp.hl), _lib.stream_ptr()), "pp_avgpool2_hl")
+    _chk(sp.hl, "pp_avgpool2_hl")
+    return out, sp
+
+
+def corr_operand_out():
+    return os.environ.get("PP_CORR_OPERAND_OUT", "1") != "0"
+
+
 def decoder_lean():
     return os.environ.get("PP_DECODER_LEAN", "1") != "0"
 
@@ -1069,7 +1084,7 @@
             and os.environ.get("PP_CORR_TILED", "1") != "0" and os.environ.get("PP_CORR_HL", "1") != "0")
 
 
-def corr_lookup(f1, f2, flow, levels, radius, c_pad=None, f1_hl=None, f2_hl=None):
+def corr_lookup(f1, f2, flow, levels, radius, c_pad=None, f1_hl=None, f2_hl=None, out_split=False):
     (H, W, C), B = f2.shape[1:], flow.shape[0]
     assert f2.is_contiguous() and flow.stride(3) == 1 and B % f2.shape[0] == 0 and tuple(flow.shape[1:3]) == (H, W)
     operands = corr_takes_operands(f1_hl, f2_hl, H, W, C)
@@ -1077,19 +1092,39 @@
         assert operands, "corr_lookup without the fp32 map f1 needs the operand form of both maps (corr_takes_operands)"
     else:
         assert tuple(f1.shape) == (B, H, W, C) and f1.stride(3) == 1 and f1.stride(1) == W * f1.stride(2) and f1.stride(0) == H * f1.stride(1)
-    pyr = [f2]
-    for _ in range(levels - 1):
-        pyr.append(avgpool2(pyr[-1]))
     n = levels * (2 * radius + 1) ** 2
     np_ = c_pad if c_pad and c_pad > n else n
-    out = (torch.zeros if np_ > n and not decoder_lean() else torch.empty)(B, H, W, np_, dtype=torch.float32, device=f2.device)
+    assert not out_split or (operands and np_ % 8 == 0), "corr_lookup(out_split=True) needs the operand branch and a padded channel count"
+    fused = operands and corr_operand_out()
+    pyr, hls = [f2], [f2_hl.hl if operands else None]
+    for i in range(levels - 1):
+        if fused:
+            p, sp = avgpool2_hl(pyr[-1], keep_f32=i < levels - 2)
+            pyr.append(p)
+            hls.append(sp.hl)
+        else:
+            pyr.append(avgpool2(pyr[-1]))
+            if operands:
+                p = pyr[-1]
+                hls.append(split_activation(p, p.shape[0], p.shape[1] * p.shape[2], C, p.shape[1] * p.shape[2] * C, C))
     if operands:
         tgt, col0 = f1_hl
         assert tgt.shape[0] == B * H * W and col0 % 8 == 0 and col0 + C <= tgt.shape[1] and f2_hl.shape == (f2.shape[0] * H * W, C)
-        hls = [f2_hl.hl] + [split_activation(p, p.shape[0], p.shape[1] * p.shape[2], C, p.shape[1] * p.shape[2] * C, C) for p in pyr[1:]]
-        _lib.check(_lib.lib().pp_corr_lookup_nhwc_hl(tgt.hl.data_ptr() + 4 * col0, tgt.shape[1], _p(hls[0]), _p(hls[1]) if levels > 1 else None,
-                                                     _p(hls[2]) if levels > 2 else None, f2.shape[0], _p(flow), B, H, W, C, levels, radius,
-                                                     flow.stride(2), _p(out), np_, _lib.stream_ptr()), "pp_corr_lookup_nhwc_hl")
+        args = (tgt.hl.data_ptr() + 4 * col0, tgt.shape[1], _p(hls[0]), _p(hls[1]) if levels > 1 else None, _p(hls[2]) if levels > 2 else None,
+                f2.shape[0], _p(flow), B, H, W, C, levels, radius, flow.stride(2))
+        if out_split and fused:
+            sp = Split.empty(B * H * W, np_, f2.device)
+            sp.image = (B, H, W)
+            _lib.check(_lib.lib().pp_corr_lookup_nhwc_hl_op(*args, None, np_, _p(sp.hl), np_, _lib.stream_ptr()), "pp_corr_lookup_nhwc_hl_op")
+            _chk(sp.hl, "pp_corr_lookup_nhwc_hl_op")
+            return sp
+    out = (torch.zeros if np_ > n and not decoder_lean() else torch.empty)(B, H, W, np_, dtype=torch.float32, device=f2.device)
+    if operands:
+        _lib.check(_lib.lib().pp_corr_lookup_nhwc_hl(*args, _p(out), np_, _lib.stream_ptr()), "pp_corr_lookup_nhwc_hl")
+        if out_split:
+            sp = Split(split_activation(out, B, H * W, np_, H * W * np_, np_))
+            sp.image = (B, H, W)
+            return sp
         return out
     _lib.check(_lib.lib().pp_corr_lookup_nhwc_ex(_p(f1), f1.stride(2), _p(pyr[0]), _p(pyr[1]) if levels > 1 else None,
                                                  _p(pyr[2]) if levels > 2 else None, f2.shape[0], _p(flow), B, H, W, C,
```

Measured after the change: 590.8 (median of 6 runs). 1.1% higher.
